# BenChung/SuccessiveConvexification

Measured on AMD Instinct MI355X. Metric: 6-DoF K=50 SCvx iterations/sec (batch), higher is better.
Workload: dtype f64

## Files before the change

successiveconvexification_amd/csrc/scvx_batch.hip:

```cpp
#include <cmath>
#include <cstdlib>
#include <cstring>
#include <limits>
#include <new>
#include <vector>

#include <cstdio>
#include "scvx_socp.hpp"

using scvx::fail;

namespace scvx {

__global__ __launch_bounds__(64, SCVX_K4_OCC) void socp_kernel(ipm::Consts C, int B, size_t work_stride,
                                                  const double* __restrict__ x, const double* __restrict__ u,
                                                  const double* __restrict__ endpoint, const double* __restrict__ deriv,
                                                  const double* __restrict__ rk, const double* __restrict__ ic,
                                                  const int* __restrict__ active, double* __restrict__ work,
                                                  double* __restrict__ sol, double* __restrict__ nu,
                                                  double* __restrict__ info, const int* __restrict__ step_status,
                                                  double* __restrict__ ttr, double* __restrict__ acc,
                                                  const double* __restrict__ marg) {
    socp_body<WaveEx>(C, B, work_stride, x, u, endpoint, deriv, rk, ic, active, work, sol, nu, info, step_status, ttr, acc, marg);
}
__global__ __launch_bounds__(64, SCVX_K4_OCC) void socp_lin32_kernel(ipm::Consts C, int B, size_t work_stride,
                                                  const double* __restrict__ x, const double* __restrict__ u,
                                                  const double* __restrict__ endpoint, const float* __restrict__ deriv,
                                                  const double* __restrict__ rk, const double* __restrict__ ic,
                                                  const int* __restrict__ active, double* __restrict__ work,
                                                  double* __restrict__ sol, double* __restrict__ nu,
                                                  double* __restrict__ info, const int* __restrict__ step_status,
                                                  double* __restrict__ ttr, double* __restrict__ acc,
                                                  const double* __restrict__ marg) {
    socp_body<WaveEx, float>(C, B, work_stride, x, u, endpoint, deriv, rk, ic, active, work, sol, nu, info, step_status, ttr, acc, marg);
}


__global__ void candidate_kernel(int B, int nrec, const double* __restrict__ traj, const double* __restrict__ sol,
                                 double* __restrict__ cand) {
    const size_t i = (size_t)blockIdx.x * blockDim.x + threadIdx.x;
    if (i < (size_t)B * nrec) cand[i] = traj[i] + sol[i];
}

__global__ void unpack_kernel(int B, int K, int NU, const double* __restrict__ rec, double* __restrict__ x,
                              double* __restrict__ u, double* __restrict__ sigma) {
    const int nrec = (K + 1) * (14 + NU) + 1, nx = (K + 1) * 14, nu = (K + 1) * NU;
    const size_t i = (size_t)blockIdx.x * blockDim.x + threadIdx.x;
    if (i >= (size_t)B * nrec) return;
    const size_t b = i / nrec;
    const int r = (int)(i - b * nrec);
    const double v = rec[i];
    if (r < nx) x[b * nx + r] = v;
    else if (r < nx + nu) u[b * nu + (r - nx)] = v;
    else sigma[b] = v;
}

struct TrParams {
    double wNu, rh0, rh1, rh2, alph, bet, ri, nuTol, delTol;
    int K, imax, NU, pad;
};

__global__ __launch_bounds__(64) void tr_update_kernel(TrParams P, int B, const double* __restrict__ cand,
                                                       const double* __restrict__ xprop, const double* __restrict__ nu,
                                                       const double* __restrict__ info, double* __restrict__ traj,
                                                       double* __restrict__ rk, double* __restrict__ cost,
                                                       int* __restrict__ iter, int* __restrict__ status,
                                                       const int* mask , int* active,
                                                       int* live, double* __restrict__ out, double* __restrict__ acc,
                                                       int* __restrict__ nlive, int* __restrict__ k1skip) {
    const int b = blockIdx.x;
    if (b >= B) return;
    if (!mask[b]) {
        if (threadIdx.x == 0) k1skip[b] = SCVX_ST_REJECTED;
        return;
    }
    const int K = P.K, nrec = (K + 1) * (14 + P.NU) + 1;
    const double* c = cand + (size_t)b * nrec;
    const double* xp = xprop + (size_t)b * K * 14;
    const double* nv = nu + (size_t)b * K * 14;
    double d2 = 0, n2 = 0;
    for (int i = threadIdx.x; i < K * 14; i += 64) {
        const double d = c[14 + i] - xp[i];
        d2 += d * d;
        n2 += nv[i] * nv[i];
    }
#pragma unroll
    for (int o = 32; o > 0; o >>= 1) { d2 += __shfl_xor(d2, o, 64); n2 += __shfl_xor(n2, o, 64); }
    const double mf = c[14 * K];
    const double jK = -mf + P.wNu * sqrt(d2);
    const double nun = sqrt(n2);
    const double lK = -mf + P.wNu * nun;
    const int sstat = (int)info[4 * b];
    int st;
    bool accept = false;
    double next_rk = rk[b], dJ = INFINITY;
    if (sstat != 0 && sstat != 4) {
        st = sstat == 3 ? SCVX_ST_NONFINITE : (sstat == 5 ? SCVX_ST_INFEASIBLE : SCVX_ST_SOLVER);
    } else if (!(jK == jK) || !(lK == lK)) {
        st = SCVX_ST_NONFINITE;
    } else {
        const double jKm = cost[b];
        const double djk = jKm - jK, dlk = jKm - lK;
        const double rhk = djk / dlk;
        if (rk[b] == INFINITY) { next_rk = P.ri; accept = true; dJ = NAN; }
        else if (rhk < P.rh0) { next_rk = rk[b] / P.alph; accept = false; dJ = INFINITY; }
        else {
            accept = true;
            dJ = djk;
            if (rhk < P.rh1) next_rk = rk[b] / P.alph;
            else if (P.rh1 <= rhk && rhk < P.rh2) next_rk = rk[b];
            else next_rk = P.bet * rk[b];
        }
        st = accept ? SCVX_ST_RUNNING : SCVX_ST_REJECTED;
    }
    if (accept) {
        double* t = traj + (size_t)b * nrec;
        for (int i = threadIdx.x; i < nrec; i += 64) t[i] = c[i];
    }
    if (threadIdx.x == 0) {
        const int it = iter[b] + 1;
        iter[b] = it;
        const int was_live = live[b];
        if (st == SCVX_ST_SOLVER || st == SCVX_ST_NONFINITE || st == SCVX_ST_INFEASIBLE) {
            active[b] = 0;
            live[b] = 0;
        } else {
            rk[b] = next_rk;
            if (accept) cost[b] = jK;
            if (accept && nun <= P.nuTol && dJ <= P.delTol) { st = SCVX_ST_CONVERGED; live[b] = 0; }
        }
        if (was_live && !live[b]) atomicSub(nlive, 1);
        status[b] = st;
        k1skip[b] = accept && st != SCVX_ST_SOLVER && st != SCVX_ST_NONFINITE && st != SCVX_ST_INFEASIBLE ? SCVX_ST_RUNNING : SCVX_ST_REJECTED;
        out[2 * b] = nun;
        out[2 * b + 1] = dJ;
        atomicAdd(acc + ACC_TRAJ_STEPS, 1.0);
        if (st == SCVX_ST_REJECTED) atomicAdd(acc + ACC_REJECTED, 1.0);
        else if (st == SCVX_ST_CONVERGED) atomicAdd(acc + ACC_CONVERGED, 1.0);
        else if (st != SCVX_ST_RUNNING) atomicAdd(acc + ACC_FAILED, 1.0);
    }
}

__global__ void reset_scalars_kernel(int B, double* __restrict__ rk, double* __restrict__ cost, int* __restrict__ iter,
                                     int* __restrict__ status, int* __restrict__ active, int* __restrict__ live,
                                     double* __restrict__ out, double* __restrict__ info) {
    const int i = blockIdx.x * blockDim.x + threadIdx.x;
    if (i >= B) return;
    rk[i] = 100.0; cost[i] = INFINITY; iter[i] = 0; status[i] = SCVX_ST_RUNNING; active[i] = 1; live[i] = 1;
    out[2 * i] = 0.0; out[2 * i + 1] = 0.0;
    for (int q = 0; q < 4; q++) info[4 * i + q] = 0.0;
}

__global__ void replan_scalars_kernel(int B, double* __restrict__ rk, double* __restrict__ cost, int* __restrict__ iter,
                                      int* __restrict__ status, const int* __restrict__ active, int* __restrict__ live,
                                      double* __restrict__ ttr) {
    const int i = blockIdx.x * blockDim.x + threadIdx.x;
    if (i >= B || !active[i]) return;
    rk[i] = 100.0; cost[i] = INFINITY; iter[i] = 0; status[i] = SCVX_ST_RUNNING; live[i] = 1;
    ttr[i] = 1.7976931348623157e308;
}

__global__ __launch_bounds__(64) void margins_from_psig_kernel(int B, int K, const double* __restrict__ psig, double nsigma, double cap,
                                                               double* __restrict__ marg) {
    const int b = blockIdx.x;
    if (b >= B) return;
    const double* p = psig + (size_t)b * (K + 1) * SCVX_PSIG_N;
    int bad = 0;
    for (int k = threadIdx.x; k <= K; k += 64) {
        const double s = p[(size_t)k * SCVX_PSIG_N + SCVX_PSIG_THRUST];
        bad |= !(s == s);
    }
    bad = __syncthreads_or(bad);
    double* m = marg + (size_t)b * (K + 1) * 2;
    for (int k = threadIdx.x; k <= K; k += 64) {
        const double v = bad ? 0.0 : fmin(nsigma * p[(size_t)k * SCVX_PSIG_N + SCVX_PSIG_THRUST], cap);
        m[2 * k] = v;
        m[2 * k + 1] = v;
    }
}

__global__ void copy_flags_kernel(int B, const int* __restrict__ src, int* __restrict__ dst, int* __restrict__ nlive) {
    const int i = blockIdx.x * blockDim.x + threadIdx.x;
    const int v = i < B ? src[i] : 0;
    if (i < B) dst[i] = v;
    const unsigned long long m = __ballot(v != 0);
    if ((threadIdx.x & 63) == 0 && m) atomicAdd(nlive, (int)__popcll(m));
}

}

struct scvx_batch {
    scvx_ctx* ctx = nullptr;
    int B = 0, K = 0, nrec = 0;
    int NU = 3, dsz = 294;
    scvx_solver_opts opts{};
    scvx::ipm::Consts C{};
    scvx::TrParams tr{};
    size_t work_stride = 0;
    double *traj = nullptr, *cand = nullptr, *sol = nullptr;
    double *traj0 = nullptr;
    double *x = nullptr, *u = nullptr, *sigma = nullptr;
    double *cx = nullptr, *cu = nullptr, *csigma = nullptr;
    double *endpoint = nullptr, *deriv = nullptr, *xprop = nullptr, *nu = nullptr;
    float* deriv_f = nullptr;
    double *rk = nullptr, *cost = nullptr, *ic = nullptr, *info = nullptr, *out = nullptr, *work = nullptr;
    double *ttr = nullptr;
    double *acc = nullptr;
    double *marg = nullptr;
    bool marg_on = false;
    double *cov_s0 = nullptr, *cov_rep = nullptr, *cov_psig = nullptr;
    double *track_gain = nullptr, *track_p0 = nullptr;
    int *k1skip = nullptr;
    int *d_nlive = nullptr;
    int *h_nlive = nullptr;
    hipEvent_t ev_nlive[2] = {nullptr, nullptr};
    int *iter = nullptr, *status = nullptr;
    int *active = nullptr;
    int *live = nullptr;
    int device = 0;
    int nactive_host = -1;
    int nlive_hint = -1;
    bool initialised = false;
    bool profiling = false;
    std::vector<hipEvent_t> events;
    size_t nmarks = 0;
};

namespace {


void rotation_between_e1(const double* b, double* q) {
    const double nb = std::sqrt(b[0] * b[0] + b[1] * b[1] + b[2] * b[2]);
    double w = nb + b[0];
    double v[3];
    if (std::fabs(w) < 100 * std::numeric_limits<double>::epsilon()) {
        v[0] = 0; v[1] = 0; v[2] = 1;
        w = 0;
    } else {
        v[0] = 0; v[1] = -b[2]; v[2] = b[1];
    }
    const double n = std::sqrt(w * w + v[0] * v[0] + v[1] * v[1] + v[2] * v[2]);
    q[0] = w / n; q[1] = v[0] / n; q[2] = v[1] / n; q[3] = v[2] / n;
}

template <class T>
int dmalloc(scvx_ctx* ctx, T** p, size_t n) {
    SCVX_HIP(ctx, hipMalloc((void**)p, n * sizeof(T)));
    return SCVX_OK;
}

int split_views(scvx_batch* b, const double* rec, double* x, double* u, double* sigma) {
    const size_t n = (size_t)b->B * b->nrec;
    hipLaunchKernelGGL(scvx::unpack_kernel, dim3((unsigned)((n + 255) / 256)), dim3(256), 0, b->ctx->stream, b->B, b->K, b->NU,
                       rec, x, u, sigma);
    SCVX_HIP(b->ctx, hipGetLastError());
    return SCVX_OK;
}

int socp_waves(int B, int num_cus) {
    if (const char* v = std::getenv("SCVX_K4_WAVES"); v && *v) {
        const int w = std::atoi(v);
        return w >= 4 ? 4 : (w >= 2 ? 2 : 1);
    }
    const int cus = num_cus > 0 ? num_cus : 256;
    return B <= 2 * cus ? 4 : (B <= 4 * cus ? 2 : 1);
}

template <int NW>
void launch_socp_block(scvx_batch* b, const int* mask) {
    constexpr int NU = 3;
    if (b->deriv_f)
        hipLaunchKernelGGL((scvx::socp_block_kernel<NW, float, NU>), dim3(b->B), dim3(64 * NW), 0, b->ctx->stream, b->C, b->B, b->work_stride,
                           b->x, b->u, b->endpoint, b->deriv_f, b->rk, b->ic, mask, b->work, b->sol, b->nu, b->info, b->status, b->ttr, b->acc, b->marg_on ? b->marg : nullptr);
    else
        hipLaunchKernelGGL((scvx::socp_block_kernel<NW, double, NU>), dim3(b->B), dim3(64 * NW), 0, b->ctx->stream, b->C, b->B, b->work_stride,
                           b->x, b->u, b->endpoint, b->deriv, b->rk, b->ic, mask, b->work, b->sol, b->nu, b->info, b->status, b->ttr, b->acc, b->marg_on ? b->marg : nullptr);
}

hipError_t relinearize(scvx_batch* b, const int* skip) {
    const double dt = 1.0 / (b->K + 1);
    if (b->deriv_f)
        return scvx::launch_linearize_store_f32(b->ctx, b->B, b->K, b->x, b->u, b->sigma, dt, b->endpoint, b->deriv_f, b->ctx->stream, skip);
    return scvx::launch_linearize(b->ctx, b->B, b->K, b->x, b->u, b->sigma, dt, b->endpoint, b->deriv, b->ctx->stream, skip);
}

int enqueue_socp(scvx_batch* b, const int* mask) {
    const int w = socp_waves(b->nlive_hint >= 0 && b->nlive_hint < b->B ? (b->nlive_hint > 0 ? b->nlive_hint : 1) : b->B, b->ctx->num_cus);
    if (b->NU == 5) {
        scvx::SocpLaunch a{b->C, b->B, b->work_stride, b->x, b->u, b->endpoint, b->deriv, b->deriv_f, b->rk, b->ic, mask,
                           b->work, b->sol, b->nu, b->info, b->status, b->ttr, b->acc, b->marg_on ? b->marg : nullptr, b->ctx->stream};
        scvx::launch_socp_fin(a, w);
    } else if (w == 4) launch_socp_block<4>(b, mask);
    else if (w == 2) launch_socp_block<2>(b, mask);
    else if (b->deriv_f)
        hipLaunchKernelGGL(scvx::socp_lin32_kernel, dim3(b->B), dim3(64), 0, b->ctx->stream, b->C, b->B, b->work_stride, b->x, b->u,
                           b->endpoint, b->deriv_f, b->rk, b->ic, mask, b->work, b->sol, b->nu, b->info, b->status, b->ttr, b->acc, b->marg_on ? b->marg : nullptr);
    else
        hipLaunchKernelGGL(scvx::socp_kernel, dim3(b->B), dim3(64), 0, b->ctx->stream, b->C, b->B, b->work_stride, b->x, b->u,
                           b->endpoint, b->deriv, b->rk, b->ic, mask, b->work, b->sol, b->nu, b->info, b->status, b->ttr, b->acc, b->marg_on ? b->marg : nullptr);
    SCVX_HIP(b->ctx, hipGetLastError());
    return SCVX_OK;
}

constexpr size_t PROF_MAX_STEPS = 4096;

int mark(scvx_batch* b) {
    if (!b->profiling || b->nmarks >= 7 * PROF_MAX_STEPS) return SCVX_OK;
    if (b->nmarks == b->events.size()) {
        hipEvent_t e;
        SCVX_HIP(b->ctx, hipEventCreate(&e));
        b->events.push_back(e);
    }
    SCVX_HIP(b->ctx, hipEventRecord(b->events[b->nmarks], b->ctx->stream));
    b->nmarks++;
    return SCVX_OK;
}

int enqueue_step(scvx_batch* b, const int* mask) {
    scvx_ctx* ctx = b->ctx;
    hipStream_t st = ctx->stream;
    const double dt = 1.0 / (b->K + 1);
    int rc = mark(b);
    if (rc) return rc;
    rc = enqueue_socp(b, mask);
    if (rc) return rc;
    if ((rc = mark(b))) return rc;
    const size_t n = (size_t)b->B * b->nrec;
    hipLaunchKernelGGL(scvx::candidate_kernel, dim3((unsigned)((n + 255) / 256)), dim3(256), 0, st, b->B, b->nrec, b->traj,
                       b->sol, b->cand);
    SCVX_HIP(ctx, hipGetLastError());
    rc = split_views(b, b->cand, b->cx, b->cu, b->csigma);
    if (rc) return rc;
    if ((rc = mark(b))) return rc;
    SCVX_HIP(ctx, scvx::launch_propagate(ctx, b->B, b->K, b->cx, b->cu, b->csigma, dt, b->xprop, st));
    if ((rc = mark(b))) return rc;
    hipLaunchKernelGGL(scvx::tr_update_kernel, dim3(b->B), dim3(64), 0, st, b->tr, b->B, b->cand, b->xprop, b->nu, b->info,
                       b->traj, b->rk, b->cost, b->iter, b->status, mask, b->active, b->live, b->out, b->acc, b->d_nlive, b->k1skip);
    SCVX_HIP(ctx, hipGetLastError());
    if ((rc = mark(b))) return rc;
    rc = split_views(b, b->traj, b->x, b->u, b->sigma);
    if (rc) return rc;
    if ((rc = mark(b))) return rc;
    SCVX_HIP(ctx, relinearize(b, b->k1skip));
    if ((rc = mark(b))) return rc;
    return SCVX_OK;
}

int check_batch(scvx_batch* b, bool need_init) {
    if (!b || !b->ctx) return SCVX_ERR_ARG;
    if (need_init && !b->initialised) return fail(b->ctx, SCVX_ERR_STATE, "call scvx_batch_init first");
    if (b->ctx->prob.aero_kind == 1 && !b->ctx->dyn.aero)
        return fail(b->ctx, SCVX_ERR_STATE, "AtmosphericData problem: call scvx_set_aero_table first");
    hipError_t e = hipSetDevice(b->ctx->device);
    if (e != hipSuccess) return fail(b->ctx, SCVX_ERR_HIP, "hipSetDevice failed");
    return SCVX_OK;
}

}

extern "C" {

int scvx_solver_default_opts(scvx_solver_opts* o) {
    if (!o) return SCVX_ERR_ARG;
    o->max_iter = 60;
    o->refine = 6;
    o->tol = 1e-8;
    o->accept_tol = 1e-8;
    o->reuse_inactive_tr = 0;
    o->warm_start = 1;
    o->retries = 5;
    o->reserved0 = 0;
    return SCVX_OK;
}

int scvx_batch_create(scvx_ctx* ctx, int B, scvx_batch** out) {
    if (!ctx || !out) return SCVX_ERR_ARG;
    *out = nullptr;
    if (B < 1) return fail(ctx, SCVX_ERR_ARG, "B >= 1 required");
    SCVX_HIP(ctx, hipSetDevice(ctx->device));
    scvx_batch* b = new (std::nothrow) scvx_batch();
    if (!b) return SCVX_ERR_NOMEM;
    b->ctx = ctx;
    b->device = ctx->device;
    b->B = B;
    const scvx_problem& p = ctx->prob;
    const int K = p.K;
    b->K = K;
    b->NU = scvx_control_dim(ctx);
    b->dsz = 14 * (14 + 2 * b->NU + 1);
    b->nrec = (K + 1) * (14 + b->NU) + 1;
    scvx_solver_default_opts(&b->opts);
    scvx::ipm::Consts& C = b->C;
    const double d2r = M_PI / 180.0;
    C.K = K; C.max_iter = b->opts.max_iter; C.refine = b->opts.refine; C.pad = 0; C.tol = b->opts.tol;
    C.accept = b->opts.accept_tol;
    C.pad = b->opts.reuse_inactive_tr;
    C.warm = b->opts.warm_start;
    C.retries = b->opts.retries;
    C.itan = 1.0 / std::tan(p.gammaGs * d2r);
    C.sqcm = std::sqrt((1.0 - std::cos(p.thetaMax * d2r)) / 2.0);
    C.icos = 1.0 / std::cos(p.deltaMax * d2r);
    C.Tmax = p.Tmax; C.Tmin = p.Tmin; C.omMax = p.omMax; C.mdry = p.mdry; C.wNu = p.wNu; C.mwet = p.mwet;
    C.vmax = (p.model_flags & SCVX_MODEL_DPMAX) ? std::sqrt(2.0 * p.dpMax / p.rho) : 0.0;
    C.finmxf = p.finmxf;
    for (int i = 0; i < 3; i++) { C.rIf[i] = p.rIf[i]; C.vIf[i] = p.vIf[i]; C.wBi[i] = p.wBi[i]; C.wBf[i] = p.wBf[i]; }
    for (int i = 0; i < 4; i++) C.qBIf[i] = p.qBIf[i];
    scvx::TrParams& T = b->tr;
    T.wNu = p.wNu; T.rh0 = p.rh0; T.rh1 = p.rh1; T.rh2 = p.rh2; T.alph = p.alph; T.bet = p.bet; T.ri = p.ri;
    T.nuTol = p.nuTol; T.delTol = p.delTol; T.K = K; T.imax = p.imax; T.NU = b->NU; T.pad = 0;
    scvx::ipm::Layout L;
    L.init(K, C.vmax > 0.0, b->NU);
    b->work_stride = (L.work_doubles() + 7) & ~(size_t)7;
    if (const char* v = std::getenv("SCVX_WORK_PAD"); v && *v) b->work_stride += (size_t)std::atoi(v) & ~(size_t)7;
    const size_t nB = (size_t)B;
    int rc = 0;
    rc |= dmalloc(ctx, &b->traj, nB * b->nrec);
    rc |= dmalloc(ctx, &b->cand, nB * b->nrec);
    rc |= dmalloc(ctx, &b->traj0, nB * b->nrec);
    rc |= dmalloc(ctx, &b->sol, nB * b->nrec);
    rc |= dmalloc(ctx, &b->x, nB * (K + 1) * 14);
    rc |= dmalloc(ctx, &b->u, nB * (K + 1) * b->NU);
    rc |= dmalloc(ctx, &b->sigma, nB);
    rc |= dmalloc(ctx, &b->cx, nB * (K + 1) * 14);
    rc |= dmalloc(ctx, &b->cu, nB * (K + 1) * b->NU);
    rc |= dmalloc(ctx, &b->csigma, nB);
    rc |= dmalloc(ctx, &b->endpoint, nB * K * 14);
    rc |= dmalloc(ctx, &b->deriv, nB * K * b->dsz);
    rc |= dmalloc(ctx, &b->xprop, nB * K * 14);
    rc |= dmalloc(ctx, &b->nu, nB * K * 14);
    rc |= dmalloc(ctx, &b->rk, nB);
    rc |= dmalloc(ctx, &b->cost, nB);
    rc |= dmalloc(ctx, &b->ic, nB * 6);
    rc |= dmalloc(ctx, &b->info, nB * 4);
    rc |= dmalloc(ctx, &b->out, nB * 2);
    rc |= dmalloc(ctx, &b->ttr, nB);
    rc |= dmalloc(ctx, &b->acc, (size_t)scvx::ACC_N);
    rc |= dmalloc(ctx, &b->d_nlive, (size_t)1);
    rc |= dmalloc(ctx, &b->k1skip, nB);
    rc |= dmalloc(ctx, &b->marg, nB * (K + 1) * 2);
    if (!rc && (hipHostMalloc((void**)&b->h_nlive, 2 * sizeof(int), hipHostMallocDefault) != hipSuccess ||
                hipEventCreateWithFlags(&b->ev_nlive[0], hipEventDisableTiming) != hipSuccess ||
                hipEventCreateWithFlags(&b->ev_nlive[1], hipEventDisableTiming) != hipSuccess)) rc = SCVX_ERR_HIP;
    if (!rc && hipMemset(b->acc, 0, sizeof(double) * scvx::ACC_N) != hipSuccess) rc = SCVX_ERR_HIP;
    rc |= dmalloc(ctx, &b->work, nB * b->work_stride);
    rc |= dmalloc(ctx, &b->iter, nB);
    rc |= dmalloc(ctx, &b->status, nB);
    rc |= dmalloc(ctx, &b->active, nB);
    rc |= dmalloc(ctx, &b->live, nB);
    if (rc) {
        scvx_batch_destroy(b);
        return fail(ctx, SCVX_ERR_NOMEM, "device allocation failed for the batch (" + std::to_string(nB * b->work_stride * 8 >> 20) + " MiB of solver workspace)");
    }
    *out = b;
    return SCVX_OK;
}

void scvx_batch_destroy(scvx_batch* b) {
    if (!b) return;
    (void)hipSetDevice(b->device);
    for (hipEvent_t e : b->events) (void)hipEventDestroy(e);
    for (hipEvent_t e : b->ev_nlive) if (e) (void)hipEventDestroy(e);
    if (b->h_nlive) (void)hipHostFree(b->h_nlive);
    void* ptrs[] = {b->traj0, b->traj, b->cand, b->sol, b->x, b->u, b->sigma, b->cx, b->cu, b->csigma, b->endpoint, b->deriv, b->xprop,
                    b->nu, b->rk, b->cost, b->ic, b->info, b->out, b->work, b->iter, b->status, b->active, b->live, b->ttr, b->deriv_f, b->acc, b->d_nlive, b->k1skip,
                    b->track_gain, b->track_p0, b->marg, b->cov_s0, b->cov_rep, b->cov_psig};
    for (void* p : ptrs)
        if (p) (void)hipFree(p);
    delete b;
}

int scvx_batch_set_solver(scvx_batch* b, const scvx_solver_opts* o) {
    if (!b || !o) return SCVX_ERR_ARG;
    if (o->max_iter < 1 || o->refine < 0 || !(o->tol > 0) || !(o->accept_tol >= o->tol) || o->retries < 0 || o->retries > 7)
        return fail(b->ctx, SCVX_ERR_ARG, "bad solver options (max_iter >= 1, refine >= 0, 0 < tol <= accept_tol, 0 <= retries <= 7)");
    if (o->reserved0 != 0)
        return fail(b->ctx, SCVX_ERR_ARG, "scvx_solver_opts.reserved0 must be 0 (start from scvx_solver_opts_default; an older struct layout is not accepted)");
    b->opts = *o;
    b->C.max_iter = o->max_iter;
    b->C.refine = o->refine;
    b->C.tol = o->tol;
    b->C.accept = o->accept_tol;
    b->C.pad = o->reuse_inactive_tr ? 1 : 0;
    b->C.warm = o->warm_start ? 1 : 0;
    b->C.retries = o->retries;
    return SCVX_OK;
}

int scvx_batch_init(scvx_batch* b, const double* ic) {
    int rc = check_batch(b, false);
    if (rc) return rc;
    scvx_ctx* ctx = b->ctx;
    const scvx_problem& p = ctx->prob;
    const int K = b->K, B = b->B, nrec = b->nrec;
    std::vector<double> rec((size_t)B * nrec), hic((size_t)B * 6), hrk(B, 100.0), hcost(B, INFINITY);
    std::vector<int> hiter(B, 0), hstat(B, SCVX_ST_RUNNING), hact(B, 1);
    for (int t = 0; t < B; t++) {
        double* c = &hic[(size_t)t * 6];
        for (int i = 0; i < 3; i++) { c[i] = ic ? ic[(size_t)t * 6 + i] : p.rIi[i]; c[3 + i] = ic ? ic[(size_t)t * 6 + 3 + i] : p.vIi[i]; }
        double* r = &rec[(size_t)t * nrec];
        double* X = r;
        double* U = r + (size_t)(K + 1) * 14;
        for (int k = 0; k <= K; k++) {
            const double a = (double)(K - k) / K, bb = (double)k / K;
            double* xk = X + 14 * k;
            const double mk = a * p.mwet + bb * p.mdry;
            xk[0] = mk;
            double nv[3];
            for (int i = 0; i < 3; i++) {
                xk[1 + i] = a * c[i] + bb * p.rIf[i];
                xk[4 + i] = a * c[3 + i] + bb * p.vIf[i];
                nv[i] = -xk[4 + i];
                xk[11 + i] = 0.0;
            }
            rotation_between_e1(nv, xk + 7);
            for (int c = 0; c < b->NU; c++) U[b->NU * k + c] = 0.0;
            U[b->NU * k] = mk * p.g;
        }
        r[nrec - 1] = p.tf_guess;
    }
    hipStream_t st = ctx->stream;
    SCVX_HIP(ctx, hipMemcpyAsync(b->traj, rec.data(), rec.size() * 8, hipMemcpyHostToDevice, st));
    SCVX_HIP(ctx, hipMemcpyAsync(b->traj0, b->traj, rec.size() * 8, hipMemcpyDeviceToDevice, st));
    SCVX_HIP(ctx, hipMemcpyAsync(b->ic, hic.data(), hic.size() * 8, hipMemcpyHostToDevice, st));
    SCVX_HIP(ctx, hipMemcpyAsync(b->rk, hrk.data(), (size_t)B * 8, hipMemcpyHostToDevice, st));
    SCVX_HIP(ctx, hipMemcpyAsync(b->cost, hcost.data(), (size_t)B * 8, hipMemcpyHostToDevice, st));
    SCVX_HIP(ctx, hipMemcpyAsync(b->iter, hiter.data(), (size_t)B * 4, hipMemcpyHostToDevice, st));
    SCVX_HIP(ctx, hipMemcpyAsync(b->status, hstat.data(), (size_t)B * 4, hipMemcpyHostToDevice, st));
    SCVX_HIP(ctx, hipMemcpyAsync(b->active, hact.data(), (size_t)B * 4, hipMemcpyHostToDevice, st));
    SCVX_HIP(ctx, hipMemcpyAsync(b->live, hact.data(), (size_t)B * 4, hipMemcpyHostToDevice, st));
    SCVX_HIP(ctx, hipMemsetAsync(b->out, 0, (size_t)B * 16, st));
    SCVX_HIP(ctx, hipMemsetAsync(b->info, 0, (size_t)B * 32, st));
    SCVX_HIP(ctx, hipMemsetAsync(b->ttr, 0x7f, (size_t)B * 8, st));
    rc = split_views(b, b->traj, b->x, b->u, b->sigma);
    if (rc) return rc;
    SCVX_HIP(ctx, relinearize(b, nullptr));
    SCVX_HIP(ctx, hipStreamSynchronize(st));
    b->initialised = true;
    b->nactive_host = -1;
    b->marg_on = false;
    return SCVX_OK;
}

int scvx_batch_init_threedof(scvx_batch* b, const double* ic, const scvx_threedof_opts* opts, int32_t* status3) {
    int rc = scvx_batch_init(b, ic);
    if (rc) return rc;
    scvx_ctx* ctx = b->ctx;
    const int B = b->B, K = b->K;
    hipStream_t st = ctx->stream;
    const size_t no = (size_t)scvx_threedof_record_doubles(K);
    double *d_sol = nullptr, *d_info = nullptr;
    hipError_t e = hipMalloc((void**)&d_sol, (size_t)B * no * 8);
    if (e == hipSuccess) e = hipMalloc((void**)&d_info, (size_t)B * 6 * 8);
    std::vector<double> hinfo((size_t)B * 6);
    if (e == hipSuccess) {
        rc = scvx::threedof_solve_dev(ctx, B, b->ic, opts, d_sol, d_info);
        if (rc == SCVX_OK) rc = scvx::threedof_to_record(ctx, B, K, d_sol, d_info, b->traj, opts ? opts->attitude : 0);
        if (rc == SCVX_OK) {
            e = hipMemcpyAsync(b->traj0, b->traj, (size_t)B * b->nrec * 8, hipMemcpyDeviceToDevice, st);
            if (e == hipSuccess) e = hipMemcpyAsync(hinfo.data(), d_info, hinfo.size() * 8, hipMemcpyDeviceToHost, st);
        }
        if (rc == SCVX_OK && e == hipSuccess) rc = split_views(b, b->traj, b->x, b->u, b->sigma);
        if (rc == SCVX_OK && e == hipSuccess)
            e = relinearize(b, nullptr);
    }
    const hipError_t es = hipStreamSynchronize(st);
    if (d_sol) (void)hipFree(d_sol);
    if (d_info) (void)hipFree(d_info);
    if (rc) return rc;
    if (e != hipSuccess || es != hipSuccess)
        return fail(ctx, SCVX_ERR_HIP, std::string("scvx_batch_init_threedof: ") + hipGetErrorString(e != hipSuccess ? e : es));
    if (status3) for (int t = 0; t < B; t++) status3[t] = (int32_t)hinfo[(size_t)t * 6];
    return SCVX_OK;
}

int scvx_batch_reset(scvx_batch* b) {
    int rc = check_batch(b, true);
    if (rc) return rc;
    scvx_ctx* ctx = b->ctx;
    hipStream_t st = ctx->stream;
    SCVX_HIP(ctx, hipMemcpyAsync(b->traj, b->traj0, (size_t)b->B * b->nrec * 8, hipMemcpyDeviceToDevice, st));
    hipLaunchKernelGGL(scvx::reset_scalars_kernel, dim3((unsigned)((b->B + 255) / 256)), dim3(256), 0, st, b->B, b->rk, b->cost,
                       b->iter, b->status, b->active, b->live, b->out, b->info);
    SCVX_HIP(ctx, hipGetLastError());
    rc = split_views(b, b->traj, b->x, b->u, b->sigma);
    if (rc) return rc;
    SCVX_HIP(ctx, relinearize(b, nullptr));
    b->nactive_host = -1;
    return SCVX_OK;
}

int scvx_solve_step_async(scvx_batch* b) {
    int rc = check_batch(b, true);
    if (rc) return rc;
    b->nlive_hint = b->nactive_host >= 0 && b->nactive_host < b->B ? b->nactive_host : -1;
    rc = enqueue_step(b, b->active);
    b->nlive_hint = -1;
    return rc;
}

static int read_step_outputs(scvx_batch* b, int32_t* status, double* nu_norm, double* dJ) {
    scvx_ctx* ctx = b->ctx;
    const int B = b->B;
    std::vector<double> out((size_t)B * 2);
    SCVX_HIP(ctx, hipMemcpyAsync(out.data(), b->out, out.size() * 8, hipMemcpyDeviceToHost, ctx->stream));
    if (status) SCVX_HIP(ctx, hipMemcpyAsync(status, b->status, (size_t)B * 4, hipMemcpyDeviceToHost, ctx->stream));
    SCVX_HIP(ctx, hipStreamSynchronize(ctx->stream));
    for (int t = 0; t < B; t++) {
        if (nu_norm) nu_norm[t] = out[2 * t];
        if (dJ) dJ[t] = out[2 * t + 1];
    }
    return SCVX_OK;
}

int scvx_solve_step(scvx_batch* b, int32_t* status, double* nu_norm, double* dJ) {
    int rc = scvx_solve_step_async(b);
    if (rc) return rc;
    return read_step_outputs(b, status, nu_norm, dJ);
// ... 372 lines not shown
        SCVX_HIP(ctx, relinearize(b, nullptr));
        SCVX_HIP(ctx, hipMemsetAsync(b->ttr, 0x7f, (size_t)b->B * 8, ctx->stream));
        SCVX_HIP(ctx, hipStreamSynchronize(ctx->stream));
    }
    return SCVX_OK;
}

int scvx_batch_get_scalars(scvx_batch* b, double* rk, double* cost, int32_t* iter) {
    int rc = check_batch(b, true);
    if (rc) return rc;
    scvx_ctx* ctx = b->ctx;
    if (rk) SCVX_HIP(ctx, hipMemcpyAsync(rk, b->rk, (size_t)b->B * 8, hipMemcpyDeviceToHost, ctx->stream));
    if (cost) SCVX_HIP(ctx, hipMemcpyAsync(cost, b->cost, (size_t)b->B * 8, hipMemcpyDeviceToHost, ctx->stream));
    if (iter) SCVX_HIP(ctx, hipMemcpyAsync(iter, b->iter, (size_t)b->B * 4, hipMemcpyDeviceToHost, ctx->stream));
    SCVX_HIP(ctx, hipStreamSynchronize(ctx->stream));
    return SCVX_OK;
}

int scvx_batch_set_scalars(scvx_batch* b, const double* rk, const double* cost, const int32_t* iter) {
    int rc = check_batch(b, true);
    if (rc) return rc;
    scvx_ctx* ctx = b->ctx;
    if (rk) SCVX_HIP(ctx, hipMemcpyAsync(b->rk, rk, (size_t)b->B * 8, hipMemcpyHostToDevice, ctx->stream));
    if (cost) SCVX_HIP(ctx, hipMemcpyAsync(b->cost, cost, (size_t)b->B * 8, hipMemcpyHostToDevice, ctx->stream));
    if (iter) SCVX_HIP(ctx, hipMemcpyAsync(b->iter, iter, (size_t)b->B * 4, hipMemcpyHostToDevice, ctx->stream));
    SCVX_HIP(ctx, hipMemsetAsync(b->ttr, 0x7f, (size_t)b->B * 8, ctx->stream));
    SCVX_HIP(ctx, hipStreamSynchronize(ctx->stream));
    return SCVX_OK;
}

int scvx_batch_get_solver_stats(scvx_batch* b, int32_t* status, int32_t* iters, double* merit, double* pobj) {
    int rc = check_batch(b, true);
    if (rc) return rc;
    scvx_ctx* ctx = b->ctx;
    std::vector<double> info((size_t)b->B * 4);
    SCVX_HIP(ctx, hipMemcpyAsync(info.data(), b->info, info.size() * 8, hipMemcpyDeviceToHost, ctx->stream));
    SCVX_HIP(ctx, hipStreamSynchronize(ctx->stream));
    for (int t = 0; t < b->B; t++) {
        if (status) status[t] = (int32_t)info[4 * t];
        if (iters) iters[t] = (int32_t)info[4 * t + 1];
        if (merit) merit[t] = info[4 * t + 2];
        if (pobj) pobj[t] = info[4 * t + 3];
    }
    return SCVX_OK;
}

int scvx_debug_build_switches(char* out, int n) {
    return std::snprintf(out, (size_t)(n > 0 ? n : 0),
                         "CHOL_DPP=%d CHOL_ORDER=%d RESID_UPDATE=%d RESID_FRESH_FROM=%g TWISTED_TSPACE=%d FUSED_RES=%d CARRY_BIGSUMS=%d REFINE_FUSED=%d "
                         "K4_OCC=%d K4_BLOCK_OCC=%d K4_PIPELINE=%d K4_TWISTED=%d STREAM_U=%d CHAIN_R=%d FACTOR_T=%d PROF=%d",
                         SCVX_CHOL_DPP, SCVX_CHOL_ORDER, SCVX_RESID_UPDATE, (double)SCVX_RESID_FRESH_FROM, SCVX_TWISTED_TSPACE, SCVX_FUSED_RES,
                         SCVX_CARRY_BIGSUMS, SCVX_REFINE_FUSED, SCVX_K4_OCC, SCVX_K4_BLOCK_OCC, SCVX_K4_PIPELINE, SCVX_K4_TWISTED, SCVX_STREAM_U,
                         SCVX_CHAIN_R, (int)sizeof(SCVX_FACTOR_T),
#if defined(SCVX_IPM_PROF)
                         1
#else
                         0
#endif
                         );
}

#if defined(SCVX_IPM_PROF)
int scvx_debug_ipm_prof(scvx_batch* b, double* out32) {
    (void)hipStreamSynchronize(b->ctx->stream);
    return hipMemcpy(out32, b->work, 128 * 8, hipMemcpyDeviceToHost) == hipSuccess ? 0 : -2;
}
#endif

int scvx_batch_get_step_stats(scvx_batch* b, double* out8, int reset) {
    int rc = check_batch(b, false);
    if (rc) return rc;
    if (!out8) return fail(b->ctx, SCVX_ERR_ARG, "null buffer");
    scvx_ctx* ctx = b->ctx;
    static_assert(scvx::ACC_N == 8, "scvx_batch_get_step_stats documents eight totals");
    SCVX_HIP(ctx, hipMemcpyAsync(out8, b->acc, sizeof(double) * scvx::ACC_N, hipMemcpyDeviceToHost, ctx->stream));
    if (reset) SCVX_HIP(ctx, hipMemsetAsync(b->acc, 0, sizeof(double) * scvx::ACC_N, ctx->stream));
    SCVX_HIP(ctx, hipStreamSynchronize(ctx->stream));
    return SCVX_OK;
}

int scvx_batch_set_profiling(scvx_batch* b, int enable) {
    if (!b) return SCVX_ERR_ARG;
    b->nmarks = 0;
    b->profiling = enable != 0;
    return SCVX_OK;
}

int scvx_batch_get_profile(scvx_batch* b, double* ms, int64_t* steps) {
    int rc = check_batch(b, true);
    if (rc) return rc;
    if (!ms || !steps) return fail(b->ctx, SCVX_ERR_ARG, "null buffer");
    scvx_ctx* ctx = b->ctx;
    SCVX_HIP(ctx, hipStreamSynchronize(ctx->stream));
    for (int i = 0; i < 5; i++) ms[i] = 0.0;
    const size_t n = b->nmarks / 7;
    static const int slot[6] = {0, 4, 1, 2, 4, 3};
    for (size_t s = 0; s < n; s++)
        for (int i = 0; i < 6; i++) {
            float t = 0.f;
            SCVX_HIP(ctx, hipEventElapsedTime(&t, b->events[7 * s + i], b->events[7 * s + i + 1]));
            ms[slot[i]] += (double)t;
        }
    *steps = (int64_t)n;
    b->nmarks = 0;
    return SCVX_OK;
}

int scvx_batch_get_flags(scvx_batch* b, int32_t* status, int32_t* active, int32_t* live) {
    int rc = check_batch(b, true);
    if (rc) return rc;
    scvx_ctx* ctx = b->ctx;
    if (status) SCVX_HIP(ctx, hipMemcpyAsync(status, b->status, (size_t)b->B * 4, hipMemcpyDeviceToHost, ctx->stream));
    if (active) SCVX_HIP(ctx, hipMemcpyAsync(active, b->active, (size_t)b->B * 4, hipMemcpyDeviceToHost, ctx->stream));
    if (live) SCVX_HIP(ctx, hipMemcpyAsync(live, b->live, (size_t)b->B * 4, hipMemcpyDeviceToHost, ctx->stream));
    SCVX_HIP(ctx, hipStreamSynchronize(ctx->stream));
    return SCVX_OK;
}

int scvx_batch_set_flags(scvx_batch* b, const int32_t* status, const int32_t* active, const int32_t* live) {
    int rc = check_batch(b, true);
    if (rc) return rc;
    scvx_ctx* ctx = b->ctx;
    if (status) SCVX_HIP(ctx, hipMemcpyAsync(b->status, status, (size_t)b->B * 4, hipMemcpyHostToDevice, ctx->stream));
    if (active) {
        SCVX_HIP(ctx, hipMemcpyAsync(b->active, active, (size_t)b->B * 4, hipMemcpyHostToDevice, ctx->stream));
        int n = 0;
        for (int t = 0; t < b->B; t++) n += active[t] != 0;
        b->nactive_host = n;
    }
    if (live) SCVX_HIP(ctx, hipMemcpyAsync(b->live, live, (size_t)b->B * 4, hipMemcpyHostToDevice, ctx->stream));
    SCVX_HIP(ctx, hipMemsetAsync(b->ttr, 0x7f, (size_t)b->B * 8, ctx->stream));
    SCVX_HIP(ctx, hipStreamSynchronize(ctx->stream));
    return SCVX_OK;
}

int scvx_allgather_trajectories(scvx_batch* b, double* out_dev) {
    int rc = check_batch(b, true);
    if (rc) return rc;
    return scvx_allgather_f64(b->ctx, b->traj, out_dev, (int64_t)b->B * b->nrec);
}

int scvx_allgather_status(scvx_batch* b, int32_t* status_out_dev, int32_t* iters_out_dev) {
    int rc = check_batch(b, true);
    if (rc) return rc;
    if (status_out_dev && (rc = scvx_allgather_i32(b->ctx, b->status, status_out_dev, b->B))) return rc;
    if (iters_out_dev && (rc = scvx_allgather_i32(b->ctx, b->iter, iters_out_dev, b->B))) return rc;
    return SCVX_OK;
}

int scvx_socp_solve(scvx_batch* b, double* sol, double* nu) {
    int rc = check_batch(b, true);
    if (rc) return rc;
    scvx_ctx* ctx = b->ctx;
    rc = enqueue_socp(b, b->active);
    if (rc) return rc;
    const size_t n = (size_t)b->B * b->nrec;
    hipLaunchKernelGGL(scvx::candidate_kernel, dim3((unsigned)((n + 255) / 256)), dim3(256), 0, ctx->stream, b->B, b->nrec,
                       b->traj, b->sol, b->cand);
    SCVX_HIP(ctx, hipGetLastError());
    if (sol) SCVX_HIP(ctx, hipMemcpyAsync(sol, b->cand, n * 8, hipMemcpyDeviceToHost, ctx->stream));
    if (nu) SCVX_HIP(ctx, hipMemcpyAsync(nu, b->nu, (size_t)b->B * b->K * 14 * 8, hipMemcpyDeviceToHost, ctx->stream));
    SCVX_HIP(ctx, hipStreamSynchronize(ctx->stream));
    return SCVX_OK;
}

}
```

successiveconvexification_amd/csrc/scvx_discretize.hip:

```cpp
#include <type_traits>
#include "scvx_internal.hpp"

namespace scvx {

constexpr int WAVES_PER_BLOCK = 4;

template <bool AERO, bool FIN = false> struct K1Map {
    static constexpr int LPS = FIN ? 25 : (AERO ? 21 : 15), SPW = FIN ? 2 : (AERO ? 3 : 4);
    static constexpr int NU = FIN ? 5 : 3, NP = 14 + 2 * NU + 1, DSZ = 14 * NP, HV = DSZ / 2;
};
__device__ __forceinline__ int exo_slot_to_col(int slot) {
    return slot == 0 ? 0 : slot + 6;
}

__device__ __forceinline__ bool block_unchanged(const int* skip, long seg0, int nseg_block, long nseg, int K) {
    if (!skip || seg0 >= nseg) return false;
    long seg1 = seg0 + nseg_block - 1;
    if (seg1 >= nseg) seg1 = nseg - 1;
    const long b0 = seg0 / K, b1 = seg1 / K;
    for (long b = b0; b <= b1; b++)
        if (skip[b] < SCVX_ST_REJECTED) return false;
    return true;
}

template <typename R> struct Vec2;
template <> struct Vec2<double> { typedef double2 type; };
template <> struct Vec2<float> { typedef float2 type; };

template <bool AERO, typename R>
__global__ __launch_bounds__(64 * WAVES_PER_BLOCK, sizeof(R) == 4 ? 2 : 1) void linearize_kernel(
    DynP<R> p, long nseg, int K, const R* __restrict__ x, const R* __restrict__ u,
    const R* __restrict__ sigma, R dt, int nsub, R* __restrict__ endpoint,
    R* __restrict__ deriv, const int* __restrict__ skip) {
    constexpr int LPS = K1Map<AERO>::LPS, SPW = K1Map<AERO>::SPW;
    typedef typename Vec2<R>::type VEC2;
    if (block_unchanged(skip, (long)blockIdx.x * WAVES_PER_BLOCK * SPW, WAVES_PER_BLOCK * SPW, nseg, K)) return;
    __shared__ __attribute__((aligned(16))) R tile[WAVES_PER_BLOCK][SPW * 294];
    const int lane = threadIdx.x & 63;
    const int wave = threadIdx.x >> 6;
    const long gwave = (long)blockIdx.x * WAVES_PER_BLOCK + wave;
    const int sl = lane / LPS;
    const int slot = lane - sl * LPS;
    const int col = AERO ? slot : exo_slot_to_col(slot);
    const long seg0 = gwave * SPW;
    long seg = seg0 + sl;
    const bool active = (sl < SPW) && (seg < nseg);
    if (!active) seg = (seg0 < nseg) ? seg0 : nseg - 1;
    const long b = seg / K;
    const int k = (int)(seg - b * K);
    const R* xk = x + ((size_t)b * (K + 1) + k) * 14;
    const R* uk = u + ((size_t)b * (K + 1) + k) * 3;
    const R sig = sigma[b];

    R xs[14], c[14];
#pragma unroll
    for (int i = 0; i < 14; i++) {
        xs[i] = xk[i];
        c[i] = (col == i) ? R(1.0) : R(0.0);
    }
    const R uk0 = uk[0], uk1 = uk[1], uk2 = uk[2];
    const R up0 = uk[3], up1 = uk[4], up2 = uk[5];
    const bool is_uk = (col >= 14) && (col < 17);
    const bool is_up = (col >= 17) && (col < 20);
    const int comp = is_uk ? col - 14 : (is_up ? col - 17 : -1);
    const R gsel = (col == 20) ? R(1.0) : R(0.0);
    const R e0 = (comp == 0) ? R(1.0) : R(0.0), e1 = (comp == 1) ? R(1.0) : R(0.0), e2 = (comp == 2) ? R(1.0) : R(0.0);

    const R h = dt / R(nsub);
    const R inv_n = R(1.0) / R(nsub);
    for (int s = 0; s < nsub; s++) {
        R xa[14], ca[14], xt[14], ct[14];
#pragma unroll
        for (int i = 0; i < 14; i++) {
            xa[i] = xs[i];
            ca[i] = c[i];
            xt[i] = xs[i];
            ct[i] = c[i];
        }
#pragma unroll
        for (int stg = 0; stg < 4; stg++) {
            const R lkp = (R(s) + (stg == 0 ? R(0.0) : (stg == 3 ? R(1.0) : R(0.5)))) * inv_n;
            const R lkm = R(1.0) - lkp;
            R uu[3] = {fma(uk0, lkm, up0 * lkp), fma(uk1, lkm, up1 * lkp), fma(uk2, lkm, up2 * lkp)};
            const R wk = is_uk ? lkm : (is_up ? lkp : R(0.0));
            const R wc[3] = {e0 * wk, e1 * wk, e2 * wk};
            Stage<AERO, R> st;
            stage_eval<AERO>(p, xt, uu, st);
            R dc[14];
            column_deriv<AERO>(p, st, xt, uu, ct, wc, gsel, sig, dc);
            const R wacc = h * ((stg == 0 || stg == 3) ? (R(1.0) / R(6.0)) : (R(1.0) / R(3.0)));
            const R wnext = h * (stg == 2 ? R(1.0) : R(0.5));
#pragma unroll
            for (int i = 0; i < 14; i++) {
                const R dx = sig * st.g[i];
                xa[i] = fma(wacc, dx, xa[i]);
                ca[i] = fma(wacc, dc[i], ca[i]);
                if (stg < 3) {
                    xt[i] = fma(wnext, dx, xs[i]);
                    ct[i] = fma(wnext, dc[i], c[i]);
                }
            }
        }
#pragma unroll
        for (int i = 0; i < 14; i++) {
            xs[i] = xa[i];
            c[i] = ca[i];
        }
    }

    R* t = tile[wave];
    if (sl < SPW) {
#pragma unroll
        for (int i = 0; i < 14; i++) t[sl * 294 + col * 14 + i] = c[i];
        if (!AERO && slot < 6) {
            const int j = slot < 3 ? slot : slot - 3;
            R* cc = t + sl * 294 + (slot < 3 ? 1 + j : 4 + j) * 14;
#pragma unroll
            for (int i = 0; i < 14; i++) cc[i] = R(0.0);
            if (slot < 3) cc[1 + j] = R(1.0);
            else { cc[1 + j] = sig * dt; cc[4 + j] = R(1.0); }
        }
    }
    __syncthreads();
    if (seg0 < nseg) {
        const long rem = nseg - seg0;
        const int nvalid = rem < SPW ? (int)rem : SPW;
        const int n2 = nvalid * 147;
        VEC2* out = reinterpret_cast<VEC2*>(deriv + (size_t)seg0 * 294);
        const VEC2* src = reinterpret_cast<const VEC2*>(t);
#pragma unroll
        for (int r = 0; r < (SPW * 147 + 63) / 64; r++) {
            const int e = lane + 64 * r;
            if (e < n2) out[e] = src[e];
        }
        if (active && slot == 0) {
            R* ep = endpoint + (size_t)seg * 14;
#pragma unroll
            for (int i = 0; i < 14; i++) ep[i] = xs[i];
        }
    }
}

#ifndef SCVX_PC_WAVES
#define SCVX_PC_WAVES 8
#endif
#ifndef SCVX_PC_PROD
#define SCVX_PC_PROD 0
#endif
#ifndef SCVX_PC_BLOCKS_PER_CU
#define SCVX_PC_BLOCKS_PER_CU 1
#endif
constexpr int PC_BLOCKS_PER_CU = SCVX_PC_BLOCKS_PER_CU;
constexpr int PC_WAVES = SCVX_PC_WAVES;
constexpr int PC_PROD = SCVX_PC_PROD;
__device__ __forceinline__ void lds_barrier() {
    __builtin_amdgcn_fence(__ATOMIC_RELEASE, "workgroup", "local");
    __builtin_amdgcn_s_barrier();
    __builtin_amdgcn_fence(__ATOMIC_ACQUIRE, "workgroup", "local");
}
#if defined(SCVX_K1_PROF)
__device__ double g_k1prof[2 * 16];
#define K1_BAR() do { const unsigned long long tb_ = __builtin_amdgcn_s_memtime(); lds_barrier(); k1wait_ += (double)(__builtin_amdgcn_s_memtime() - tb_); } while (0)
#else
#define K1_BAR() lds_barrier()
#endif
template <bool AERO, bool FIN, bool TRQ, typename R>
__device__ __forceinline__ void column_deriv_rec_any(const DynP<R>& p, const R* rec, int stride, const R* c, const R* wc, R gsel,
                                                     R sigma, R* dc) {
    column_deriv_rec_pieces<AERO, FIN, TRQ, R>(p, rec, stride, c, wc, gsel, sigma, dc);
}
constexpr int PC_GROUP = 4;
template <bool AERO, bool SG, typename R, typename O = R, bool FIN = false, bool TRQ = false>
__global__ __launch_bounds__(64 * PC_WAVES) void linearize_pc_kernel(
    DynPK<R, TRQ> p, long nseg, int K, const R* __restrict__ x, const R* __restrict__ u,
    const R* __restrict__ sigma, R dt, int nsub, R* __restrict__ endpoint,
    O* __restrict__ deriv, const int* __restrict__ skip) {
    constexpr int LPS = K1Map<AERO, FIN>::LPS, SPW = K1Map<AERO, FIN>::SPW;
    constexpr int NU = K1Map<AERO, FIN>::NU, NP = K1Map<AERO, FIN>::NP, DSZ = K1Map<AERO, FIN>::DSZ, HV = K1Map<AERO, FIN>::HV;
    typedef typename Vec2<R>::type VEC2;
    typedef typename Vec2<O>::type OVEC2;
    constexpr int NC = PC_WAVES - 1;
    if (block_unchanged(skip, (long)blockIdx.x * (NC * SPW), NC * SPW, nseg, K)) return;
    constexpr int NS = NC * SPW;
    constexpr int NR = StageRec<AERO, FIN, TRQ>::N;
    constexpr int RING = SG ? 2 : 2 * PC_GROUP;
    constexpr int RING_D = RING * NR * NS, TILE_D = NC * SPW * DSZ;
    __shared__ __attribute__((aligned(16))) R lds[RING_D > TILE_D ? RING_D : TILE_D];
    const int lane = threadIdx.x & 63;
    const int wave = threadIdx.x >> 6;
    const long seg_base = (long)blockIdx.x * NS;
    const R h = dt / R(nsub);
    const R inv_n = R(1.0) / R(nsub);

    if (wave == PC_PROD) {
        const bool live = lane < NS;
        long seg = seg_base + (live ? lane : 0);
        const bool valid = live && seg < nseg;
        if (seg >= nseg) seg = nseg - 1;
        const long b = seg / K;
        const int k = (int)(seg - b * K);
        const R* xk = x + ((size_t)b * (K + 1) + k) * 14;
        const R* uk = u + ((size_t)b * (K + 1) + k) * NU;
        const R sig = sigma[b];
        R xs[14], xa[14], xt[14];
#pragma unroll
        for (int i = 0; i < 14; i++) { xs[i] = xk[i]; xa[i] = xs[i]; xt[i] = xs[i]; }
        R ukv[NU], upv[NU];
#pragma unroll
        for (int j = 0; j < NU; j++) { ukv[j] = uk[j]; upv[j] = uk[NU + j]; }
        const int l = live ? lane : 0;
        for (int s = 0; s <= nsub; s++) {
            if (s < nsub) {
#pragma unroll
                for (int stg = 0; stg < 4; stg++) {
                    const R lkp = (R(s) + (stg == 0 ? R(0.0) : (stg == 3 ? R(1.0) : R(0.5)))) * inv_n;
                    const R lkm = R(1.0) - lkp;
                    R uu[NU];
#pragma unroll
                    for (int j = 0; j < NU; j++) uu[j] = fma(ukv[j], lkm, upv[j] * lkp);
                    struct { R g[14]; } st;
                    stage_eval_publish<AERO, FIN, TRQ>(p, xt, uu, st.g, lds + (SG ? (stg & 1) : (s & 1) * PC_GROUP + stg) * NR * NS + l, NS, live);
                    const R wacc = h * ((stg == 0 || stg == 3) ? (R(1.0) / R(6.0)) : (R(1.0) / R(3.0)));
                    const R wnext = h * (stg == 2 ? R(1.0) : R(0.5));
#pragma unroll
                    for (int i = 0; i < 14; i++) {
                        const R dx = sig * st.g[i];
                        xa[i] = fma(wacc, dx, xa[i]);
                        xt[i] = (stg < 3) ? fma(wnext, dx, xs[i]) : xa[i];
                    }
                    if (SG) __syncthreads();
                }
#pragma unroll
                for (int i = 0; i < 14; i++) xs[i] = xa[i];
            }
            if (!SG || s == nsub) __syncthreads();
        }
        if (valid) {
            R* ep = endpoint + (size_t)seg * 14;
#pragma unroll
            for (int i = 0; i < 14; i++) ep[i] = xs[i];
        }
        __syncthreads();
        return;
    }

    const int cw = wave < PC_PROD ? wave : wave - 1;
    const int sl = lane / LPS;
    const int slot = lane - sl * LPS;
    const int col = (AERO || FIN) ? slot : exo_slot_to_col(slot);
    const bool lane_live = sl < SPW;
    const int ls = cw * SPW + (lane_live ? sl : 0);
    long seg = seg_base + ls;
    if (seg >= nseg) seg = nseg - 1;
    const R sig = sigma[seg / K];
    R c[14], ca[14], ct[14];
#pragma unroll
    for (int i = 0; i < 14; i++) { c[i] = (col == i) ? R(1.0) : R(0.0); ca[i] = c[i]; ct[i] = c[i]; }
    const bool is_uk = (col >= 14) && (col < 14 + NU);
    const bool is_up = (col >= 14 + NU) && (col < 14 + 2 * NU);
    const int comp = is_uk ? col - 14 : (is_up ? col - 14 - NU : -1);
    const R gsel = (col == NP - 1) ? R(1.0) : R(0.0);
    R ec[NU];
#pragma unroll
    for (int j = 0; j < NU; j++) ec[j] = (comp == j) ? R(1.0) : R(0.0);
    __syncthreads();
    for (int s = 0; s < nsub; s++) {
#pragma unroll
        for (int stg = 0; stg < 4; stg++) {
            const R lkp = (R(s) + (stg == 0 ? R(0.0) : (stg == 3 ? R(1.0) : R(0.5)))) * inv_n;
            const R lkm = R(1.0) - lkp;
            const R wk = is_uk ? lkm : (is_up ? lkp : R(0.0));
            R wc[NU];
#pragma unroll
            for (int j = 0; j < NU; j++) wc[j] = ec[j] * wk;
            R dc[14];
            column_deriv_rec_any<AERO, FIN, TRQ>(p, lds + (SG ? (stg & 1) : (s & 1) * PC_GROUP + stg) * NR * NS + ls, NS, ct, wc, gsel, sig, dc);
            const R wacc = h * ((stg == 0 || stg == 3) ? (R(1.0) / R(6.0)) : (R(1.0) / R(3.0)));
            const R wnext = h * (stg == 2 ? R(1.0) : R(0.5));
#pragma unroll
            for (int i = 0; i < 14; i++) {
                ca[i] = fma(wacc, dc[i], ca[i]);
                ct[i] = (stg < 3) ? fma(wnext, dc[i], c[i]) : ca[i];
            }
            if (SG) __syncthreads();
        }
#pragma unroll
        for (int i = 0; i < 14; i++) c[i] = ca[i];
        if (!SG) __syncthreads();
    }
    R* t = lds + cw * SPW * DSZ;
    if (lane_live) {
#pragma unroll
        for (int i = 0; i < 14; i++) t[sl * DSZ + col * 14 + i] = c[i];
        if (!AERO && !FIN && slot < 6) {
            const int j = slot < 3 ? slot : slot - 3;
            R* cc = t + sl * DSZ + (slot < 3 ? 1 + j : 4 + j) * 14;
#pragma unroll
            for (int i = 0; i < 14; i++) cc[i] = R(0.0);
            if (slot < 3) cc[1 + j] = R(1.0);
            else { cc[1 + j] = sig * dt; cc[4 + j] = R(1.0); }
        }
    }
    __syncthreads();
    const long seg0 = seg_base + (long)cw * SPW;
    if (seg0 < nseg) {
        const long rem = nseg - seg0;
        const int nvalid = rem < SPW ? (int)rem : SPW;
        const int n2 = nvalid * HV;
        OVEC2* out = reinterpret_cast<OVEC2*>(deriv + (size_t)seg0 * DSZ);
        const VEC2* src = reinterpret_cast<const VEC2*>(t);
#pragma unroll
        for (int r = 0; r < (SPW * HV + 63) / 64; r++) {
            const int e = lane + 64 * r;
            if (e < n2) { const VEC2 v = src[e]; OVEC2 o; o.x = O(v.x); o.y = O(v.y); out[e] = o; }
        }
    }
}

#ifndef SCVX_K1_NB_EXO
#define SCVX_K1_NB_EXO 1
#endif
template <bool AERO, typename R, typename O = R, bool FIN = false, int NB = 1, bool TRQ = false>
__global__ __launch_bounds__(64 * PC_WAVES) void linearize_pcp_kernel(
    DynPK<R, TRQ> p, long nseg, int K, const R* __restrict__ x, const R* __restrict__ u,
    const R* __restrict__ sigma, R dt, int nsub, R* __restrict__ endpoint,
    O* __restrict__ deriv, const int* __restrict__ skip) {
    constexpr int LPS = K1Map<AERO, FIN>::LPS, SPW = K1Map<AERO, FIN>::SPW;
    constexpr int NU = K1Map<AERO, FIN>::NU, NP = K1Map<AERO, FIN>::NP, DSZ = K1Map<AERO, FIN>::DSZ, HV = K1Map<AERO, FIN>::HV;
    typedef typename Vec2<R>::type VEC2;
    typedef typename Vec2<O>::type OVEC2;
    constexpr bool SG = true;
    constexpr int NC = PC_WAVES - 1;
    constexpr int NS = NC * SPW * NB;
    static_assert(NS <= 64, "one producer lane per segment");
    constexpr int NR = StageRec<AERO, FIN, TRQ>::N;
    constexpr int RING = SG ? 2 : 2 * PC_GROUP;
    constexpr int RING_D = RING * NR * NS, TILE_D = NC * SPW * DSZ;
    constexpr bool SHARE = false;
    __shared__ __attribute__((aligned(16))) R lds[SHARE ? (RING_D > TILE_D ? RING_D : TILE_D) : RING_D + TILE_D];
    R* const tiles = SHARE ? lds : lds + RING_D;
    const int lane = threadIdx.x & 63;
    const int wave = threadIdx.x >> 6;
#if defined(SCVX_K1_PROF)
    double k1wait_ = 0.0;
    const unsigned long long k1t0_ = __builtin_amdgcn_s_memtime();
#endif
    const R h = dt / R(nsub);
    const R inv_n = R(1.0) / R(nsub);
    const long ngrp = (nseg + NS - 1) / NS;
    auto advance = [&](long g) {
        while (g < ngrp && block_unchanged(skip, g * NS, NS, nseg, K)) g += gridDim.x;
        return g;
    };
    long grp = advance(blockIdx.x);

    if (wave == PC_PROD) {
        const bool live = lane < NS;
        const int l = live ? lane : 0;
        R nx[14], nu6[2 * NU], nsig = R(0.0);
        auto fetch = [&](long g) {
            long seg = g * NS + l;
            if (seg >= nseg) seg = nseg - 1;
            const long b = seg / K;
            const int k = (int)(seg - b * K);
            const R* xk = x + ((size_t)b * (K + 1) + k) * 14;
            const R* uk = u + ((size_t)b * (K + 1) + k) * NU;
#pragma unroll
            for (int i = 0; i < 14; i++) nx[i] = xk[i];
#pragma unroll
            for (int i = 0; i < 2 * NU; i++) nu6[i] = uk[i];
            nsig = sigma[b];
        };
        if (grp < ngrp) fetch(grp);
        while (grp < ngrp) {
            const long nxt = advance(grp + gridDim.x);
            const long seg = grp * NS + l;
            const bool valid = live && seg < nseg;
            const R sig = nsig;
            R xs[14], xa[14], xt[14];
#pragma unroll
            for (int i = 0; i < 14; i++) { xs[i] = nx[i]; xa[i] = xs[i]; xt[i] = xs[i]; }
            R ukv[NU], upv[NU];
#pragma unroll
            for (int j = 0; j < NU; j++) { ukv[j] = nu6[j]; upv[j] = nu6[NU + j]; }
            for (int s = 0; s <= nsub; s++) {
                if (s < nsub) {
#pragma unroll
                    for (int stg = 0; stg < 4; stg++) {
                        const R lkp = (R(s) + (stg == 0 ? R(0.0) : (stg == 3 ? R(1.0) : R(0.5)))) * inv_n;
                        const R lkm = R(1.0) - lkp;
                        R uu[NU];
#pragma unroll
                        for (int j = 0; j < NU; j++) uu[j] = fma(ukv[j], lkm, upv[j] * lkp);
                        struct { R g[14]; } st;
                        stage_eval_publish<AERO, FIN, TRQ>(p, xt, uu, st.g, lds + (SG ? (stg & 1) : (s & 1) * PC_GROUP + stg) * NR * NS + l, NS, live);
                        const R wacc = h * ((stg == 0 || stg == 3) ? (R(1.0) / R(6.0)) : (R(1.0) / R(3.0)));
                        const R wnext = h * (stg == 2 ? R(1.0) : R(0.5));
#pragma unroll
                        for (int i = 0; i < 14; i++) {
                            const R dx = sig * st.g[i];
                            xa[i] = fma(wacc, dx, xa[i]);
                            xt[i] = (stg < 3) ? fma(wnext, dx, xs[i]) : xa[i];
                        }
                        if (SG) K1_BAR();
                    }
#pragma unroll
                    for (int i = 0; i < 14; i++) xs[i] = xa[i];
                }
                if (!SG || s == nsub) K1_BAR();
            }
            if (nxt < ngrp) fetch(nxt);
            if (valid) {
                R* ep = endpoint + (size_t)seg * 14;
#pragma unroll
                for (int i = 0; i < 14; i++) ep[i] = xs[i];
            }
#pragma unroll
            for (int bb = 0; bb < NB; bb++) K1_BAR();
            if (SHARE) K1_BAR();
            grp = nxt;
        }
#if defined(SCVX_K1_PROF)
        if (blockIdx.x == 0 && lane == 0) { g_k1prof[2 * wave] = k1wait_; g_k1prof[2 * wave + 1] = (double)(__builtin_amdgcn_s_memtime() - k1t0_); }
#endif
        return;
    }

    const int cw = wave < PC_PROD ? wave : wave - 1;
    const int sl = lane / LPS;
    const int slot = lane - sl * LPS;
    const int col = (AERO || FIN) ? slot : exo_slot_to_col(slot);
    const bool lane_live = sl < SPW;
    int ls[NB];
#pragma unroll
    for (int bb = 0; bb < NB; bb++) ls[bb] = (bb * NC + cw) * SPW + (lane_live ? sl : 0);
    const bool is_uk = (col >= 14) && (col < 14 + NU);
    const bool is_up = (col >= 14 + NU) && (col < 14 + 2 * NU);
    const int comp = is_uk ? col - 14 : (is_up ? col - 14 - NU : -1);
    const R gsel = (col == NP - 1) ? R(1.0) : R(0.0);
    R ec[NU];
#pragma unroll
    for (int j = 0; j < NU; j++) ec[j] = (comp == j) ? R(1.0) : R(0.0);
    auto sigma_of = [&](long g, int bb) {
        long seg = g * NS + ls[bb];
        if (seg >= nseg) seg = nseg - 1;
        return sigma[seg / K];
    };
    R nsig[NB];
#pragma unroll
    for (int bb = 0; bb < NB; bb++) nsig[bb] = grp < ngrp ? sigma_of(grp, bb) : R(0.0);
    while (grp < ngrp) {
        const long nxt = advance(grp + gridDim.x);
        const long seg_base = grp * NS;
        R sig[NB];
        R c[NB][14], ca[NB][14], ct[NB][14];
#pragma unroll
        for (int bb = 0; bb < NB; bb++) {
            sig[bb] = nsig[bb];
#pragma unroll
            for (int i = 0; i < 14; i++) { c[bb][i] = (col == i) ? R(1.0) : R(0.0); ca[bb][i] = c[bb][i]; ct[bb][i] = c[bb][i]; }
        }
        K1_BAR();
        for (int s = 0; s < nsub; s++) {
#pragma unroll
            for (int stg = 0; stg < 4; stg++) {
                const R lkp = (R(s) + (stg == 0 ? R(0.0) : (stg == 3 ? R(1.0) : R(0.5)))) * inv_n;
                const R lkm = R(1.0) - lkp;
                const R wk = is_uk ? lkm : (is_up ? lkp : R(0.0));
                R wc[NU];
#pragma unroll
                for (int j = 0; j < NU; j++) wc[j] = ec[j] * wk;
                const R wacc = h * ((stg == 0 || stg == 3) ? (R(1.0) / R(6.0)) : (R(1.0) / R(3.0)));
                const R wnext = h * (stg == 2 ? R(1.0) : R(0.5));
#pragma unroll
                for (int bb = 0; bb < NB; bb++) {
                    R dc[14];
                    column_deriv_rec_any<AERO, FIN, TRQ>(p, lds + (SG ? (stg & 1) : (s & 1) * PC_GROUP + stg) * NR * NS + ls[bb], NS, ct[bb], wc, gsel, sig[bb], dc);
#pragma unroll
                    for (int i = 0; i < 14; i++) {
                        ca[bb][i] = fma(wacc, dc[i], ca[bb][i]);
                        ct[bb][i] = (stg < 3) ? fma(wnext, dc[i], c[bb][i]) : ca[bb][i];
                    }
                }
                if (SG) K1_BAR();
            }
#pragma unroll
            for (int bb = 0; bb < NB; bb++)
#pragma unroll
                for (int i = 0; i < 14; i++) c[bb][i] = ca[bb][i];
            if (!SG) K1_BAR();
        }
#pragma unroll
        for (int bb = 0; bb < NB; bb++) if (nxt < ngrp) nsig[bb] = sigma_of(nxt, bb);
        R* t = tiles + cw * SPW * DSZ;
#pragma unroll
        for (int bb = 0; bb < NB; bb++) {
            if (lane_live) {
#pragma unroll
                for (int i = 0; i < 14; i++) t[sl * DSZ + col * 14 + i] = c[bb][i];
                if (!AERO && !FIN && slot < 6) {
                    const int j = slot < 3 ? slot : slot - 3;
                    R* cc = t + sl * DSZ + (slot < 3 ? 1 + j : 4 + j) * 14;
#pragma unroll
                    for (int i = 0; i < 14; i++) cc[i] = R(0.0);
                    if (slot < 3) cc[1 + j] = R(1.0);
                    else { cc[1 + j] = sig[bb] * dt; cc[4 + j] = R(1.0); }
                }
            }
            K1_BAR();
            const long seg0 = seg_base + (long)(bb * NC + cw) * SPW;
            if (seg0 < nseg) {
                const long rem = nseg - seg0;
                const int nvalid = rem < SPW ? (int)rem : SPW;
                const int n2 = nvalid * HV;
                OVEC2* out = reinterpret_cast<OVEC2*>(deriv + (size_t)seg0 * DSZ);
                const VEC2* src = reinterpret_cast<const VEC2*>(t);
#pragma unroll
                for (int r = 0; r < (SPW * HV + 63) / 64; r++) {
                    const int e = lane + 64 * r;
                    if (e < n2) { const VEC2 v = src[e]; OVEC2 o; o.x = O(v.x); o.y = O(v.y); out[e] = o; }
                }
            }
        }
        if (SHARE) K1_BAR();
        grp = nxt;
    }
#if defined(SCVX_K1_PROF)
    if (blockIdx.x == 0 && lane == 0) { g_k1prof[2 * wave] = k1wait_; g_k1prof[2 * wave + 1] = (double)(__builtin_amdgcn_s_memtime() - k1t0_); }
#endif
}

#ifndef SCVX_K1_SPLIT
#define SCVX_K1_SPLIT 1
#endif
#ifndef SCVX_K1_NB
#define SCVX_K1_NB 2
#endif
template <bool AERO> struct K1Split { static constexpr int NB = AERO ? SCVX_K1_NB : 1; };
template <bool AERO, typename R, typename O = R, bool FIN = false, bool TRQ = false>
__global__ __launch_bounds__(64 * PC_WAVES) void linearize_pcp2_kernel(
    DynPK<R, TRQ> p, long nseg, int K, const R* __restrict__ x, const R* __restrict__ u,
    const R* __restrict__ sigma, R dt, int nsub, R* __restrict__ endpoint,
    O* __restrict__ deriv, const int* __restrict__ skip) {
    static_assert(AERO || FIN, "the exo producer is not the bottleneck");
    constexpr int LPS = K1Map<AERO, FIN>::LPS, SPW = K1Map<AERO, FIN>::SPW;
    constexpr int NU = K1Map<AERO, FIN>::NU, NP = K1Map<AERO, FIN>::NP, DSZ = K1Map<AERO, FIN>::DSZ, HV = K1Map<AERO, FIN>::HV;
    typedef typename Vec2<R>::type VEC2;
    typedef typename Vec2<O>::type OVEC2;
    constexpr int NC = PC_WAVES - 2;
    constexpr int NB = K1Split<AERO>::NB;
    constexpr int NS = NC * SPW * NB;
    constexpr int NR = StageRec<AERO, FIN, TRQ>::N, NH = HandRec<FIN, TRQ>::N;
    constexpr int RING_D = 3 * NR * NS, HAND_D = 2 * NH * NS, TILE_D = NC * SPW * DSZ;
    __shared__ __attribute__((aligned(16))) R lds[RING_D + HAND_D + TILE_D];
    R* const hand = lds + RING_D;
    R* const tiles = hand + HAND_D;
    const int lane = threadIdx.x & 63;
    const int wave = threadIdx.x >> 6;
#if defined(SCVX_K1_PROF)
    double k1wait_ = 0.0;
    const unsigned long long k1t0_ = __builtin_amdgcn_s_memtime();
#endif
    const R h = dt / R(nsub);
    const R inv_n = R(1.0) / R(nsub);
    const int T = 4 * nsub;
    const long ngrp = (nseg + NS - 1) / NS;
    auto advance = [&](long g) {
        while (g < ngrp && block_unchanged(skip, g * NS, NS, nseg, K)) g += gridDim.x;
        return g;
    };
    long grp = advance(blockIdx.x);

    if (wave == 0) {
        const bool live = lane < NS;
        const int l = live ? lane : 0;
        R nx[14], nu6[2 * NU], nsig = R(0.0);
        auto fetch = [&](long g) {
            long seg = g * NS + l;
            if (seg >= nseg) seg = nseg - 1;
            const long b = seg / K;
            const int k = (int)(seg - b * K);
            const R* xk = x + ((size_t)b * (K + 1) + k) * 14;
            const R* uk = u + ((size_t)b * (K + 1) + k) * NU;
#pragma unroll
            for (int i = 0; i < 14; i++) nx[i] = xk[i];
#pragma unroll
            for (int i = 0; i < 2 * NU; i++) nu6[i] = uk[i];
            nsig = sigma[b];
        };
        if (grp < ngrp) fetch(grp);
        while (grp < ngrp) {
            const long nxt = advance(grp + gridDim.x);
            const long seg = grp * NS + l;
            const bool valid = live && seg < nseg;
            const R sig = nsig;
            R xs[14], xa[14], xt[14];
#pragma unroll
            for (int i = 0; i < 14; i++) { xs[i] = nx[i]; xa[i] = xs[i]; xt[i] = xs[i]; }
            R ukv[NU], upv[NU];
#pragma unroll
            for (int j = 0; j < NU; j++) { ukv[j] = nu6[j]; upv[j] = nu6[NU + j]; }
            int slot = 0, hs = 0;
            for (int s = 0; s < nsub; s++) {
#pragma unroll
                for (int stg = 0; stg < 4; stg++) {
                    const R lkp = (R(s) + (stg == 0 ? R(0.0) : (stg == 3 ? R(1.0) : R(0.5)))) * inv_n;
                    const R lkm = R(1.0) - lkp;
                    R uu[NU];
#pragma unroll
                    for (int j = 0; j < NU; j++) uu[j] = fma(ukv[j], lkm, upv[j] * lkp);
                    struct { R g[14]; } st;
                    stage_state_publish<AERO, FIN, TRQ>(p, xt, uu, st.g, lds + slot * NR * NS + l, NS, live, hand + hs * NH * NS + l, NS);
                    const R wacc = h * ((stg == 0 || stg == 3) ? (R(1.0) / R(6.0)) : (R(1.0) / R(3.0)));
                    const R wnext = h * (stg == 2 ? R(1.0) : R(0.5));
#pragma unroll
                    for (int i = 0; i < 14; i++) {
                        const R dx = sig * st.g[i];
                        xa[i] = fma(wacc, dx, xa[i]);
                        xt[i] = (stg < 3) ? fma(wnext, dx, xs[i]) : xa[i];
                    }
                    slot = slot == 2 ? 0 : slot + 1;
                    hs ^= 1;
                    K1_BAR();
                }
#pragma unroll
                for (int i = 0; i < 14; i++) xs[i] = xa[i];
            }
            K1_BAR();
            K1_BAR();
            if (nxt < ngrp) fetch(nxt);
            if (valid) {
                R* ep = endpoint + (size_t)seg * 14;
#pragma unroll
                for (int i = 0; i < 14; i++) ep[i] = xs[i];
            }
#pragma unroll
            for (int bb = 0; bb < NB; bb++) K1_BAR();
            grp = nxt;
        }
#if defined(SCVX_K1_PROF)
        if (blockIdx.x == 0 && lane == 0) { g_k1prof[2 * wave] = k1wait_; g_k1prof[2 * wave + 1] = (double)(__builtin_amdgcn_s_memtime() - k1t0_); }
#endif
        return;
    }
    if (wave == 1) {
        const bool live = lane < NS;
        const int l = live ? lane : 0;
        while (grp < ngrp) {
            const long nxt = advance(grp + gridDim.x);
            int slot = 0, hs = 0;
            K1_BAR();
            for (int n = 0; n < T; n++) {
                stage_cols_publish<AERO, FIN, TRQ>(p, hand + hs * NH * NS + l, NS, lds + slot * NR * NS + l, NS, live);
                slot = slot == 2 ? 0 : slot + 1;
                hs ^= 1;
                K1_BAR();
            }
            K1_BAR();
#pragma unroll
            for (int bb = 0; bb < NB; bb++) K1_BAR();
            grp = nxt;
        }
#if defined(SCVX_K1_PROF)
        if (blockIdx.x == 0 && lane == 0) { g_k1prof[2 * wave] = k1wait_; g_k1prof[2 * wave + 1] = (double)(__builtin_amdgcn_s_memtime() - k1t0_); }
#endif
        return;
    }

    const int cw = wave - 2;
    const int sl = lane / LPS;
    const int slot_c = lane - sl * LPS;
    const int col = slot_c;
    const bool lane_live = sl < SPW;
    int ls[NB];
#pragma unroll
    for (int bb = 0; bb < NB; bb++) ls[bb] = (bb * NC + cw) * SPW + (lane_live ? sl : 0);
    const bool is_uk = (col >= 14) && (col < 14 + NU);
    const bool is_up = (col >= 14 + NU) && (col < 14 + 2 * NU);
    const int comp = is_uk ? col - 14 : (is_up ? col - 14 - NU : -1);
    const R gsel = (col == NP - 1) ? R(1.0) : R(0.0);
    R ec[NU];
#pragma unroll
    for (int j = 0; j < NU; j++) ec[j] = (comp == j) ? R(1.0) : R(0.0);
    auto sigma_of = [&](long g, int bb) {
        long seg = g * NS + ls[bb];
        if (seg >= nseg) seg = nseg - 1;
        return sigma[seg / K];
    };
    R nsig[NB];
#pragma unroll
    for (int bb = 0; bb < NB; bb++) nsig[bb] = grp < ngrp ? sigma_of(grp, bb) : R(0.0);
    while (grp < ngrp) {
        const long nxt = advance(grp + gridDim.x);
        const long seg_base = grp * NS;
        R sig[NB];
        R c[NB][14], ca[NB][14], ct[NB][14];
#pragma unroll
        for (int bb = 0; bb < NB; bb++) {
            sig[bb] = nsig[bb];
#pragma unroll
            for (int i = 0; i < 14; i++) { c[bb][i] = (col == i) ? R(1.0) : R(0.0); ca[bb][i] = c[bb][i]; ct[bb][i] = c[bb][i]; }
        }
        K1_BAR();
        K1_BAR();
        int slot = 0;
        for (int s = 0; s < nsub; s++) {
#pragma unroll
            for (int stg = 0; stg < 4; stg++) {
                const R lkp = (R(s) + (stg == 0 ? R(0.0) : (stg == 3 ? R(1.0) : R(0.5)))) * inv_n;
                const R lkm = R(1.0) - lkp;
                const R wk = is_uk ? lkm : (is_up ? lkp : R(0.0));
                R wc[NU];
#pragma unroll
                for (int j = 0; j < NU; j++) wc[j] = ec[j] * wk;
                const R wacc = h * ((stg == 0 || stg == 3) ? (R(1.0) / R(6.0)) : (R(1.0) / R(3.0)));
                const R wnext = h * (stg == 2 ? R(1.0) : R(0.5));
#pragma unroll
                for (int bb = 0; bb < NB; bb++) {
                    R dc[14];
                    column_deriv_rec_any<AERO, FIN, TRQ>(p, lds + slot * NR * NS + ls[bb], NS, ct[bb], wc, gsel, sig[bb], dc);
#pragma unroll
                    for (int i = 0; i < 14; i++) {
                        ca[bb][i] = fma(wacc, dc[i], ca[bb][i]);
                        ct[bb][i] = (stg < 3) ? fma(wnext, dc[i], c[bb][i]) : ca[bb][i];
                    }
                }
                slot = slot == 2 ? 0 : slot + 1;
                K1_BAR();
            }
#pragma unroll
            for (int bb = 0; bb < NB; bb++)
#pragma unroll
                for (int i = 0; i < 14; i++) c[bb][i] = ca[bb][i];
        }
#pragma unroll
        for (int bb = 0; bb < NB; bb++) if (nxt < ngrp) nsig[bb] = sigma_of(nxt, bb);
        R* t = tiles + cw * SPW * DSZ;
#pragma unroll
        for (int bb = 0; bb < NB; bb++) {
            if (lane_live) {
#pragma unroll
                for (int i = 0; i < 14; i++) t[sl * DSZ + col * 14 + i] = c[bb][i];
            }
            K1_BAR();
            const long seg0 = seg_base + (long)(bb * NC + cw) * SPW;
            if (seg0 < nseg) {
                const long rem = nseg - seg0;
                const int nvalid = rem < SPW ? (int)rem : SPW;
                const int n2 = nvalid * HV;
                OVEC2* out = reinterpret_cast<OVEC2*>(deriv + (size_t)seg0 * DSZ);
                const VEC2* src = reinterpret_cast<const VEC2*>(t);
#pragma unroll
                for (int r = 0; r < (SPW * HV + 63) / 64; r++) {
                    const int e = lane + 64 * r;
                    if (e < n2) { const VEC2 v = src[e]; OVEC2 o; o.x = O(v.x); o.y = O(v.y); out[e] = o; }
                }
            }
        }
        grp = nxt;
    }
#if defined(SCVX_K1_PROF)
    if (blockIdx.x == 0 && lane == 0) { g_k1prof[2 * wave] = k1wait_; g_k1prof[2 * wave + 1] = (double)(__builtin_amdgcn_s_memtime() - k1t0_); }
#endif
}

template <bool AERO, typename R, bool FIN = false, bool TRQ = false>
__global__ __launch_bounds__(256) void propagate_kernel(DynPK<R, TRQ> p, long nseg, int K, const R* __restrict__ x,
                                                        const R* __restrict__ u,
                                                        const R* __restrict__ sigma, R dt, int nsub,
                                                        R* __restrict__ xnext) {
    const long seg = (long)blockIdx.x * blockDim.x + threadIdx.x;
    if (seg >= nseg) return;
    const long b = seg / K;
    const int k = (int)(seg - b * K);
    const R* xk = x + ((size_t)b * (K + 1) + k) * 14;
    constexpr int NU = FIN ? 5 : 3;
    const R* uk = u + ((size_t)b * (K + 1) + k) * NU;
    const R sig = sigma[b];
    R xs[14];
#pragma unroll
    for (int i = 0; i < 14; i++) xs[i] = xk[i];
    R ukv[NU], upv[NU];
#pragma unroll
    for (int j = 0; j < NU; j++) { ukv[j] = uk[j]; upv[j] = uk[NU + j]; }
    const R h = dt / R(nsub);
    const R inv_n = R(1.0) / R(nsub);
    for (int s = 0; s < nsub; s++) {
        R xa[14], xt[14];
#pragma unroll
        for (int i = 0; i < 14; i++) {
            xa[i] = xs[i];
            xt[i] = xs[i];
        }
#pragma unroll
        for (int stg = 0; stg < 4; stg++) {
            const R lkp = (R(s) + (stg == 0 ? R(0.0) : (stg == 3 ? R(1.0) : R(0.5)))) * inv_n;
            const R lkm = R(1.0) - lkp;
            R uu[NU];
#pragma unroll
            for (int j = 0; j < NU; j++) uu[j] = fma(ukv[j], lkm, upv[j] * lkp);
            R g[14];
            rhs_only<AERO, FIN, TRQ>(p, xt, uu, g);
            const R wacc = h * ((stg == 0 || stg == 3) ? (R(1.0) / R(6.0)) : (R(1.0) / R(3.0)));
            const R wnext = h * (stg == 2 ? R(1.0) : R(0.5));
#pragma unroll
            for (int i = 0; i < 14; i++) {
                const R dx = sig * g[i];
                xa[i] = fma(wacc, dx, xa[i]);
                if (stg < 3) xt[i] = fma(wnext, dx, xs[i]);
            }
        }
#pragma unroll
        for (int i = 0; i < 14; i++) xs[i] = xa[i];
    }
    R* o = xnext + (size_t)seg * 14;
#pragma unroll
    for (int i = 0; i < 14; i++) o[i] = xs[i];
}

template <typename R>
hipError_t launch_linearize_simple(const scvx_ctx* ctx, int B, int K, const R* x, const R* u, const R* sigma, R dt,
                                   R* endpoint, R* deriv, hipStream_t st, const int* skip = nullptr) {
    const long nseg = (long)B * K;
    if (nseg == 0) return hipSuccess;
    const int spw = ctx->dyn.aero ? K1Map<true>::SPW : K1Map<false>::SPW;
    const long nwave = (nseg + spw - 1) / spw;
    const unsigned grid = (unsigned)((nwave + WAVES_PER_BLOCK - 1) / WAVES_PER_BLOCK);
    const DynP<R> dp(ctx->dyn);
    if (ctx->dyn.aero)
        hipLaunchKernelGGL((linearize_kernel<true, R>), dim3(grid), dim3(64 * WAVES_PER_BLOCK), 0, st, dp, nseg, K, x, u,
                           sigma, dt, ctx->nsub, endpoint, deriv, skip);
    else
        hipLaunchKernelGGL((linearize_kernel<false, R>), dim3(grid), dim3(64 * WAVES_PER_BLOCK), 0, st, dp, nseg, K, x, u,
                           sigma, dt, ctx->nsub, endpoint, deriv, skip);
    return hipGetLastError();
}

template <typename R, typename O = R>
hipError_t launch_linearize_t(const scvx_ctx* ctx, int B, int K, const R* x, const R* u, const R* sigma, R dt, R* endpoint,
                              O* deriv, hipStream_t st, const int* skip = nullptr) {
    const long nseg = (long)B * K;
    if (nseg == 0) return hipSuccess;
    const bool fin = ctx->dyn.fin != 0;
    const bool trq = ctx->dyn.trq != 0;
    if constexpr (std::is_same<R, O>::value)
        if (ctx->k1_variant == 0 && !fin && !trq) return launch_linearize_simple<R>(ctx, B, K, x, u, sigma, dt, endpoint, deriv, st, skip);
    const bool split = SCVX_K1_SPLIT != 0 && (fin || ctx->dyn.aero) && ctx->k1_sg != 0 && (ctx->k1_persist < 0 ? ctx->nsub >= 3 : ctx->k1_persist != 0);
    const bool exo_nb = !fin && !ctx->dyn.aero && ctx->k1_sg != 0 && (ctx->k1_persist < 0 ? ctx->nsub >= 3 : ctx->k1_persist != 0);
    const int ns = (PC_WAVES - (split ? 2 : 1)) * (split ? (ctx->dyn.aero ? K1Split<true>::NB : K1Split<false>::NB) : (exo_nb ? SCVX_K1_NB_EXO : 1))
                   * (fin ? K1Map<true, true>::SPW : (ctx->dyn.aero ? K1Map<true>::SPW : K1Map<false>::SPW));
    const bool sg = ctx->k1_sg != 0;
    const long ngrp = (nseg + ns - 1) / ns;
    const long cap = (long)(ctx->num_cus > 0 ? ctx->num_cus : 256) * PC_BLOCKS_PER_CU;
    const bool persist = (sg || fin || trq) && (ctx->k1_persist < 0 ? ctx->nsub >= 3 : ctx->k1_persist != 0);
    const unsigned grid = (unsigned)(!persist || ngrp < cap ? ngrp : cap);
    const dim3 g(grid), blk(64 * PC_WAVES);
    const DynP<R> dp(ctx->dyn);
    if (trq) {
        const DynPT<R> dpt(ctx->dyn);
        if (split) {
            if (fin) hipLaunchKernelGGL((linearize_pcp2_kernel<true, R, O, true, true>), g, blk, 0, st, dpt, nseg, K, x, u, sigma, dt, ctx->nsub, endpoint, deriv, skip);
            else hipLaunchKernelGGL((linearize_pcp2_kernel<true, R, O, false, true>), g, blk, 0, st, dpt, nseg, K, x, u, sigma, dt, ctx->nsub, endpoint, deriv, skip);
        } else if (persist) {
            if (fin) hipLaunchKernelGGL((linearize_pcp_kernel<true, R, O, true, 1, true>), g, blk, 0, st, dpt, nseg, K, x, u, sigma, dt, ctx->nsub, endpoint, deriv, skip);
            else hipLaunchKernelGGL((linearize_pcp_kernel<true, R, O, false, 1, true>), g, blk, 0, st, dpt, nseg, K, x, u, sigma, dt, ctx->nsub, endpoint, deriv, skip);
        } else {
            if (fin) hipLaunchKernelGGL((linearize_pc_kernel<true, true, R, O, true, true>), g, blk, 0, st, dpt, nseg, K, x, u, sigma, dt, ctx->nsub, endpoint, deriv, skip);
            else hipLaunchKernelGGL((linearize_pc_kernel<true, true, R, O, false, true>), g, blk, 0, st, dpt, nseg, K, x, u, sigma, dt, ctx->nsub, endpoint, deriv, skip);
        }
    } else if (split) {
        if (fin) {
            if (ctx->dyn.aero) hipLaunchKernelGGL((linearize_pcp2_kernel<true, R, O, true>), g, blk, 0, st, dp, nseg, K, x, u, sigma, dt, ctx->nsub, endpoint, deriv, skip);
            else hipLaunchKernelGGL((linearize_pcp2_kernel<false, R, O, true>), g, blk, 0, st, dp, nseg, K, x, u, sigma, dt, ctx->nsub, endpoint, deriv, skip);
        } else hipLaunchKernelGGL((linearize_pcp2_kernel<true, R, O, false>), g, blk, 0, st, dp, nseg, K, x, u, sigma, dt, ctx->nsub, endpoint, deriv, skip);
    } else if (fin) {
        if (persist) {
            if (ctx->dyn.aero) hipLaunchKernelGGL((linearize_pcp_kernel<true, R, O, true>), g, blk, 0, st, dp, nseg, K, x, u, sigma, dt, ctx->nsub, endpoint, deriv, skip);
            else hipLaunchKernelGGL((linearize_pcp_kernel<false, R, O, true>), g, blk, 0, st, dp, nseg, K, x, u, sigma, dt, ctx->nsub, endpoint, deriv, skip);
        } else {
            if (ctx->dyn.aero) hipLaunchKernelGGL((linearize_pc_kernel<true, true, R, O, true>), g, blk, 0, st, dp, nseg, K, x, u, sigma, dt, ctx->nsub, endpoint, deriv, skip);
            else hipLaunchKernelGGL((linearize_pc_kernel<false, true, R, O, true>), g, blk, 0, st, dp, nseg, K, x, u, sigma, dt, ctx->nsub, endpoint, deriv, skip);
        }
    } else if (persist) {
        if (ctx->dyn.aero) hipLaunchKernelGGL((linearize_pcp_kernel<true, R, O>), g, blk, 0, st, dp, nseg, K, x, u, sigma, dt, ctx->nsub, endpoint, deriv, skip);
        else hipLaunchKernelGGL((linearize_pcp_kernel<false, R, O, false, SCVX_K1_NB_EXO>), g, blk, 0, st, dp, nseg, K, x, u, sigma, dt, ctx->nsub, endpoint, deriv, skip);
    } else if (ctx->dyn.aero) {
        if (sg) hipLaunchKernelGGL((linearize_pc_kernel<true, true, R, O>), g, blk, 0, st, dp, nseg, K, x, u, sigma, dt, ctx->nsub, endpoint, deriv, skip);
        else hipLaunchKernelGGL((linearize_pc_kernel<true, false, R, O>), g, blk, 0, st, dp, nseg, K, x, u, sigma, dt, ctx->nsub, endpoint, deriv, skip);
    } else {
        if (sg) hipLaunchKernelGGL((linearize_pc_kernel<false, true, R, O>), g, blk, 0, st, dp, nseg, K, x, u, sigma, dt, ctx->nsub, endpoint, deriv, skip);
        else hipLaunchKernelGGL((linearize_pc_kernel<false, false, R, O>), g, blk, 0, st, dp, nseg, K, x, u, sigma, dt, ctx->nsub, endpoint, deriv, skip);
    }
    return hipGetLastError();
}

hipError_t launch_linearize(const scvx_ctx* ctx, int B, int K, const double* x, const double* u, const double* sigma,
                            double dt, double* endpoint, double* deriv, hipStream_t st, const int* skip) {
    return launch_linearize_t<double>(ctx, B, K, x, u, sigma, dt, endpoint, deriv, st, skip);
}

hipError_t launch_linearize_store_f32(const scvx_ctx* ctx, int B, int K, const double* x, const double* u, const double* sigma,
                                      double dt, double* endpoint, float* deriv, hipStream_t st, const int* skip) {
    return launch_linearize_t<double, float>(ctx, B, K, x, u, sigma, dt, endpoint, deriv, st, skip);
}

hipError_t launch_linearize_f32(const scvx_ctx* ctx, int B, int K, const float* x, const float* u, const float* sigma,
                                float dt, float* endpoint, float* deriv, hipStream_t st) {
    if (ctx->nsub <= 2 && ctx->k1_variant != 0 && !ctx->dyn.fin && !ctx->dyn.trq) return launch_linearize_simple<float>(ctx, B, K, x, u, sigma, dt, endpoint, deriv, st);
    return launch_linearize_t<float>(ctx, B, K, x, u, sigma, dt, endpoint, deriv, st);
}

template <typename R>
hipError_t launch_propagate_t(const scvx_ctx* ctx, int B, int K, const R* x, const R* u, const R* sigma, R dt, R* xnext,
                              hipStream_t st) {
    const long nseg = (long)B * K;
    if (nseg == 0) return hipSuccess;
    const unsigned grid = (unsigned)((nseg + 255) / 256);
    const DynP<R> dp(ctx->dyn);
    if (ctx->dyn.trq) {
        const DynPT<R> dpt(ctx->dyn);
        if (ctx->dyn.fin) hipLaunchKernelGGL((propagate_kernel<true, R, true, true>), dim3(grid), dim3(256), 0, st, dpt, nseg, K, x, u, sigma, dt, ctx->nsub, xnext);
        else hipLaunchKernelGGL((propagate_kernel<true, R, false, true>), dim3(grid), dim3(256), 0, st, dpt, nseg, K, x, u, sigma, dt, ctx->nsub, xnext);
    } else if (ctx->dyn.fin) {
        if (ctx->dyn.aero) hipLaunchKernelGGL((propagate_kernel<true, R, true>), dim3(grid), dim3(256), 0, st, dp, nseg, K, x, u, sigma, dt, ctx->nsub, xnext);
        else hipLaunchKernelGGL((propagate_kernel<false, R, true>), dim3(grid), dim3(256), 0, st, dp, nseg, K, x, u, sigma, dt, ctx->nsub, xnext);
    } else if (ctx->dyn.aero)
        hipLaunchKernelGGL((propagate_kernel<true, R>), dim3(grid), dim3(256), 0, st, dp, nseg, K, x, u, sigma, dt,
                           ctx->nsub, xnext);
    else
        hipLaunchKernelGGL((propagate_kernel<false, R>), dim3(grid), dim3(256), 0, st, dp, nseg, K, x, u, sigma, dt,
                           ctx->nsub, xnext);
    return hipGetLastError();
}

hipError_t launch_propagate(const scvx_ctx* ctx, int B, int K, const double* x, const double* u, const double* sigma,
                            double dt, double* xnext, hipStream_t st) {
    return launch_propagate_t<double>(ctx, B, K, x, u, sigma, dt, xnext, st);
}
hipError_t launch_propagate_f32(const scvx_ctx* ctx, int B, int K, const float* x, const float* u, const float* sigma,
                                float dt, float* xnext, hipStream_t st) {
    return launch_propagate_t<float>(ctx, B, K, x, u, sigma, dt, xnext, st);
}

#if defined(SCVX_K1_PROF)
extern "C" int scvx_debug_k1_prof(double* out32) {
    (void)hipDeviceSynchronize();
    return hipMemcpyFromSymbol(out32, HIP_SYMBOL(g_k1prof), sizeof(double) * 32) == hipSuccess ? 0 : -2;
}
#endif

}
```

successiveconvexification_amd/csrc/scvx_internal.hpp:

```cpp
#pragma once
#include <hip/hip_runtime.h>
#include <string>
#include "scvx.h"
#include "scvx_dyn.hpp"

namespace scvx { struct TdCache; }

struct scvx_ctx {
    int device = 0;
    hipStream_t own_stream = nullptr;
    hipStream_t stream = nullptr;
    scvx_problem prob{};
    scvx::DynParams dyn{};
    int nsub = 10;
    int k1_persist = -1;
    int num_cus = 0;
    int k1_variant = 1;
    int k1_sg = 1;
    double* d_cdrag = nullptr;
    double* d_clift = nullptr;
    double* d_ctrq = nullptr;
    void* comm = nullptr;
    int comm_rank = 0, comm_world = 0;
    scvx::TdCache* td = nullptr;
    std::string err;
};

namespace scvx {

struct NcclId { char internal[SCVX_COMM_ID_BYTES]; };

hipError_t launch_linearize(const scvx_ctx* ctx, int B, int K, const double* x, const double* u, const double* sigma,
                            double dt, double* endpoint, double* deriv, hipStream_t st, const int* skip = nullptr);
hipError_t launch_linearize_store_f32(const scvx_ctx* ctx, int B, int K, const double* x, const double* u, const double* sigma,
                                      double dt, double* endpoint, float* deriv, hipStream_t st, const int* skip = nullptr);
hipError_t launch_propagate(const scvx_ctx* ctx, int B, int K, const double* x, const double* u, const double* sigma,
                            double dt, double* xnext, hipStream_t st);

hipError_t launch_linearize_f32(const scvx_ctx* ctx, int B, int K, const float* x, const float* u, const float* sigma,
                                float dt, float* endpoint, float* deriv, hipStream_t st);
hipError_t launch_propagate_f32(const scvx_ctx* ctx, int B, int K, const float* x, const float* u, const float* sigma,
                                float dt, float* xnext, hipStream_t st);

struct PathK {
    double rIf[3], vIf[3], qBIf[4], wBf[3];
    double mdry, tggs, sqcm, omMax, Tmax, Tmin, inv_cosd, vmax, finmxf;
    int dp;
};
PathK path_constants(const scvx_problem& P);

__device__ __forceinline__ double nan_max(double a, double v) { return (v > a || v != v) ? v : a; }
__device__ __forceinline__ double nan_min(double a, double v) { return (v < a || v != v) ? v : a; }

template <typename T>
struct DevBuf {
    T* p = nullptr;
    ~DevBuf() {
        if (p) (void)hipFree(p);
    }
};

hipError_t launch_flight(const scvx_ctx* ctx, int B, int K, const double* x, const double* u, const double* sigma, int nsub,
                         int mode, double* report, double* xfly, hipStream_t st);
int check_flight(scvx_ctx* ctx, int B, int K, const void* x, const void* u, const void* sigma, int nsub, int mode, const void* report);

hipError_t launch_track_gains(const scvx_ctx* ctx, int B, int K, const double* deriv, const double* q, const double* r, const double* qf,
                              double* gain, double* p0, hipStream_t st);
hipError_t launch_track_gains_f32(const scvx_ctx* ctx, int B, int K, const float* deriv, const double* q, const double* r,
                                  const double* qf, double* gain, double* p0, hipStream_t st);
hipError_t launch_track_fly(const scvx_ctx* ctx, int B, int K, const double* x, const double* u, const double* sigma, const double* gain,
                            const double* dx0, int nsub, int flags, double* report, double* xfly, double* ufly, hipStream_t st);
hipError_t launch_track_fly_nav(const scvx_ctx* ctx, int B, int K, const double* x, const double* u, const double* sigma,
                                const double* gain, const double* dx0, const double* nav, int nsub, int flags, double* report,
                                double* xfly, double* ufly, hipStream_t st);
int check_track_weights(scvx_ctx* ctx, const double* q, const double* r, const double* qf);
int check_track_fly(scvx_ctx* ctx, int B, int K, const void* x, const void* u, const void* sigma, const void* gain, int nsub, int flags,
                    const void* report);

hipError_t launch_cov(const scvx_ctx* ctx, int B, int K, const double* x, const double* u, const double* deriv, const double* gain,
                      const double* S0, const double* w, double* report, double* sig, double* covK, double* cov, hipStream_t st);
hipError_t launch_cov_f32(const scvx_ctx* ctx, int B, int K, const double* x, const double* u, const float* deriv, const double* gain,
                          const double* S0, const double* w, double* report, double* sig, double* covK, double* cov, hipStream_t st);
hipError_t launch_cov_psig(const scvx_ctx* ctx, int B, int K, const double* x, const double* u, const double* deriv, const double* gain,
                           const double* S0, const double* w, double* report, double* psig, hipStream_t st);
hipError_t launch_cov_psig_f32(const scvx_ctx* ctx, int B, int K, const double* x, const double* u, const float* deriv, const double* gain,
                               const double* S0, const double* w, double* report, double* psig, hipStream_t st);
int check_cov_noise(scvx_ctx* ctx, const double* w);
int check_cov(scvx_ctx* ctx, int B, int K, const void* x, const void* u, const void* deriv, const void* gain, const void* S0,
              const double* w, const void* report);

hipError_t launch_nav_cov(const scvx_ctx* ctx, int B, int K, const double* x, const double* u, const double* deriv, const double* gain,
                          const double* S0, const double* N0, int m, const double* H, const double* rm, const double* w, double* report,
                          double* navrep, double* sig, double* navsig, double* kf, double* joint, hipStream_t st);
hipError_t launch_nav_cov_f32(const scvx_ctx* ctx, int B, int K, const double* x, const double* u, const float* deriv, const double* gain,
                              const double* S0, const double* N0, int m, const double* H, const double* rm, const double* w,
                              double* report, double* navrep, double* sig, double* navsig, double* kf, double* joint, hipStream_t st);
int check_nav_model(scvx_ctx* ctx, int m, const double* H, const double* rm);

int threedof_solve_dev(scvx_ctx* ctx, int B, const double* ic_dev, const scvx_threedof_opts* opts, double* sol_dev,
                       double* info_dev);
int threedof_to_record(scvx_ctx* ctx, int B, int K, const double* sol_dev, const double* info_dev, double* rec_dev, int attitude);
void td_cache_free(scvx_ctx* ctx);

inline int fail(scvx_ctx* ctx, int code, const std::string& msg) {
    if (ctx) ctx->err = msg;
    return code;
}

}

#define SCVX_HIP(ctx, call)                                                                        \
    do {                                                                                           \
        hipError_t e_ = (call);                                                                    \
        if (e_ != hipSuccess)                                                                      \
            return scvx::fail((ctx), SCVX_ERR_HIP, std::string(#call) + ": " + hipGetErrorString(e_)); \
    } while (0)
```

successiveconvexification_amd/csrc/scvx_ipm_core.hpp:

```cpp
#pragma once
#include <math.h>
#include <stdint.h>
#include <type_traits>

#if defined(__HIPCC__)
#define SCVX_HD __host__ __device__ __forceinline__
#define SCVX_HD_NI __host__ __device__ __attribute__((noinline))
#else
#define SCVX_HD inline
#define SCVX_HD_NI inline
#endif
#if defined(SCVX_IPM_PROF) && defined(__HIP_DEVICE_COMPILE__)
#define SCVX_TS(v) const unsigned long long v = __builtin_amdgcn_s_memtime()
#define SCVX_TE(v, slot) prof[slot] += (double)(__builtin_amdgcn_s_memtime() - v)
#else
#define SCVX_TS(v)
#define SCVX_TE(v, slot)
#endif
#ifndef SCVX_NODE_QR
#define SCVX_NODE_QR 0
#endif
#ifndef SCVX_STALL_ITERS
#define SCVX_STALL_ITERS 3
#endif
// ... 236 lines not shown
    Mi[0] = i00 * i00 + i10 * i10 + i20 * i20;
    Mi[1] = Mi[3] = i10 * i11 + i20 * i21;
    Mi[2] = Mi[6] = i20 * i22;
    Mi[4] = i11 * i11 + i21 * i21;
    Mi[5] = Mi[7] = i21 * i22;
    Mi[8] = i22 * i22;
}
template <class PO>
SCVX_HD void inv2(double a, double b, double d, PO Mi) {
    const double l00 = sqrt(a), l10 = b / l00, l11 = sqrt(piv_floor(d - l10 * l10, d));
    const double i00 = 1.0 / l00, i11 = 1.0 / l11, i10 = -l10 * i00 * i11;
    Mi[0] = i00 * i00 + i10 * i10; Mi[1] = Mi[2] = i10 * i11; Mi[3] = i11 * i11;
}

template <class PO>
SCVX_HD void inv_iso_rank1_3(double a, double kappa, double v0, double v1, double v2, PO Mi) {
    const double n2 = v0 * v0 + v1 * v1 + v2 * v2;
    const double den = 1.0 / (a + kappa * n2), ia = 1.0 / a;
    const double off = -kappa * ia * den;
    Mi[0] = (a + kappa * (v1 * v1 + v2 * v2)) * ia * den;
    Mi[4] = (a + kappa * (v0 * v0 + v2 * v2)) * ia * den;
    Mi[8] = (a + kappa * (v0 * v0 + v1 * v1)) * ia * den;
    Mi[1] = Mi[3] = off * v0 * v1;
    Mi[2] = Mi[6] = off * v0 * v2;
    Mi[5] = Mi[7] = off * v1 * v2;
}
template <class PO>
SCVX_HD void inv_iso_rank1_2(double a, double kappa, double v0, double v1, PO Mi) {
    const double den = 1.0 / (a + kappa * (v0 * v0 + v1 * v1)), ia = 1.0 / a;
    Mi[0] = (a + kappa * v1 * v1) * ia * den;
    Mi[3] = (a + kappa * v0 * v0) * ia * den;
    Mi[1] = Mi[2] = -kappa * v0 * v1 * ia * den;
}
template <int D>
SCVX_HD void soc_Winv_col(const double* v, double ibeta, const double* x, double* y) {
    double vx = v[0] * x[0];
    for (int i = 1; i < D; i++) vx -= v[i] * x[i];
    y[0] = (2.0 * vx * v[0] - x[0]) * ibeta;
    for (int i = 1; i < D; i++) y[i] = (-2.0 * vx * v[i] + x[i]) * ibeta;
}
template <int NR, class PO>
SCVX_HD void qr_inv3(double (&A)[NR][3], PO Mi) {
    double R[3][3] = {{0, 0, 0}, {0, 0, 0}, {0, 0, 0}};
    for (int j = 0; j < 3; j++) {
        double nrm2 = 0;
        for (int r = j; r < NR; r++) nrm2 += A[r][j] * A[r][j];
        const double nrm = sqrt(nrm2);
        const double x0 = A[j][j];
        const double alpha = x0 > 0.0 ? -nrm : nrm;
        R[j][j] = alpha;
        const double v0 = x0 - alpha;
        const double vtv = nrm2 - x0 * x0 + v0 * v0;
        if (vtv > 0.0) {
            const double tv = 2.0 / vtv;
            for (int c = j + 1; c < 3; c++) {
                double d = v0 * A[j][c];
                for (int r = j + 1; r < NR; r++) d += A[r][j] * A[r][c];
                d *= tv;
                R[j][c] = A[j][c] - d * v0;
                for (int r = j + 1; r < NR; r++) A[r][c] -= d * A[r][j];
            }
        } else {
            for (int c = j + 1; c < 3; c++) R[j][c] = A[j][c];
        }
    }
    for (int j = 0; j < 3; j++) if (!(fabs(R[j][j]) > 1e-300)) R[j][j] = 1e-300;
    const double i00 = 1.0 / R[0][0], i11 = 1.0 / R[1][1], i22 = 1.0 / R[2][2];
    const double i01 = -R[0][1] * i00 * i11;
    const double i12 = -R[1][2] * i11 * i22;
    const double i02 = -(R[0][1] * i12 + R[0][2] * i22) * i00;
    Mi[0] = i00 * i00 + i01 * i01 + i02 * i02;
    Mi[1] = Mi[3] = i01 * i11 + i02 * i12;
    Mi[2] = Mi[6] = i02 * i22;
    Mi[4] = i11 * i11 + i12 * i12;
    Mi[5] = Mi[7] = i12 * i22;
    Mi[8] = i22 * i22;
}

template <class PH>
SCVX_HD double hxi_entry(PH h, int a, int b) {
    if (a == 0) return b == 0 ? h[HX_M] : 0.0;
    if (a < 4) return (b >= 1 && b < 4) ? h[HX_R + 3 * (a - 1) + (b - 1)] : 0.0;
    if (a < 7) return (b >= 4 && b < 7) ? h[HX_V + 3 * (a - 4) + (b - 4)] : 0.0;
    if (a < 9) return a == b ? h[HX_Q] : 0.0;
    if (a < 11) return (b >= 9 && b < 11) ? h[HX_Q34 + 2 * (a - 9) + (b - 9)] : 0.0;
    return (b >= 11) ? h[HX_W + 3 * (a - 11) + (b - 11)] : 0.0;
}
template <class PH>
SCVX_HD void hxi_apply(PH h, const double* x, double* y) {
    y[0] = h[HX_M] * x[0];
    for (int i = 0; i < 3; i++) y[1 + i] = h[HX_R + 3 * i] * x[1] + h[HX_R + 3 * i + 1] * x[2] + h[HX_R + 3 * i + 2] * x[3];
    for (int i = 0; i < 3; i++) y[4 + i] = h[HX_V + 3 * i] * x[4] + h[HX_V + 3 * i + 1] * x[5] + h[HX_V + 3 * i + 2] * x[6];
    y[7] = h[HX_Q] * x[7]; y[8] = h[HX_Q] * x[8];
    y[9] = h[HX_Q34] * x[9] + h[HX_Q34 + 1] * x[10];
    y[10] = h[HX_Q34 + 2] * x[9] + h[HX_Q34 + 3] * x[10];
    for (int i = 0; i < 3; i++) y[11 + i] = h[HX_W + 3 * i] * x[11] + h[HX_W + 3 * i + 1] * x[12] + h[HX_W + 3 * i + 2] * x[13];
}
SCVX_HD int hx_dense_pos(int l) {
    if (l >= HX_SZ) return 8 * 15;
    if (l >= HX_W) { const int q = l - HX_W; return 14 * (11 + q / 3) + 11 + q % 3; }
    if (l >= HX_Q34) { const int q = l - HX_Q34; return 14 * (9 + q / 2) + 9 + q % 2; }
    if (l == HX_Q) return 7 * 15;
    if (l >= HX_V) { const int q = l - HX_V; return 14 * (4 + q / 3) + 4 + q % 3; }
    if (l >= HX_R) { const int q = l - HX_R; return 14 * (1 + q / 3) + 1 + q % 3; }
    return 0;
}
struct Result {
    int status;
    int iters;
    double merit, pobj;
    int warmed;
    int attempts;
};

template <class Ex, class Stor = double, class DStor = Stor, int NU = 3, class FStor = SCVX_FACTOR_T>
struct Solver {
    static_assert(NU == 3 || NU == 5, "control_dim 3 (the reference's live model) or 5 (fin extension)");
    static constexpr int NP = 14 + 2 * NU + 1;
    static constexpr int DSZ = 14 * NP;
    static constexpr int CS = 14 + 2 * NU;
    static constexpr int NXU = 14 + NU;
    static constexpr int HU_SZ = hu_size(NU);
    static constexpr int NODE_SZ = HX_SZ + HU_SZ;
    static constexpr int TW = 14 + 2 * NU;
    static constexpr int TS = NU == 5 ? 26 : 22;
    static constexpr int BPN = 14 * NU;
    static constexpr int NPW = (DSZ + 63) / 64;
    typedef typename gp<Stor>::ptr gptr;
    typedef typename gp<Stor>::cptr cgptr;
    typedef typename gp<DStor>::ptr dptr;
    typedef typename gp<DStor>::cptr dcptr;
    typedef typename gp<double>::cptr cdptr;
    typedef typename gp<FStor>::ptr fptr;
    typedef typename gp<FStor>::cptr cfptr;
    Ex& ex;
    const Consts& C;
    Layout L;
    cdptr xbar, ubar, endpoint;
    dcptr D;
    double rk;
    gptr dk, V, rx, gx, dw, r1, cw, Vbest, tmpv;
    gptr y, ry, dy, r2, cy, tmpy, tmpy2, rp, tq0, tq1;
    gptr S, Z, lam, Wv, Wibz, tmpc, Wirz, sd;
    gptr Wbeta;
    gptr hx, hu;
    fptr Linv, Nf;
    gptr tchain;
    dptr At;
    gptr ys, ytr, ynu;
    gptr ptl, rtr;
    gptr tmpl, tmpl2;
    gptr uhat, lb0, tmx;
    cgptr marg = nullptr;
    gptr wh, Vw, yw, Sw, Zw;
    double h_tr[4], h_nu[4], hrk, hnui;
    double q_tr[2], q_nu[2], q_sg[4], h00s;
    double css, cst, csn, cts, ctt, ctn, cns, cnt_, pny;
    double p_step_frac = SCVX_STEP_FRAC, p_init_shift = SCVX_INIT_SHIFT, p_init_balance = SCVX_INIT_BALANCE;
    bool p_sigma_cube = false;
    double p_mu_floor = 0.25;
    double bigvz[2];
    double bigs[2][6];
    bool bigs_ok;
    double bigvv[2];
    double bigq[2][6];
    double res_nrx2, res_nry2, res_sgy;
    bool tsp;
    double gram[16];
    double gn_pred;
    double bigvx2[2];
#if defined(SCVX_IPM_PROF)
    double prof[32];
#endif
    double cur_gate;

    SCVX_HD Solver(Ex& e, const Consts& c) : ex(e), C(c) {
        L.init(c.K, c.vmax > 0.0, NU);
#if defined(SCVX_IPM_PROF)
        for (int i = 0; i < 32; i++) prof[i] = 0.0;
#endif
    }

    SCVX_HD void carve(gptr w) {
        const int nv = L.nv, ny = L.ny, nc = L.nc, nloc = L.nloc, K = L.K;
        dk = w; w += ny;
        V = w; w += nv; rx = w; w += nv; gx = w; w += nv; dw = w; w += nv; r1 = w; w += nv; cw = w; w += nv;
        Vbest = w; w += nv; tmpv = w; w += nv;
        y = w; w += ny; ry = w; w += ny; dy = w; w += ny; r2 = w; w += ny; cy = w; w += ny; tmpy = w; w += ny; tmpy2 = w; w += ny; rp = w; w += ny; tq0 = w; w += ny; tq1 = w; w += ny;
        S = w; w += nc; Z = w; w += nc; lam = w; w += nc; Wv = w; w += nc;
        Wibz = w; w += nc; tmpc = w; w += nc; Wirz = w; w += nc; sd = w; w += nc;
        Wbeta = w; w += L.ncones;
        hx = w; w += (size_t)(K + 1) * HX_SZ; hu = w; w += (size_t)(K + 1) * HU_SZ;
        Linv = (fptr)w; w += (size_t)K * LINV_SZ; Nf = (fptr)w; w += (size_t)K * 196; At = (dptr)w; w += (size_t)K * 196;
        tchain = w; w += ny;
        ys = w; w += ny; ytr = w; w += ny; ynu = w; w += ny; rtr = w; w += ny; ptl = w; w += nloc;
        tmpl = w; w += nloc; tmpl2 = w; w += nloc;
        uhat = w; w += 3 * (K + 1); lb0 = w; w += (K + 1); tmx = w; w += (K + 1);
        w += 64;
        wh = w; w += 8; Vw = w; w += nv; yw = w; w += ny; Sw = w; w += nc; Zw = w; w += nc;
    }

    SCVX_HD bool fixed_x(int k, int j) const {
        if (k == 0) return !(j >= 7 && j < 11);
        if (k == L.K) return j != 0;
        return false;
    }
    SCVX_HD bool fixed_u(int k, int c) const { return k == L.K && (c == 1 || c == 2); }

    template <class PH>
    static SCVX_HD double bhu(const double* Dt, int c0, int i, int c, PH h) {
        if (NU == 3 || c < 3) return Dt[14 * c0 + i] * h[c] + Dt[14 * (c0 + 1) + i] * h[3 + c] + Dt[14 * (c0 + 2) + i] * h[6 + c];
        return Dt[14 * (c0 + 3) + i] * h[9 + (c - 3)] + Dt[14 * (c0 + 4) + i] * h[11 + (c - 3)];
    }
    static SCVX_HD double so_elem(const double* T, const double* Bp, int i, int j) {
        double a = -T[TS * i + j];
        SCVX_UNROLL
        for (int c = 0; c < NU; c++) a += T[TS * i + 14 + c] * Bp[14 * c + j];
        return a;
    }

    template <int U = SCVX_STREAM_U, class LD, class ST>
    SCVX_HD void stream(int i0, int n, LD&& ld, ST&& st) {
        const int nl = ex.nlanes();
        int i = i0 + ex.lane();
        for (; i + (U - 1) * nl < n; i += U * nl) {
            decltype(ld(0)) v[U];
            SCVX_UNROLL
            for (int q = 0; q < U; q++) v[q] = ld(i + q * nl);
            SCVX_UNROLL
            for (int q = 0; q < U; q++) st(i + q * nl, v[q]);
        }
        for (; i < n; i += nl) st(i, ld(i));
    }
    struct D2 { double a, b; };
    struct D3 { double a, b, c; };
    struct D4 { double a, b, c, d; };
    struct D5 { double a, b, c, d, e; };

    SCVX_HD double dot(cgptr a, cgptr b, int n) {
        double s = 0;
        stream(0, n, [&](int i) { return D2{a[i], b[i]}; }, [&](int, const D2& v) { s += v.a * v.b; });
        return ex.sum(s);
    }
    SCVX_HD double sumsq(cgptr a, int n) {
        double s = 0;
        stream<8>(0, n, [&](int i) { return a[i]; }, [&](int, double v) { s += v * v; });
        return ex.sum(s);
    }
    SCVX_HD void zero(gptr o, int n) {
        for (int i = ex.lane(); i < n; i += ex.nlanes()) o[i] = 0.0;
        ex.sync();
    }
    SCVX_HD void copy(gptr o, cgptr a, int n) {
        stream<8>(0, n, [&](int i) { return a[i]; }, [&](int i, double v) { o[i] = v; });
        ex.sync();
    }

    SCVX_HD_NI double E_apply(cgptr v, gptr out, bool with_s, cgptr add = nullptr, double sa = 1.0) {
        SCVX_THIS_LDS();
        SCVX_T0();
        const int K = L.K;
        const double s = with_s ? v[L.iS] : 0.0;
        double n2 = 0;
        for (int r = ex.lane(); r < 14 * K; r += ex.nlanes()) {
            const int k = r / 14, i = r - 14 * k;
            dcptr Dk = D + (size_t)k * DSZ + i;
            cgptr dx = v + 14 * k;
            cgptr du = v + L.nx + NU * k;
            const double ad = add ? add[r] : 0.0;
            double a = 0;
            for (int j = 0; j < 14; j++) a += Dk[14 * j] * dx[j];
            for (int j = 0; j < 2 * NU; j++) a += Dk[14 * (14 + j)] * du[j];
            a += Dk[14 * CS] * s;
            a += v[L.nx + L.nu_ + r] - v[14 * (k + 1) + i];
            a += sa * ad;
            out[r] = a;
            n2 += a * a;
        }
        ex.sync();
        SCVX_T1(1);
        return ex.sum(n2);
    }
    SCVX_HD_NI double Et_apply(cgptr yy, gptr g, cgptr base = nullptr, int mode = 0, double pc = 0.0, double pn = 0.0, gptr eout = nullptr,
                               double* n2out = nullptr) {
        SCVX_THIS_LDS();
        SCVX_T0();
        const int K = L.K;
        const bool corr = pc != 0.0 || pn != 0.0;
        const bool resn = n2out != nullptr;
        double n2 = 0.0;
        cgptr Pt = Wv + L.o_tr + 1; cgptr Pn = Wv + L.o_nu + 1;
        for (int t = ex.lane(); t < L.nx; t += ex.nlanes()) {
            const int k = t / 14, j = t - 14 * k;
            const double b0 = mode ? base[t] - (corr ? pc * Pt[t] : 0.0) : 0.0;
            double a = 0;
            if (k < K) {
                dcptr col = At + (size_t)k * 196 + j;
                cgptr yk = yy + 14 * k;
                for (int i = 0; i < 14; i++) a += col[14 * i] * yk[i];
            }
            if (k > 0) a -= yy[14 * (k - 1) + j];
            if (eout) eout[t] = a;
            if (mode) a = mode == 1 ? b0 - a : a - b0;
            if (resn) {
                if (t == 14 * K) a += -1.0;
                if ((k == 0 && fixed_x(0, j)) || (k == K && fixed_x(K, j))) a = 0.0;
// ... 2469 lines not shown
            mask_fixed(gx);
        }
        SCVX_COUNT(0);
        kkt_solve(gx, ry, dw, dy, -1.0, pred);
#if defined(SCVX_IPM_DEBUG) && !defined(__HIPCC__)
        {
            H_apply(dw, r1);
            const double sgy = Et_apply(dy, tmpl);
            double e1 = 0, e2 = 0, e3 = 0;
            for (int i = 0; i < L.nloc; i++) { double r = gx[i] - r1[i] - tmpl[i]; bool fx = false;
                if (i < 14) fx = fixed_x(0, i); else if (i >= 14 * L.K && i < L.nx) fx = fixed_x(L.K, i - 14 * L.K); else if (i == L.nx + NU * L.K + 1 || i == L.nx + NU * L.K + 2) fx = true;
                if (!fx) { if (i < L.nx + L.nu_) e1 += r * r; else e2 += r * r; } }
            E_apply(dw, tmpy2, true);
            for (int i = 0; i < L.ny; i++) { double r = -ry[i] - tmpy2[i]; e3 += r * r; }
            SCVX_DBG("      kkt res: xu %.2e nu %.2e s %.2e tnu %.2e ttr %.2e ts %.2e | E %.2e\n", sqrt(e1), sqrt(e2), gx[L.iS] - r1[L.iS] - sgy,
                     gx[L.iTNU] - r1[L.iTNU], gx[L.iTTR] - r1[L.iTTR], gx[L.iTS] - r1[L.iTS], sqrt(e3));
        }
#endif
        const int nref = (cur_gate < SCVX_REFINE_FROM && !(pred && !SCVX_REFINE_PRED)) ? C.refine : 0;
        double nr_prev = INFINITY;
        for (int it = 0; it < nref; it++) {
            SCVX_COUNT(1);
            H_apply(dw, r1);
            const double sgy = Et_apply(dy, tmpl);
            ex.sync();
            {
                gptr r1_ = r1; cgptr g_ = gx; cgptr tl = tmpl;
                stream(0, L.nloc, [&](int i) { return D3{g_[i], r1_[i], tl[i]}; }, [&](int i, const D3& v) { r1_[i] = v.a - v.b - v.c; });
            }
            ex.sync();
            if (ex.lane() == 0) {
                r1[L.iS] = gx[L.iS] - r1[L.iS] - sgy;
                r1[L.iTNU] = gx[L.iTNU] - r1[L.iTNU];
                r1[L.iTTR] = gx[L.iTTR] - r1[L.iTTR];
                r1[L.iTS] = gx[L.iTS] - r1[L.iTS];
            }
            ex.sync();
            mask_fixed(r1);
            const double nr1 = sqrt(sumsq(r1, L.nv));
            SCVX_DBG("      refine %d: |r1| %.3e\n", it, nr1);
#if defined(SCVX_IPM_DEBUG) && !defined(__HIPCC__)
            if (it == 0) {
                int am = 0; double mx = 0;
                for (int i = 0; i < L.nv; i++) if (fabs((double)r1[i]) > mx) { mx = fabs((double)r1[i]); am = i; }
                if (am < L.nx) SCVX_DBG("        max at x node %d comp %d (%.3e)\n", am / 14, am % 14, mx);
                else if (am < L.nx + L.nu_) SCVX_DBG("        max at u node %d comp %d (%.3e)\n", (am - L.nx) / NU, (am - L.nx) % NU, mx);
                else SCVX_DBG("        max at index %d of nv %d (%.3e)\n", am, L.nv, mx);
            }
#endif
            if (nr1 <= SCVX_REFINE_STOP * C.tol * (C.wNu > 1.0 ? C.wNu : 1.0)) break;
            if (it > 0 && !(nr1 < 0.5 * nr_prev)) break;
            nr_prev = nr1;
            E_apply(dw, tmpy2, true);
            ex.sync();
            {
                gptr t2 = tmpy2; cgptr ry_ = ry;
                stream(0, L.ny, [&](int i) { return D2{ry_[i], t2[i]}; }, [&](int i, const D2& v) { t2[i] = -v.a - v.b; });
            }
            ex.sync();
            SCVX_COUNT(2);
            kkt_solve(r1, tmpy2, cw, cy);
            {
                gptr dw_ = dw; cgptr cw_ = cw; gptr dy_ = dy; cgptr cy_ = cy;
                stream(0, L.nv, [&](int i) { return D2{dw_[i], cw_[i]}; }, [&](int i, const D2& v) { dw_[i] = v.a + v.b; });
                stream(0, L.ny, [&](int i) { return D2{dy_[i], cy_[i]}; }, [&](int i, const D2& v) { dy_[i] = v.a + v.b; });
            }
            ex.sync();
        }
    }

    SCVX_NEWTON_CORR_ATTR double newton_corr() {
        SCVX_THIS_LDS();
        cone_map_t(tmpc, gx, rx, false, false, true);
        SCVX_COUNT(0);
        const int nref = cur_gate < SCVX_REFINE_FROM ? C.refine : 0;
        if (nref == 0) {
            kkt_solve(gx, ry, dw, dy, -1.0, false);
            return dir_pass<false>();
        }
        const gptr et = tmpv;
        double sgy = 0.0;
        kkt_solve(gx, ry, dw, dy, -1.0, false, et, &sgy);
        const int nxu = L.nx + L.nu_;
        double nr_prev = INFINITY, amax = INFINITY;
        for (int it = 0;; it++) {
            if (it >= nref) { amax = dir_pass<false>(); break; }
            amax = dir_pass<false, true>();
            SCVX_COUNT(1);
            cone_map_t(tmpc, r1, nullptr, true);
            {
                gptr r1_ = r1; cgptr g_ = gx; cgptr et_ = et; cgptr dy_ = dy;
                stream(0, nxu, [&](int i) { return D3{g_[i], r1_[i], et_[i]}; }, [&](int i, const D3& v) { r1_[i] = v.a - v.b - v.c; });
                stream(nxu, L.nloc, [&](int i) { return D3{g_[i], r1_[i], dy_[i - nxu]}; }, [&](int i, const D3& v) { r1_[i] = v.a - v.b - v.c; });
            }
            ex.sync();
            if (ex.lane() == 0) {
                r1[L.iS] = gx[L.iS] - r1[L.iS] - sgy;
                r1[L.iTNU] = gx[L.iTNU] - r1[L.iTNU];
                r1[L.iTTR] = gx[L.iTTR] - r1[L.iTTR];
                r1[L.iTS] = gx[L.iTS] - r1[L.iTS];
            }
            ex.sync();
            mask_fixed(r1);
            const double nr1 = sqrt(sumsq(r1, L.nv));
            SCVX_DBG("      refine %d: |r1| %.3e\n", it, nr1);
            if (nr1 <= SCVX_REFINE_STOP * C.tol * (C.wNu > 1.0 ? C.wNu : 1.0)) break;
            if (it > 0 && !(nr1 < 0.5 * nr_prev)) break;
            nr_prev = nr1;
            E_apply(dw, tmpy2, true);
            ex.sync();
            {
                gptr t2 = tmpy2; cgptr ry_ = ry;
                stream(0, L.ny, [&](int i) { return D2{ry_[i], t2[i]}; }, [&](int i, const D2& v) { t2[i] = -v.a - v.b; });
            }
            ex.sync();
            SCVX_COUNT(2);
            double sgc = 0.0;
            kkt_solve(r1, tmpy2, cw, cy, 1.0, false, tmpl, &sgc);
            sgy += sgc;
            {
                gptr dw_ = dw; cgptr cw_ = cw; gptr dy_ = dy; cgptr cy_ = cy; gptr et_ = et; cgptr ec = tmpl;
                stream(0, L.nv, [&](int i) { return D2{dw_[i], cw_[i]}; }, [&](int i, const D2& v) { dw_[i] = v.a + v.b; });
                stream(0, L.ny, [&](int i) { return D2{dy_[i], cy_[i]}; }, [&](int i, const D2& v) { dy_[i] = v.a + v.b; });
                stream(0, nxu, [&](int i) { return D2{et_[i], ec[i]}; }, [&](int i, const D2& v) { et_[i] = v.a + v.b; });
            }
            ex.sync();
        }
        return amax;
    }

    SCVX_HD_NI void shift_into_cone(gptr X) {
        SCVX_THIS_LDS();
        all_small([&](auto Dt_, int off, int) {
            constexpr int dm = decltype(Dt_)::value;
            double n = 0;
            for (int i = 1; i < dm; i++) n += X[off + i] * X[off + i];
            const double m = sqrt(n) - X[off];
            if (m >= -p_init_shift) X[off] += p_init_shift + m;
        }, true);
        const int offs[2] = {L.o_nu, L.o_tr};
        const int dims[2] = {14 * L.K + 1, NXU * (L.K + 1) + 1};
        for (int q = 0; q < 2; q++) {
            double n = 0;
            for (int i = 1 + ex.lane(); i < dims[q]; i += ex.nlanes()) n += X[offs[q] + i] * X[offs[q] + i];
            n = ex.sum(n);
            const double m = sqrt(n) - X[offs[q]];
            ex.sync();
            if (ex.lane() == 0 && m >= -p_init_shift) X[offs[q]] += p_init_shift + m;
        }
        ex.sync();
    }

    SCVX_HD void set_margins(cgptr m) { marg = m; }

    SCVX_HD Result solve(cdptr xbar_, cdptr ubar_, cdptr endpoint_, dcptr D_,
                         double rk_, cdptr ic, gptr work, bool warm = false) {
        xbar = xbar_; ubar = ubar_; endpoint = endpoint_; D = D_; rk = rk_;
        SCVX_TS(tTot_);
        carve(work);
        const int K = L.K;
        for (int r = ex.lane(); r < L.ny; r += ex.nlanes()) dk[r] = endpoint[r] - xbar[14 + r];
        {
            const dcptr D_ = D; const dptr At_ = At;
            stream(0, 196 * K, [&](int e) { const int k = e / 196, r = e - 196 * k, i = r / 14, j = r - 14 * i; return D_[(size_t)k * DSZ + 14 * j + i]; },
                   [&](int e, double v) { At_[e] = v; });
        }
        for (int k = ex.lane(); k <= K; k += ex.nlanes()) {
            cdptr u = ubar + NU * k;
            const double un = sqrt(u[0] * u[0] + u[1] * u[1] + u[2] * u[2]);
            for (int c = 0; c < 3; c++) uhat[3 * k + c] = u[c] / un;
            lb0[k] = (marg ? C.Tmin + marg[2 * k] : C.Tmin) - un;
            tmx[k] = marg ? C.Tmax - marg[2 * k + 1] : C.Tmax;
        }
        ex.sync();
        Result res;
        int iters_all = 0, first_warmed = 0;
        const gptr V_first = V, Vbest_first = Vbest;
        for (int attempt = 0;; attempt++) {
            V = V_first; Vbest = Vbest_first;
            const double r_step[8] = {SCVX_STEP_FRAC,   0.9,  0.95, SCVX_STEP_FRAC, 0.8, 0.9, 0.85, 0.7};
            const double r_shift[8] = {SCVX_INIT_SHIFT, SCVX_INIT_SHIFT, SCVX_INIT_SHIFT, 1.0, SCVX_INIT_SHIFT, 5.0, 2.0, 0.5};
            const double r_bal[8] = {SCVX_INIT_BALANCE, SCVX_INIT_BALANCE, SCVX_INIT_BALANCE, 0.5, SCVX_INIT_BALANCE, SCVX_INIT_BALANCE, 0.5, 2.0};
            const double r_floor[8] = {0.25, 0.25, 0.25, 0.25, 0.5, 0.25, 0.25, 0.5};
            const int a = attempt < 8 ? attempt : 7;
            p_step_frac = r_step[a]; p_init_shift = r_shift[a]; p_init_balance = r_bal[a]; p_mu_floor = r_floor[a];
            p_sigma_cube = a == 2 || a == 6;
            res = attempt_solve(ic, warm && attempt == 0);
            iters_all += res.iters;
            if (attempt == 0) first_warmed = res.warmed;
            if (!(res.status >= 1 && res.status <= 3) || attempt >= C.retries) { res.attempts = attempt + 1; break; }
            SCVX_DBG("attempt %d ended with status %d at merit %.3e: next rule\n", attempt, res.status, res.merit);
        }
        res.iters = iters_all; res.warmed = first_warmed;
        SCVX_TE(tTot_, 15);
        return res;
    }

    SCVX_HD_NI Result attempt_solve(cdptr ic, bool warm) {
        SCVX_THIS_LDS();
        const int K = L.K;
        zero(V, L.nv); zero(y, L.ny);
        if (ex.lane() == 0) {
            V[0] = C.mwet - xbar[0];
            for (int i = 0; i < 3; i++) { V[1 + i] = ic[i] - xbar[1 + i]; V[4 + i] = ic[3 + i] - xbar[4 + i]; V[11 + i] = C.wBi[i] - xbar[11 + i]; }
            cdptr xK = xbar + 14 * K;
            gptr vK = V + 14 * K;
            for (int i = 0; i < 3; i++) { vK[1 + i] = C.rIf[i] - xK[1 + i]; vK[4 + i] = C.vIf[i] - xK[4 + i]; vK[11 + i] = C.wBf[i] - xK[11 + i]; }
            for (int i = 0; i < 4; i++) vK[7 + i] = C.qBIf[i] - xK[7 + i];
            V[L.nx + NU * K + 1] = 0.0 - ubar[NU * K + 1];
            V[L.nx + NU * K + 2] = 0.0 - ubar[NU * K + 2];
        }
        ex.sync();
        Result res; res.status = 1; res.iters = 0; res.merit = INFINITY; res.pobj = 0; res.warmed = 0; res.attempts = 1;
        {
            const double r1 = ic[0], r2 = ic[1], r3 = ic[2];
            bool bad = sqrt(r2 * r2 + r3 * r3) > r1 * C.itan * (1.0 + 1e-12) + 1e-14;
            bad = bad || sqrt(C.wBi[0] * C.wBi[0] + C.wBi[1] * C.wBi[1] + C.wBi[2] * C.wBi[2]) > C.omMax * (1.0 + 1e-12);
            if (C.vmax > 0.0) bad = bad || sqrt(ic[3] * ic[3] + ic[4] * ic[4] + ic[5] * ic[5]) > C.vmax * (1.0 + 1e-12);
            if (bad) { res.status = 5; return res; }
        }
        cur_gate = INFINITY;
        bigs_ok = false;
        const bool warmed = warm && wh[0] == 1.0 && Vw[L.iTTR] < SCVX_WARM_RADIUS * rk;
        const bool blend = warm && wh[0] == 1.0 && !warmed;
        res.warmed = warmed ? 1 : 0;
        if (warmed) {
            copy(V, Vw, L.nv); copy(y, yw, L.ny); copy(S, Sw, L.nc); copy(Z, Zw, L.nc);
            if (ex.lane() == 0) {
                const double srk = rk - V[L.iTTR], flo = 1e-3 * rk;
                S[L.o_rk] = srk > flo ? srk : flo;
            }
            ex.sync();
        } else {
        ex.sync();
        if (ex.lane() == 0) wh[0] = 0.0;
        identity_scaling();
        if (!build_kkt()) { res.status = 2; return res; }
        cone_map(V, S, true);
        cone_map_t(S, gx);
        for (int i = ex.lane(); i < L.nv; i += ex.nlanes()) gx[i] = -gx[i];
        ex.sync();
        mask_fixed(gx);
        E_apply(V, ry, true);
        for (int i = ex.lane(); i < L.ny; i += ex.nlanes()) r2[i] = -(ry[i] + dk[i]);
        ex.sync();
        kkt_solve(gx, r2, dw, dy);
        for (int i = ex.lane(); i < L.nv; i += ex.nlanes()) V[i] += dw[i];
        ex.sync();
        cone_map(V, S, true);
        zero(gx, L.nv);
        if (ex.lane() == 0) { gx[14 * K] = 1.0; gx[L.iTNU] = -C.wNu; gx[L.iTTR] = -0.5; gx[L.iTS] = -1.0; }
        ex.sync();
        mask_fixed(gx);
        zero(r2, L.ny);
        kkt_solve(gx, r2, dw, y);
        cone_map(dw, Z, false);
        for (int i = ex.lane(); i < L.nc; i += ex.nlanes()) Z[i] = -Z[i];
        ex.sync();
        SCVX_DBG("init: |V|^2 %.12e s %.6e tnu %.6e ttr %.6e ts %.6e |y|^2 %.6e |S|^2 %.12e |Z|^2 %.6e\n", dot(V, V, L.nv), V[L.iS], V[L.iTNU], V[L.iTTR], V[L.iTS], dot(y, y, L.ny), dot(S, S, L.nc), dot(Z, Z, L.nc));
        shift_into_cone(S);
        shift_into_cone(Z);
        if (p_init_balance > 0.0) {
            const double sz = dot(S, Z, L.nc);
            double es = 0, ez = 0;
            all_small([&](auto, int off, int) { es += S[off]; ez += Z[off]; }, true);
            if (ex.lane() == 0) { es += S[L.o_nu] + S[L.o_tr]; ez += Z[L.o_nu] + Z[L.o_tr]; }
            es = ex.sum(es); ez = ex.sum(ez);
            const double dsh = p_init_balance * sz / ez, dzh = p_init_balance * sz / es;
            ex.sync();
            all_small([&](auto, int off, int) { S[off] += dsh; Z[off] += dzh; }, true);
            if (ex.lane() == 0) { S[L.o_nu] += dsh; S[L.o_tr] += dsh; Z[L.o_nu] += dzh; Z[L.o_tr] += dzh; }
            ex.sync();
        }
        SCVX_DBG("shifted: |S|^2 %.12e |Z|^2 %.12e\n", dot(S, S, L.nc), dot(Z, Z, L.nc));
        if (blend && SCVX_BLEND_WARM > 0.0) {
            const double lm = SCVX_BLEND_WARM, th = SCVX_BLEND_RADIUS * rk / Vw[L.iTTR];
            cone_map(V, tmpc, true);
            for (int i = ex.lane(); i < L.nc; i += ex.nlanes()) tmpc[i] = S[i] - tmpc[i];
            ex.sync();
            for (int i = ex.lane(); i < L.nv; i += ex.nlanes()) {
                bool fx = false;
                if (i < 14) fx = fixed_x(0, i); else if (i >= 14 * K && i < L.nx) fx = fixed_x(K, i - 14 * K);
                else if (i == L.nx + NU * K + 1 || i == L.nx + NU * K + 2) fx = true;
                if (!fx) V[i] = lm * th * Vw[i] + (1.0 - lm) * V[i];
            }
            for (int i = ex.lane(); i < L.ny; i += ex.nlanes()) y[i] = lm * yw[i] + (1.0 - lm) * y[i];
            ex.sync();
            cone_map(V, S, true);
            for (int i = ex.lane(); i < L.nc; i += ex.nlanes()) { S[i] += (1.0 - lm) * tmpc[i]; Z[i] = lm * Zw[i] + (1.0 - lm) * Z[i]; }
            ex.sync();
        }
        }

        double best_merit = INFINITY; int best_it = 0;
        bool best_in_V = false;
        bool kept = false;
        const int degree = L.ncones;
        bool res_carried = false;
        double nrx_c = 0.0, nry_c = 0.0;
        for (int it = 1; it <= C.max_iter; it++) {
            res.iters = it;
            double gap, nrz2;
            scale_pass(gap, nrz2);
            SCVX_TS(tR_);
            const bool fused = SCVX_FUSED_RES != 0 && Ex::kFusedResidual && !(warmed && it == 1);
            double nrx, nry;
            bool kkt_ok = true;
            auto eval_residuals = [&]() {
                cone_map_t(Z, rx);
                double nrx2 = 0.0;
                const double sgy = Et_apply(y, rx, rx, 2, 0.0, 0.0, nullptr, &nrx2);
                const double g0 = -rx[L.iS] + sgy, g1 = C.wNu - rx[L.iTNU], g2 = 0.5 - rx[L.iTTR], g3 = 1.0 - rx[L.iTS];
                ex.sync();
                if (ex.lane() == 0) { rx[L.iS] = g0; rx[L.iTNU] = g1; rx[L.iTTR] = g2; rx[L.iTS] = g3; }
                ex.sync();
// ... 119 lines not shown
```

successiveconvexification_amd/csrc/scvx_socp.hpp:

```cpp
#pragma once
#include <new>
#include "scvx_internal.hpp"
#include "scvx_ipm_core.hpp"

#ifndef SCVX_LDS_FENCE_SCOPE
#define SCVX_LDS_FENCE_SCOPE "wavefront"
#endif
#ifndef SCVX_CHOL_FUSED_INV
#define SCVX_CHOL_FUSED_INV 0
#endif
#ifndef SCVX_CHOL_DPP
#define SCVX_CHOL_DPP 2
#endif
#ifndef SCVX_CHOL_ORDER
#define SCVX_CHOL_ORDER 1
#endif
#ifndef SCVX_CHAIN_R
#define SCVX_CHAIN_R 8
#endif

namespace scvx {

__shared__ __attribute__((aligned(16))) double g_socp_lds[SCVX_FUSED_RES ? 2112 : 1904];
__shared__ __attribute__((aligned(16))) double g_socp_lds5[SCVX_FUSED_RES ? 2272 : 2072];
// ... 370 lines not shown
        const bool zin = rin && g < NR;
        const int offZ = zin ? n : 0;
        ipm::cgptr zp = z[0];
        ipm::gptr op = o[0];
#pragma unroll
        for (int q = 1; q < NR; q++) {
            if (g == q) zp = z[q];
            if (n == q) op = o[q];
        }
        const double bsel = (g == n) ? 1.0 : 0.0;
        const bool oin = n < NR;
        const bool oin3 = oin && g < 2;
        const int dk = reverse ? -1 : 1;
        typedef decltype(+(*N)) NT;
        NT st[R][4];
        double sz[R];
        auto issue = [&](int s, NT (&f)[4], double& fz) {
            const int k = k0 + dk * s;
            const NP base = N + (size_t)(reverse ? (k + 1 < K ? k + 1 : k) : k) * 196;
#pragma unroll
            for (int c = 0; c < 4; c++) f[c] = base[offA[c]];
            fz = zp[14 * k + offZ];
        };
#pragma unroll
        for (int q = 0; q < R; q++)
            if (q < ns) issue(q, st[q], sz[q]);
        v4f64 d = {0.0, 0.0, 0.0, 0.0};
        for (int s0 = 0; s0 < ns; s0 += R) {
#pragma unroll
            for (int q = 0; q < R; q++) {
                const int s = s0 + q;
                if (s < ns) {
                    const double m0 = s > 0 ? 1.0 : 0.0;
                    v4f64 acc = {0.0, 0.0, 0.0, 0.0};
                    acc = __builtin_amdgcn_mfma_f64_16x16x4f64(zin ? sz[q] : 0.0, bsel, acc, 0, 0, 0);
#pragma unroll
                    for (int c = 0; c < 4; c++) {
                        const double a = (mA[c] * m0 != 0.0) ? (double)st[q][c] : 0.0;
                        acc = __builtin_amdgcn_mfma_f64_16x16x4f64(a, d[c], acc, 0, 0, 0);
                    }
                    d = acc;
                    if (s + R < ns) issue(s + R, st[q], sz[q]);
                    const int k = k0 + dk * s;
                    const bool st_ = store_first || s > 0;
                    if (oin && st_) {
                        op[14 * k + g] = d[0];
                        op[14 * k + g + 4] = d[1];
                        op[14 * k + g + 8] = d[2];
                    }
                    if (oin3 && st_) op[14 * k + g + 12] = d[3];
                }
            }
        }
    }
    template <class NP>
    __device__ __forceinline__ void chain(int K, ipm::cgptr z, NP N, ipm::gptr out, bool reverse) {
        const ipm::cgptr zs[1] = {z};
        const ipm::gptr os[1] = {out};
        chain_n<1>(K, zs, N, os, reverse);
    }
};

typedef WaveExT<3> WaveEx;

template <int NW, int NU_ = 3>
struct BlockEx {
    WaveExT<NU_> w0;
    static constexpr int kLanes = 64 * NW;
    static constexpr int kPrefetchRegs = 1;
    static constexpr bool kFusedResidual = false;
    static constexpr bool kPipelineFactor = SCVX_K4_PIPELINE != 0;
    static constexpr bool kTwisted = SCVX_K4_PIPELINE != 0 && ((NW == 4 && SCVX_K4_TWISTED != 0) || (NW == 2 && SCVX_K4_TWISTED2 != 0));
    static constexpr int kPipeDoubles = NU_ == 5 ? SCVX_PIPE_LDS5 : SCVX_PIPE_LDS3;
    static constexpr int kPipe1Doubles = NU_ == 5 ? SCVX_PIPE1_LDS5 : SCVX_PIPE1_LDS3;
    __device__ __forceinline__ double* pipe_scratch2() { return socp_pipe_lds2<NU_>(); }
    template <int NR, class NP>
    __device__ __forceinline__ void chain_range_n(int wv, int K, const ipm::cgptr (&z)[NR], NP N, const ipm::gptr (&o)[NR],
                                                     bool reverse, int k0, int ns, bool store_first) {
        if (wave() == (NW == 2 ? wv >> 1 : wv)) w0.template chain_range_n<NR>(K, z, N, o, reverse, k0, ns, store_first);
    }
    __device__ __forceinline__ int wave() const { return (int)(threadIdx.x >> 6); }
    __device__ __forceinline__ int wlane() const { return (int)(threadIdx.x & 63); }
    __device__ __forceinline__ double* pipe_scratch() { return socp_pipe_lds<NU_>(); }
    __device__ __forceinline__ void w_sync_lds() { w0.sync_lds(); }
    __device__ __forceinline__ void w_tile_gemm(double* Cm, int sci, int scj, const double* A, int sai, int sak, const double* B,
                                                int sbk, int sbj, int Kd, double alpha, bool acc) {
        w0.tile_gemm(Cm, sci, scj, A, sai, sak, B, sbk, sbj, Kd, alpha, acc);
    }
    __device__ __forceinline__ bool w_chol_inv14(const double* M, double* Li) { return w0.chol_inv14(M, Li); }
    typedef typename WaveExT<NU_>::Acc WAcc;
    __device__ __forceinline__ void w_acc_zero(WAcc& c) { w0.acc_zero(c); }
    __device__ __forceinline__ void w_acc_mac(WAcc& c, const double* A, int sai, int sak, const double* B, int sbk, int sbj, int Kd,
                                              double alpha, int nb = 14) { w0.acc_mac(c, A, sai, sak, B, sbk, sbj, Kd, alpha, nb); }
    __device__ __forceinline__ void w_acc_store(const WAcc& c, double* Cm, int sci, int scj, bool add, int nb = 14) { w0.acc_store(c, Cm, sci, scj, add, nb); }
    __device__ __forceinline__ void w_acc_store_init(const WAcc& c, double* Cm, const double* H, double diag) { w0.acc_store_init(c, Cm, H, diag); }
    __device__ __forceinline__ void acc_store_init(const WAcc& c, double* Cm, const double* H, double diag) { if (first()) w0.acc_store_init(c, Cm, H, diag); }
    __device__ __forceinline__ int lane() const { return (int)threadIdx.x; }
    __device__ __forceinline__ int nlanes() const { return 64 * NW; }
    __device__ __forceinline__ void sync() { __syncthreads(); }
    __device__ __forceinline__ void sync_lds() { __syncthreads(); }
    __device__ __forceinline__ double* hdr() { if constexpr (kPipelineFactor) return g_socp_blk_hdr; else return socp_lds<NU_>(); }
    __device__ __forceinline__ double* scratch() { return hdr(); }
    __device__ __forceinline__ bool first() const { return threadIdx.x < 64; }
    template <class OP>
    __device__ __forceinline__ double reduce(double x, OP op) {
#pragma unroll
        for (int o = 32; o > 0; o >>= 1) x = op(x, __shfl_xor(x, o, 64));
        double* red = hdr();
        if ((threadIdx.x & 63) == 0) red[threadIdx.x >> 6] = x;
        __syncthreads();
        double r = red[0];
#pragma unroll
        for (int q = 1; q < NW; q++) r = op(r, red[q]);
        __syncthreads();
        return r;
    }
    __device__ __forceinline__ double sum(double x) { return reduce(x, [](double a, double b) { return a + b; }); }
    __device__ __forceinline__ double min(double x) { return reduce(x, [](double a, double b) { return fmin(a, b); }); }
    __device__ __forceinline__ bool all(bool b) { return __syncthreads_and(b ? 1 : 0) != 0; }
    __device__ __forceinline__ void tile_gemm(double* Cm, int sci, int scj, const double* A, int sai, int sak, const double* B,
                                              int sbk, int sbj, int Kd, double alpha, bool acc, int nb = 14) {
        if (first()) w0.tile_gemm(Cm, sci, scj, A, sai, sak, B, sbk, sbj, Kd, alpha, acc, nb);
    }
    typedef typename WaveExT<NU_>::Acc Acc;
    __device__ __forceinline__ void acc_zero(Acc& c) { w0.acc_zero(c); }
    __device__ __forceinline__ void acc_mac(Acc& c, const double* A, int sai, int sak, const double* B, int sbk, int sbj, int Kd,
                                            double alpha, int nb = 14) {
        if (first()) w0.acc_mac(c, A, sai, sak, B, sbk, sbj, Kd, alpha, nb);
    }
    __device__ __forceinline__ void acc_store(const Acc& c, double* Cm, int sci, int scj, bool add, int nb = 14) {
        if (first()) w0.acc_store(c, Cm, sci, scj, add, nb);
    }
    __device__ __forceinline__ bool chol_inv14(const double* M, double* Li) {
        double* flag = hdr() + 16;
        if (first()) {
            const bool ok = w0.chol_inv14(M, Li);
            if (threadIdx.x == 0) *flag = ok ? 1.0 : 0.0;
        }
        __syncthreads();
        const bool ok = *flag != 0.0;
        __syncthreads();
        return ok;
    }
    template <class NP>
    __device__ __forceinline__ void chain(int K, ipm::cgptr z, NP N, ipm::gptr out, bool reverse) {
        if (first()) w0.chain(K, z, N, out, reverse);
    }
    template <int NR, class NP>
    __device__ __forceinline__ void chain_n(int K, const ipm::cgptr (&z)[NR], NP N, const ipm::gptr (&o)[NR], bool reverse) {
        if (first()) w0.template chain_n<NR>(K, z, N, o, reverse);
    }
};

enum { ACC_TRAJ_STEPS = 0, ACC_SOLVES, ACC_IPM_ITERS, ACC_WARM, ACC_SKIPPED, ACC_REJECTED, ACC_FAILED, ACC_CONVERGED, ACC_N };

template <class Ex, class DS = double, int NU = 3>
__device__ __forceinline__ void socp_body(const ipm::Consts& Cin, int B, size_t work_stride, const double* x, const double* u,
                                          const double* endpoint, const DS* deriv, const double* rk, const double* ic,
                                          const int* active, double* work, double* sol, double* nu, double* info,
                                          const int* step_status, double* ttr, double* acc, const double* marg) {
    const int b = blockIdx.x;
    if (b >= B) return;
    if (active && !active[b]) return;
    if (Cin.pad && step_status[b] == SCVX_ST_REJECTED && ttr[b] <= (1.0 - 1e-6) * rk[b]) {
        if (threadIdx.x == 0) { info[4 * b + 1] = 0.0; atomicAdd(acc + ACC_SKIPPED, 1.0); }
        return;
    }
#if defined(SCVX_K4_STAGGER_US)
    if (blockIdx.x < 2048) {
        const unsigned long long t0 = __builtin_amdgcn_s_memrealtime();
        const unsigned long long wait = (unsigned long long)(((blockIdx.x * 2654435761u) >> 16) % 16u) * (unsigned long long)(SCVX_K4_STAGGER_US * 100 / 16);
        while (__builtin_amdgcn_s_memrealtime() - t0 < wait) __builtin_amdgcn_s_sleep(64);
    }
#endif
    const int K = Cin.K;
    typedef ipm::Solver<Ex, double, DS, NU, SCVX_FACTOR_T> SolverT;
    struct Frame {
        ipm::Consts C; Ex ex; SolverT S;
        __device__ Frame(const ipm::Consts& c) : C(c), ex(), S(ex, C) {}
    };
    constexpr int NWV = Ex::kLanes / 64;
    constexpr int FSZ = (int)((sizeof(Frame) + 15) & ~(size_t)15);
    __shared__ __attribute__((aligned(16))) unsigned char frame_mem[NWV * FSZ];
    Frame* const F = new (frame_mem + (threadIdx.x >> 6) * FSZ) Frame(Cin);
    const ipm::Consts& C = F->C;
    Ex& ex = F->ex;
    SolverT& S = F->S;
    const bool warm = C.warm && step_status[b] == SCVX_ST_REJECTED && ttr[b] < 1e300;
    S.set_margins(marg ? (ipm::cgptr)(marg + (size_t)b * (K + 1) * 2) : (ipm::cgptr) nullptr);
    const ipm::Result r = S.solve((ipm::cgptr)(x + (size_t)b * (K + 1) * 14), (ipm::cgptr)(u + (size_t)b * (K + 1) * NU),
                                  (ipm::cgptr)(endpoint + (size_t)b * K * 14), (typename ipm::gp<DS>::cptr)(deriv + (size_t)b * K * (14 * (14 + 2 * NU + 1))), rk[b],
                                  (ipm::cgptr)(ic + (size_t)b * 6), (ipm::gptr)(work + (size_t)b * work_stride), warm);
    const int nxu = S.L.nx + S.L.nu_;
    const int nl = ex.nlanes();
    double* so = sol + (size_t)b * (nxu + 1);
    for (int i = threadIdx.x; i < nxu; i += nl) so[i] = S.V[i];
    double* no = nu + (size_t)b * S.L.ny;
    for (int i = threadIdx.x; i < S.L.ny; i += nl) no[i] = S.V[nxu + i];
    if (threadIdx.x == 0) {
        so[nxu] = S.V[S.L.iS];
        info[4 * b + 0] = (double)r.status;
        info[4 * b + 1] = (double)r.iters;
        info[4 * b + 2] = r.merit;
        info[4 * b + 3] = r.pobj;
        ttr[b] = S.V[S.L.iTTR];
        atomicAdd(acc + ACC_SOLVES, 1.0);
        atomicAdd(acc + ACC_IPM_ITERS, (double)r.iters);
        if (r.warmed) atomicAdd(acc + ACC_WARM, 1.0);
#if defined(SCVX_IPM_PROF)
        if (b == 0) for (int i = 0; i < 32; i++) work[i] = S.prof[i];
#endif
    }
#if defined(SCVX_IPM_PROF)
    if (b == 0 && threadIdx.x > 0 && (threadIdx.x & 63) == 0 && threadIdx.x < 256)
        for (int i = 0; i < 32; i++) work[32 * (threadIdx.x >> 6) + i] = S.prof[i];
#endif
}

#ifndef SCVX_K4_OCC
#define SCVX_K4_OCC 2
#endif
template <class DS, int NU>
__global__ __launch_bounds__(64, SCVX_K4_OCC) void socp_kernel_t(ipm::Consts C, int B, size_t work_stride,
                                                  const double* __restrict__ x, const double* __restrict__ u,
                                                  const double* __restrict__ endpoint, const DS* __restrict__ deriv,
                                                  const double* __restrict__ rk, const double* __restrict__ ic,
                                                  const int* __restrict__ active, double* __restrict__ work,
                                                  double* __restrict__ sol, double* __restrict__ nu,
                                                  double* __restrict__ info, const int* __restrict__ step_status,
                                                  double* __restrict__ ttr, double* __restrict__ acc,
                                                  const double* __restrict__ marg) {
    socp_body<WaveExT<NU>, DS, NU>(C, B, work_stride, x, u, endpoint, deriv, rk, ic, active, work, sol, nu, info, step_status, ttr, acc, marg);
}
#ifndef SCVX_K4_BLOCK_OCC
#define SCVX_K4_BLOCK_OCC 2
#endif
template <int NW, class DS = double, int NU = 3>
__global__ __launch_bounds__(64 * NW, SCVX_K4_BLOCK_OCC) void socp_block_kernel(ipm::Consts C, int B, size_t work_stride,
                                                  const double* __restrict__ x, const double* __restrict__ u,
                                                  const double* __restrict__ endpoint, const DS* __restrict__ deriv,
                                                  const double* __restrict__ rk, const double* __restrict__ ic,
                                                  const int* __restrict__ active, double* __restrict__ work,
                                                  double* __restrict__ sol, double* __restrict__ nu,
                                                  double* __restrict__ info, const int* __restrict__ step_status,
                                                  double* __restrict__ ttr, double* __restrict__ acc,
                                                  const double* __restrict__ marg) {
    socp_body<BlockEx<NW, NU>, DS, NU>(C, B, work_stride, x, u, endpoint, deriv, rk, ic, active, work, sol, nu, info, step_status, ttr, acc, marg);
}

struct SocpLaunch {
    ipm::Consts C;
    int B;
    size_t work_stride;
    const double *x, *u, *endpoint, *deriv;
    const float* deriv_f;
    const double *rk, *ic;
    const int* mask;
    double *work, *sol, *nu, *info;
    const int* status;
    double *ttr, *acc;
    const double* marg;
    hipStream_t stream;
};
void launch_socp_fin(const SocpLaunch& a, int waves);

}
```

Before: 147,900.

## Fuse step tail into one kernel and relinearize only accepted trajectories via compacted list

Replaces the separate candidate/unpack/propagate/trust-region update kernels with a single fused step_tail kernel per trajectory. That kernel also builds a compacted list of trajectories that need relinearization, and the linearize kernels launch over that list so rejected trajectories cost no work. The SOCP solver also skips rebuilding the A-transposes when the data is unchanged after a rejected step. This reduces launches, intermediate buffer traffic and redundant linearization, at the cost of indirect scatter writes and more complex indexing.

```diff
diff --git a/successiveconvexification_amd/csrc/scvx_batch.hip b/successiveconvexification_amd/csrc/scvx_batch.hip
--- a/successiveconvexification_amd/csrc/scvx_batch.hip
+++ b/successiveconvexification_amd/csrc/scvx_batch.hip
@@ -54,11 +54,6 @@
     else if (r < nx + nu) u[b * nu + (r - nx)] = v;
     else sigma[b] = v;
 }
-
-struct TrParams {
-    double wNu, rh0, rh1, rh2, alph, bet, ri, nuTol, delTol;
-    int K, imax, NU, pad;
-};
 
 __global__ __launch_bounds__(64) void tr_update_kernel(TrParams P, int B, const double* __restrict__ cand,
                                                        const double* __restrict__ xprop, const double* __restrict__ nu,
@@ -211,6 +206,9 @@
     double *cov_s0 = nullptr, *cov_rep = nullptr, *cov_psig = nullptr;
     double *track_gain = nullptr, *track_p0 = nullptr;
     int *k1skip = nullptr;
+    int *k1list = nullptr;
+    int k1par = 0;
+    bool fused_tail = true;
     int *d_nlive = nullptr;
     int *h_nlive = nullptr;
     hipEvent_t ev_nlive[2] = {nullptr, nullptr};
@@ -277,11 +275,11 @@
                            b->x, b->u, b->endpoint, b->deriv, b->rk, b->ic, mask, b->work, b->sol, b->nu, b->info, b->status, b->ttr, b->acc, b->marg_on ? b->marg : nullptr);
 }
 
-hipError_t relinearize(scvx_batch* b, const int* skip) {
+hipError_t relinearize(scvx_batch* b, const int* skip, const int* list = nullptr, const int* count = nullptr) {
     const double dt = 1.0 / (b->K + 1);
     if (b->deriv_f)
-        return scvx::launch_linearize_store_f32(b->ctx, b->B, b->K, b->x, b->u, b->sigma, dt, b->endpoint, b->deriv_f, b->ctx->stream, skip);
-    return scvx::launch_linearize(b->ctx, b->B, b->K, b->x, b->u, b->sigma, dt, b->endpoint, b->deriv, b->ctx->stream, skip);
+        return scvx::launch_linearize_store_f32(b->ctx, b->B, b->K, b->x, b->u, b->sigma, dt, b->endpoint, b->deriv_f, b->ctx->stream, skip, list, count);
+    return scvx::launch_linearize(b->ctx, b->B, b->K, b->x, b->u, b->sigma, dt, b->endpoint, b->deriv, b->ctx->stream, skip, list, count);
 }
 
 int enqueue_socp(scvx_batch* b, const int* mask) {
@@ -325,6 +323,17 @@
     rc = enqueue_socp(b, mask);
     if (rc) return rc;
     if ((rc = mark(b))) return rc;
+    if (b->fused_tail) {
+        if ((rc = mark(b)) || (rc = mark(b))) return rc;
+        int* const count = b->k1list + b->B + b->k1par;
+        const scvx::StepTail a{b->tr, b->B, b->sol, b->nu, b->info, b->traj, b->x, b->u, b->sigma, b->rk, b->cost, b->iter, b->status, mask,
+                               b->active, b->live, b->out, b->acc, b->d_nlive, b->k1skip, b->k1list, count, b->k1list + b->B + (b->k1par ^ 1)};
+        SCVX_HIP(ctx, scvx::launch_step_tail(ctx, a, dt, st));
+        b->k1par ^= 1;
+        if ((rc = mark(b)) || (rc = mark(b))) return rc;
+        SCVX_HIP(ctx, relinearize(b, nullptr, b->k1list, count));
+        return mark(b);
+    }
     const size_t n = (size_t)b->B * b->nrec;
     hipLaunchKernelGGL(scvx::candidate_kernel, dim3((unsigned)((n + 255) / 256)), dim3(256), 0, st, b->B, b->nrec, b->traj,
                        b->sol, b->cand);
@@ -413,20 +422,23 @@
     b->work_stride = (L.work_doubles() + 7) & ~(size_t)7;
     if (const char* v = std::getenv("SCVX_WORK_PAD"); v && *v) b->work_stride += (size_t)std::atoi(v) & ~(size_t)7;
     const size_t nB = (size_t)B;
+    if (const char* v = std::getenv("SCVX_STEP_TAIL"); v && *v) b->fused_tail = std::atoi(v) != 0;
     int rc = 0;
     rc |= dmalloc(ctx, &b->traj, nB * b->nrec);
-    rc |= dmalloc(ctx, &b->cand, nB * b->nrec);
     rc |= dmalloc(ctx, &b->traj0, nB * b->nrec);
     rc |= dmalloc(ctx, &b->sol, nB * b->nrec);
     rc |= dmalloc(ctx, &b->x, nB * (K + 1) * 14);
     rc |= dmalloc(ctx, &b->u, nB * (K + 1) * b->NU);
     rc |= dmalloc(ctx, &b->sigma, nB);
-    rc |= dmalloc(ctx, &b->cx, nB * (K + 1) * 14);
-    rc |= dmalloc(ctx, &b->cu, nB * (K + 1) * b->NU);
-    rc |= dmalloc(ctx, &b->csigma, nB);
+    if (!b->fused_tail) {
+        rc |= dmalloc(ctx, &b->cand, nB * b->nrec);
+        rc |= dmalloc(ctx, &b->cx, nB * (K + 1) * 14);
+        rc |= dmalloc(ctx, &b->cu, nB * (K + 1) * b->NU);
+        rc |= dmalloc(ctx, &b->csigma, nB);
+        rc |= dmalloc(ctx, &b->xprop, nB * K * 14);
+    }
     rc |= dmalloc(ctx, &b->endpoint, nB * K * 14);
     rc |= dmalloc(ctx, &b->deriv, nB * K * b->dsz);
-    rc |= dmalloc(ctx, &b->xprop, nB * K * 14);
     rc |= dmalloc(ctx, &b->nu, nB * K * 14);
     rc |= dmalloc(ctx, &b->rk, nB);
     rc |= dmalloc(ctx, &b->cost, nB);
@@ -437,6 +449,8 @@
     rc |= dmalloc(ctx, &b->acc, (size_t)scvx::ACC_N);
     rc |= dmalloc(ctx, &b->d_nlive, (size_t)1);
     rc |= dmalloc(ctx, &b->k1skip, nB);
+    rc |= dmalloc(ctx, &b->k1list, nB + 2);
+    if (!rc && hipMemset(b->k1list + nB, 0, 2 * sizeof(int)) != hipSuccess) rc = SCVX_ERR_HIP;
     rc |= dmalloc(ctx, &b->marg, nB * (K + 1) * 2);
     if (!rc && (hipHostMalloc((void**)&b->h_nlive, 2 * sizeof(int), hipHostMallocDefault) != hipSuccess ||
                 hipEventCreateWithFlags(&b->ev_nlive[0], hipEventDisableTiming) != hipSuccess ||
@@ -462,7 +476,7 @@
     for (hipEvent_t e : b->ev_nlive) if (e) (void)hipEventDestroy(e);
     if (b->h_nlive) (void)hipHostFree(b->h_nlive);
     void* ptrs[] = {b->traj0, b->traj, b->cand, b->sol, b->x, b->u, b->sigma, b->cx, b->cu, b->csigma, b->endpoint, b->deriv, b->xprop,
-                    b->nu, b->rk, b->cost, b->ic, b->info, b->out, b->work, b->iter, b->status, b->active, b->live, b->ttr, b->deriv_f, b->acc, b->d_nlive, b->k1skip,
+                    b->nu, b->rk, b->cost, b->ic, b->info, b->out, b->work, b->iter, b->status, b->active, b->live, b->ttr, b->deriv_f, b->acc, b->d_nlive, b->k1skip, b->k1list,
                     b->track_gain, b->track_p0, b->marg, b->cov_s0, b->cov_rep, b->cov_psig};
     for (void* p : ptrs)
         if (p) (void)hipFree(p);
@@ -1141,9 +1155,10 @@
     int rc = check_batch(b, true);
     if (rc) return rc;
     scvx_ctx* ctx = b->ctx;
+    const size_t n = (size_t)b->B * b->nrec;
+    if (!b->cand) SCVX_HIP(ctx, hipMalloc((void**)&b->cand, n * 8));
     rc = enqueue_socp(b, b->active);
     if (rc) return rc;
-    const size_t n = (size_t)b->B * b->nrec;
     hipLaunchKernelGGL(scvx::candidate_kernel, dim3((unsigned)((n + 255) / 256)), dim3(256), 0, ctx->stream, b->B, b->nrec,
                        b->traj, b->sol, b->cand);
     SCVX_HIP(ctx, hipGetLastError());
diff --git a/successiveconvexification_amd/csrc/scvx_discretize.hip b/successiveconvexification_amd/csrc/scvx_discretize.hip
--- a/successiveconvexification_amd/csrc/scvx_discretize.hip
+++ b/successiveconvexification_amd/csrc/scvx_discretize.hip
@@ -23,6 +23,14 @@
     return true;
 }
 
+__device__ __forceinline__ long k1_nseg(long nseg, const int* list, const int* count, int K) { return list ? (long)*count * K : nseg; }
+__device__ __forceinline__ long k1_traj(const int* list, long c) { return list ? (long)list[c] : c; }
+
+template <bool LIST> __device__ __forceinline__ long k1_traj_t(const int* list, long c) {
+    if constexpr (LIST) return (long)list[c];
+    else return c;
+}
+
 template <typename R> struct Vec2;
 template <> struct Vec2<double> { typedef double2 type; };
 template <> struct Vec2<float> { typedef float2 type; };
@@ -31,9 +39,11 @@
 __global__ __launch_bounds__(64 * WAVES_PER_BLOCK, sizeof(R) == 4 ? 2 : 1) void linearize_kernel(
     DynP<R> p, long nseg, int K, const R* __restrict__ x, const R* __restrict__ u,
     const R* __restrict__ sigma, R dt, int nsub, R* __restrict__ endpoint,
-    R* __restrict__ deriv, const int* __restrict__ skip) {
+    R* __restrict__ deriv, const int* __restrict__ skip, const int* __restrict__ list, const int* __restrict__ count) {
     constexpr int LPS = K1Map<AERO>::LPS, SPW = K1Map<AERO>::SPW;
     typedef typename Vec2<R>::type VEC2;
+    nseg = k1_nseg(nseg, list, count, K);
+    if ((long)blockIdx.x * WAVES_PER_BLOCK * SPW >= nseg) return;
     if (block_unchanged(skip, (long)blockIdx.x * WAVES_PER_BLOCK * SPW, WAVES_PER_BLOCK * SPW, nseg, K)) return;
     __shared__ __attribute__((aligned(16))) R tile[WAVES_PER_BLOCK][SPW * 294];
     const int lane = threadIdx.x & 63;
@@ -46,8 +56,10 @@
     long seg = seg0 + sl;
     const bool active = (sl < SPW) && (seg < nseg);
     if (!active) seg = (seg0 < nseg) ? seg0 : nseg - 1;
-    const long b = seg / K;
-    const int k = (int)(seg - b * K);
+    const long cb = seg / K;
+    const int k = (int)(seg - cb * K);
+    const long b = k1_traj(list, cb);
+    const long pseg = b * K + k;
     const R* xk = x + ((size_t)b * (K + 1) + k) * 14;
     const R* uk = u + ((size_t)b * (K + 1) + k) * 3;
     const R sig = sigma[b];
@@ -126,15 +138,16 @@
         const long rem = nseg - seg0;
         const int nvalid = rem < SPW ? (int)rem : SPW;
         const int n2 = nvalid * 147;
-        VEC2* out = reinterpret_cast<VEC2*>(deriv + (size_t)seg0 * 294);
         const VEC2* src = reinterpret_cast<const VEC2*>(t);
 #pragma unroll
         for (int r = 0; r < (SPW * 147 + 63) / 64; r++) {
             const int e = lane + 64 * r;
-            if (e < n2) out[e] = src[e];
+            const int si = e / 147 < SPW ? e / 147 : SPW - 1;
+            const long ps = __shfl(pseg, si * LPS, 64);
+            if (e < n2) reinterpret_cast<VEC2*>(deriv + (size_t)ps * 294)[e - si * 147] = src[e];
         }
         if (active && slot == 0) {
-            R* ep = endpoint + (size_t)seg * 14;
+            R* ep = endpoint + (size_t)pseg * 14;
 #pragma unroll
             for (int i = 0; i < 14; i++) ep[i] = xs[i];
         }
@@ -174,12 +187,14 @@
 __global__ __launch_bounds__(64 * PC_WAVES) void linearize_pc_kernel(
     DynPK<R, TRQ> p, long nseg, int K, const R* __restrict__ x, const R* __restrict__ u,
     const R* __restrict__ sigma, R dt, int nsub, R* __restrict__ endpoint,
-    O* __restrict__ deriv, const int* __restrict__ skip) {
+    O* __restrict__ deriv, const int* __restrict__ skip, const int* __restrict__ list, const int* __restrict__ count) {
     constexpr int LPS = K1Map<AERO, FIN>::LPS, SPW = K1Map<AERO, FIN>::SPW;
     constexpr int NU = K1Map<AERO, FIN>::NU, NP = K1Map<AERO, FIN>::NP, DSZ = K1Map<AERO, FIN>::DSZ, HV = K1Map<AERO, FIN>::HV;
     typedef typename Vec2<R>::type VEC2;
     typedef typename Vec2<O>::type OVEC2;
     constexpr int NC = PC_WAVES - 1;
+    nseg = k1_nseg(nseg, list, count, K);
+    if ((long)blockIdx.x * (NC * SPW) >= nseg) return;
     if (block_unchanged(skip, (long)blockIdx.x * (NC * SPW), NC * SPW, nseg, K)) return;
     constexpr int NS = NC * SPW;
     constexpr int NR = StageRec<AERO, FIN, TRQ>::N;
@@ -197,8 +212,9 @@
         long seg = seg_base + (live ? lane : 0);
         const bool valid = live && seg < nseg;
         if (seg >= nseg) seg = nseg - 1;
-        const long b = seg / K;
-        const int k = (int)(seg - b * K);
+        const long cb = seg / K;
+        const int k = (int)(seg - cb * K);
+        const long b = k1_traj(list, cb);
         const R* xk = x + ((size_t)b * (K + 1) + k) * 14;
         const R* uk = u + ((size_t)b * (K + 1) + k) * NU;
         const R sig = sigma[b];
@@ -236,7 +252,7 @@
             if (!SG || s == nsub) __syncthreads();
         }
         if (valid) {
-            R* ep = endpoint + (size_t)seg * 14;
+            R* ep = endpoint + ((size_t)b * K + k) * 14;
 #pragma unroll
             for (int i = 0; i < 14; i++) ep[i] = xs[i];
         }
@@ -252,7 +268,9 @@
     const int ls = cw * SPW + (lane_live ? sl : 0);
     long seg = seg_base + ls;
     if (seg >= nseg) seg = nseg - 1;
-    const R sig = sigma[seg / K];
+    const long ctraj = k1_traj(list, seg / K);
+    const long pseg = ctraj * K + seg % K;
+    const R sig = sigma[ctraj];
     R c[14], ca[14], ct[14];
 #pragma unroll
     for (int i = 0; i < 14; i++) { c[i] = (col == i) ? R(1.0) : R(0.0); ca[i] = c[i]; ct[i] = c[i]; }
@@ -307,12 +325,13 @@
         const long rem = nseg - seg0;
         const int nvalid = rem < SPW ? (int)rem : SPW;
         const int n2 = nvalid * HV;
-        OVEC2* out = reinterpret_cast<OVEC2*>(deriv + (size_t)seg0 * DSZ);
         const VEC2* src = reinterpret_cast<const VEC2*>(t);
 #pragma unroll
         for (int r = 0; r < (SPW * HV + 63) / 64; r++) {
             const int e = lane + 64 * r;
-            if (e < n2) { const VEC2 v = src[e]; OVEC2 o; o.x = O(v.x); o.y = O(v.y); out[e] = o; }
+            const int si = e / HV < SPW ? e / HV : SPW - 1;
+            const long ps = __shfl(pseg, si * LPS, 64);
+            if (e < n2) { const VEC2 v = src[e]; OVEC2 o; o.x = O(v.x); o.y = O(v.y); reinterpret_cast<OVEC2*>(deriv + (size_t)ps * DSZ)[e - si * HV] = o; }
         }
     }
 }
@@ -320,11 +339,11 @@
 #ifndef SCVX_K1_NB_EXO
 #define SCVX_K1_NB_EXO 1
 #endif
-template <bool AERO, typename R, typename O = R, bool FIN = false, int NB = 1, bool TRQ = false>
-__global__ __launch_bounds__(64 * PC_WAVES) void linearize_pcp_kernel(
-    DynPK<R, TRQ> p, long nseg, int K, const R* __restrict__ x, const R* __restrict__ u,
+template <bool LIST, bool AERO, typename R, typename O, bool FIN, int NB, bool TRQ>
+__device__ __forceinline__ void linearize_pcp_body(
+    const DynPK<R, TRQ>& p, long nseg, int K, const R* __restrict__ x, const R* __restrict__ u,
     const R* __restrict__ sigma, R dt, int nsub, R* __restrict__ endpoint,
-    O* __restrict__ deriv, const int* __restrict__ skip) {
+    O* __restrict__ deriv, const int* __restrict__ skip, const int* __restrict__ list, const int* __restrict__ count) {
     constexpr int LPS = K1Map<AERO, FIN>::LPS, SPW = K1Map<AERO, FIN>::SPW;
     constexpr int NU = K1Map<AERO, FIN>::NU, NP = K1Map<AERO, FIN>::NP, DSZ = K1Map<AERO, FIN>::DSZ, HV = K1Map<AERO, FIN>::HV;
     typedef typename Vec2<R>::type VEC2;
@@ -339,6 +358,7 @@
     constexpr bool SHARE = false;
     __shared__ __attribute__((aligned(16))) R lds[SHARE ? (RING_D > TILE_D ? RING_D : TILE_D) : RING_D + TILE_D];
     R* const tiles = SHARE ? lds : lds + RING_D;
+    __shared__ long psegs[LIST ? 2 * NS : 1];
     const int lane = threadIdx.x & 63;
     const int wave = threadIdx.x >> 6;
 #if defined(SCVX_K1_PROF)
@@ -347,6 +367,7 @@
 #endif
     const R h = dt / R(nsub);
     const R inv_n = R(1.0) / R(nsub);
+    if constexpr (LIST) nseg = (long)*count * K;
     const long ngrp = (nseg + NS - 1) / NS;
     auto advance = [&](long g) {
         while (g < ngrp && block_unchanged(skip, g * NS, NS, nseg, K)) g += gridDim.x;
@@ -358,11 +379,15 @@
         const bool live = lane < NS;
         const int l = live ? lane : 0;
         R nx[14], nu6[2 * NU], nsig = R(0.0);
+        long npseg = 0;
+        int par = 0;
         auto fetch = [&](long g) {
             long seg = g * NS + l;
             if (seg >= nseg) seg = nseg - 1;
-            const long b = seg / K;
-            const int k = (int)(seg - b * K);
+            const long cb = seg / K;
+            const int k = (int)(seg - cb * K);
+            const long b = k1_traj_t<LIST>(list, cb);
+            if constexpr (LIST) npseg = b * K + k;
             const R* xk = x + ((size_t)b * (K + 1) + k) * 14;
             const R* uk = u + ((size_t)b * (K + 1) + k) * NU;
 #pragma unroll
@@ -376,6 +401,7 @@
             const long nxt = advance(grp + gridDim.x);
             const long seg = grp * NS + l;
             const bool valid = live && seg < nseg;
+            if constexpr (LIST) { if (live) psegs[par * NS + l] = npseg; }
             const R sig = nsig;
             R xs[14], xa[14], xt[14];
 #pragma unroll
@@ -411,7 +437,7 @@
             }
             if (nxt < ngrp) fetch(nxt);
             if (valid) {
-                R* ep = endpoint + (size_t)seg * 14;
+                R* ep = endpoint + (size_t)(LIST ? psegs[par * NS + l] : seg) * 14;
 #pragma unroll
                 for (int i = 0; i < 14; i++) ep[i] = xs[i];
             }
@@ -419,6 +445,7 @@
             for (int bb = 0; bb < NB; bb++) K1_BAR();
             if (SHARE) K1_BAR();
             grp = nxt;
+            if constexpr (LIST) par ^= 1;
         }
 #if defined(SCVX_K1_PROF)
         if (blockIdx.x == 0 && lane == 0) { g_k1prof[2 * wave] = k1wait_; g_k1prof[2 * wave + 1] = (double)(__builtin_amdgcn_s_memtime() - k1t0_); }
@@ -444,11 +471,12 @@
     auto sigma_of = [&](long g, int bb) {
         long seg = g * NS + ls[bb];
         if (seg >= nseg) seg = nseg - 1;
-        return sigma[seg / K];
+        return sigma[k1_traj_t<LIST>(list, seg / K)];
     };
     R nsig[NB];
 #pragma unroll
     for (int bb = 0; bb < NB; bb++) nsig[bb] = grp < ngrp ? sigma_of(grp, bb) : R(0.0);
+    int par = 0;
     while (grp < ngrp) {
         const long nxt = advance(grp + gridDim.x);
         const long seg_base = grp * NS;
@@ -518,30 +546,55 @@
 #pragma unroll
                 for (int r = 0; r < (SPW * HV + 63) / 64; r++) {
                     const int e = lane + 64 * r;
-                    if (e < n2) { const VEC2 v = src[e]; OVEC2 o; o.x = O(v.x); o.y = O(v.y); out[e] = o; }
+                    if constexpr (LIST) {
+                        if (e < n2) {
+                            const int si = e / HV;
+                            const long ps = psegs[par * NS + (bb * NC + cw) * SPW + si];
+                            const VEC2 v = src[e]; OVEC2 o; o.x = O(v.x); o.y = O(v.y);
+                            reinterpret_cast<OVEC2*>(deriv + (size_t)ps * DSZ)[e - si * HV] = o;
+                        }
+                    } else {
+                        if (e < n2) { const VEC2 v = src[e]; OVEC2 o; o.x = O(v.x); o.y = O(v.y); out[e] = o; }
+                    }
                 }
             }
         }
         if (SHARE) K1_BAR();
         grp = nxt;
+        if constexpr (LIST) par ^= 1;
     }
 #if defined(SCVX_K1_PROF)
     if (blockIdx.x == 0 && lane == 0) { g_k1prof[2 * wave] = k1wait_; g_k1prof[2 * wave + 1] = (double)(__builtin_amdgcn_s_memtime() - k1t0_); }
 #endif
 }
 
-#ifndef SCVX_K1_SPLIT
-#define SCVX_K1_SPLIT 1
-#endif
-#ifndef SCVX_K1_NB
-#define SCVX_K1_NB 2
-#endif
-template <bool AERO> struct K1Split { static constexpr int NB = AERO ? SCVX_K1_NB : 1; };
-template <bool AERO, typename R, typename O = R, bool FIN = false, bool TRQ = false>
-__global__ __launch_bounds__(64 * PC_WAVES) void linearize_pcp2_kernel(
+template <bool AERO, typename R, typename O = R, bool FIN = false, int NB = 1, bool TRQ = false>
+__global__ __launch_bounds__(64 * PC_WAVES) void linearize_pcp_kernel(
     DynPK<R, TRQ> p, long nseg, int K, const R* __restrict__ x, const R* __restrict__ u,
     const R* __restrict__ sigma, R dt, int nsub, R* __restrict__ endpoint,
     O* __restrict__ deriv, const int* __restrict__ skip) {
+    linearize_pcp_body<false, AERO, R, O, FIN, NB, TRQ>(p, nseg, K, x, u, sigma, dt, nsub, endpoint, deriv, skip, nullptr, nullptr);
+}
+template <bool AERO, typename R, typename O = R, bool FIN = false, int NB = 1, bool TRQ = false>
+__global__ __launch_bounds__(64 * PC_WAVES) void linearize_pcp_list_kernel(
+    DynPK<R, TRQ> p, int K, const R* __restrict__ x, const R* __restrict__ u,
+    const R* __restrict__ sigma, R dt, int nsub, R* __restrict__ endpoint,
+    O* __restrict__ deriv, const int* __restrict__ list, const int* __restrict__ count) {
+    linearize_pcp_body<true, AERO, R, O, FIN, NB, TRQ>(p, 0, K, x, u, sigma, dt, nsub, endpoint, deriv, nullptr, list, count);
+}
+
+#ifndef SCVX_K1_SPLIT
+#define SCVX_K1_SPLIT 1
+#endif
+#ifndef SCVX_K1_NB
+#define SCVX_K1_NB 2
+#endif
+template <bool AERO> struct K1Split { static constexpr int NB = AERO ? SCVX_K1_NB : 1; };
+template <bool LIST, bool AERO, typename R, typename O, bool FIN, bool TRQ>
+__device__ __forceinline__ void linearize_pcp2_body(
+    const DynPK<R, TRQ>& p, long nseg, int K, const R* __restrict__ x, const R* __restrict__ u,
+    const R* __restrict__ sigma, R dt, int nsub, R* __restrict__ endpoint,
+    O* __restrict__ deriv, const int* __restrict__ skip, const int* __restrict__ list, const int* __restrict__ count) {
     static_assert(AERO || FIN, "the exo producer is not the bottleneck");
     constexpr int LPS = K1Map<AERO, FIN>::LPS, SPW = K1Map<AERO, FIN>::SPW;
     constexpr int NU = K1Map<AERO, FIN>::NU, NP = K1Map<AERO, FIN>::NP, DSZ = K1Map<AERO, FIN>::DSZ, HV = K1Map<AERO, FIN>::HV;
@@ -555,6 +608,7 @@
     __shared__ __attribute__((aligned(16))) R lds[RING_D + HAND_D + TILE_D];
     R* const hand = lds + RING_D;
     R* const tiles = hand + HAND_D;
+    __shared__ long psegs[LIST ? 2 * NS : 1];
     const int lane = threadIdx.x & 63;
     const int wave = threadIdx.x >> 6;
 #if defined(SCVX_K1_PROF)
@@ -564,6 +618,7 @@
     const R h = dt / R(nsub);
     const R inv_n = R(1.0) / R(nsub);
     const int T = 4 * nsub;
+    if constexpr (LIST) nseg = (long)*count * K;
     const long ngrp = (nseg + NS - 1) / NS;
     auto advance = [&](long g) {
         while (g < ngrp && block_unchanged(skip, g * NS, NS, nseg, K)) g += gridDim.x;
@@ -575,11 +630,15 @@
         const bool live = lane < NS;
         const int l = live ? lane : 0;
         R nx[14], nu6[2 * NU], nsig = R(0.0);
+        long npseg = 0;
+        int par = 0;
         auto fetch = [&](long g) {
             long seg = g * NS + l;
             if (seg >= nseg) seg = nseg - 1;
-            const long b = seg / K;
-            const int k = (int)(seg - b * K);
+            const long cb = seg / K;
+            const int k = (int)(seg - cb * K);
+            const long b = k1_traj_t<LIST>(list, cb);
+            if constexpr (LIST) npseg = b * K + k;
             const R* xk = x + ((size_t)b * (K + 1) + k) * 14;
             const R* uk = u + ((size_t)b * (K + 1) + k) * NU;
 #pragma unroll
@@ -593,6 +652,7 @@
             const long nxt = advance(grp + gridDim.x);
             const long seg = grp * NS + l;
             const bool valid = live && seg < nseg;
+            if constexpr (LIST) { if (live) psegs[par * NS + l] = npseg; }
             const R sig = nsig;
             R xs[14], xa[14], xt[14];
 #pragma unroll
@@ -630,13 +690,14 @@
             K1_BAR();
             if (nxt < ngrp) fetch(nxt);
             if (valid) {
-                R* ep = endpoint + (size_t)seg * 14;
+                R* ep = endpoint + (size_t)(LIST ? psegs[par * NS + l] : seg) * 14;
 #pragma unroll
                 for (int i = 0; i < 14; i++) ep[i] = xs[i];
             }
 #pragma unroll
             for (int bb = 0; bb < NB; bb++) K1_BAR();
             grp = nxt;
+            if constexpr (LIST) par ^= 1;
         }
 #if defined(SCVX_K1_PROF)
         if (blockIdx.x == 0 && lane == 0) { g_k1prof[2 * wave] = k1wait_; g_k1prof[2 * wave + 1] = (double)(__builtin_amdgcn_s_memtime() - k1t0_); }
@@ -685,11 +746,12 @@
     auto sigma_of = [&](long g, int bb) {
         long seg = g * NS + ls[bb];
         if (seg >= nseg) seg = nseg - 1;
-        return sigma[seg / K];
+        return sigma[k1_traj_t<LIST>(list, seg / K)];
     };
     R nsig[NB];
 #pragma unroll
     for (int bb = 0; bb < NB; bb++) nsig[bb] = grp < ngrp ? sigma_of(grp, bb) : R(0.0);
+    int par = 0;
     while (grp < ngrp) {
         const long nxt = advance(grp + gridDim.x);
         const long seg_base = grp * NS;
@@ -753,15 +815,75 @@
 #pragma unroll
                 for (int r = 0; r < (SPW * HV + 63) / 64; r++) {
                     const int e = lane + 64 * r;
-                    if (e < n2) { const VEC2 v = src[e]; OVEC2 o; o.x = O(v.x); o.y = O(v.y); out[e] = o; }
+                    if constexpr (LIST) {
+                        if (e < n2) {
+                            const int si = e / HV;
+                            const long ps = psegs[par * NS + (bb * NC + cw) * SPW + si];
+                            const VEC2 v = src[e]; OVEC2 o; o.x = O(v.x); o.y = O(v.y);
+                            reinterpret_cast<OVEC2*>(deriv + (size_t)ps * DSZ)[e - si * HV] = o;
+                        }
+                    } else {
+                        if (e < n2) { const VEC2 v = src[e]; OVEC2 o; o.x = O(v.x); o.y = O(v.y); out[e] = o; }
+                    }
                 }
             }
         }
         grp = nxt;
+        if constexpr (LIST) par ^= 1;
     }
 #if defined(SCVX_K1_PROF)
     if (blockIdx.x == 0 && lane == 0) { g_k1prof[2 * wave] = k1wait_; g_k1prof[2 * wave + 1] = (double)(__builtin_amdgcn_s_memtime() - k1t0_); }
 #endif
+}
+
+template <bool AERO, typename R, typename O = R, bool FIN = false, bool TRQ = false>
+__global__ __launch_bounds__(64 * PC_WAVES) void linearize_pcp2_kernel(
+    DynPK<R, TRQ> p, long nseg, int K, const R* __restrict__ x, const R* __restrict__ u,
+    const R* __restrict__ sigma, R dt, int nsub, R* __restrict__ endpoint,
+    O* __restrict__ deriv, const int* __restrict__ skip) {
+    linearize_pcp2_body<false, AERO, R, O, FIN, TRQ>(p, nseg, K, x, u, sigma, dt, nsub, endpoint, deriv, skip, nullptr, nullptr);
+}
+template <bool AERO, typename R, typename O = R, bool FIN = false, bool TRQ = false>
+__global__ __launch_bounds__(64 * PC_WAVES) void linearize_pcp2_list_kernel(
+    DynPK<R, TRQ> p, int K, const R* __restrict__ x, const R* __restrict__ u,
+    const R* __restrict__ sigma, R dt, int nsub, R* __restrict__ endpoint,
+    O* __restrict__ deriv, const int* __restrict__ list, const int* __restrict__ count) {
+    linearize_pcp2_body<true, AERO, R, O, FIN, TRQ>(p, 0, K, x, u, sigma, dt, nsub, endpoint, deriv, nullptr, list, count);
+}
+
+template <bool AERO, typename R, bool FIN, bool TRQ, int NU>
+__device__ __forceinline__ void propagate_segment(const DynPK<R, TRQ>& p, R (&xs)[14], const R (&ukv)[NU], const R (&upv)[NU], R sig, R dt,
+                                                  int nsub) {
+    const R h = dt / R(nsub);
+    const R inv_n = R(1.0) / R(nsub);
+    for (int s = 0; s < nsub; s++) {
+        R xa[14], xt[14];
+#pragma unroll
+        for (int i = 0; i < 14; i++) {
+            xa[i] = xs[i];
+            xt[i] = xs[i];
+        }
+#pragma unroll
+        for (int stg = 0; stg < 4; stg++) {
+            const R lkp = (R(s) + (stg == 0 ? R(0.0) : (stg == 3 ? R(1.0) : R(0.5)))) * inv_n;
+            const R lkm = R(1.0) - lkp;
+            R uu[NU];
+#pragma unroll
+            for (int j = 0; j < NU; j++) uu[j] = fma(ukv[j], lkm, upv[j] * lkp);
+            R g[14];
+            rhs_only<AERO, FIN, TRQ>(p, xt, uu, g);
+            const R wacc = h * ((stg == 0 || stg == 3) ? (R(1.0) / R(6.0)) : (R(1.0) / R(3.0)));
+            const R wnext = h * (stg == 2 ? R(1.0) : R(0.5));
+#pragma unroll
+            for (int i = 0; i < 14; i++) {
+                const R dx = sig * g[i];
+                xa[i] = fma(wacc, dx, xa[i]);
+                if (stg < 3) xt[i] = fma(wnext, dx, xs[i]);
+            }
+        }
+#pragma unroll
+        for (int i = 0; i < 14; i++) xs[i] = xa[i];
+    }
 }
 
 template <bool AERO, typename R, bool FIN = false, bool TRQ = false>
@@ -783,44 +905,120 @@
     R ukv[NU], upv[NU];
 #pragma unroll
     for (int j = 0; j < NU; j++) { ukv[j] = uk[j]; upv[j] = uk[NU + j]; }
-    const R h = dt / R(nsub);
-    const R inv_n = R(1.0) / R(nsub);
-    for (int s = 0; s < nsub; s++) {
-        R xa[14], xt[14];
-#pragma unroll
-        for (int i = 0; i < 14; i++) {
-            xa[i] = xs[i];
-            xt[i] = xs[i];
-        }
-#pragma unroll
-        for (int stg = 0; stg < 4; stg++) {
-            const R lkp = (R(s) + (stg == 0 ? R(0.0) : (stg == 3 ? R(1.0) : R(0.5)))) * inv_n;
-            const R lkm = R(1.0) - lkp;
-            R uu[NU];
-#pragma unroll
-            for (int j = 0; j < NU; j++) uu[j] = fma(ukv[j], lkm, upv[j] * lkp);
-            R g[14];
-            rhs_only<AERO, FIN, TRQ>(p, xt, uu, g);
-            const R wacc = h * ((stg == 0 || stg == 3) ? (R(1.0) / R(6.0)) : (R(1.0) / R(3.0)));
-            const R wnext = h * (stg == 2 ? R(1.0) : R(0.5));
-#pragma unroll
-            for (int i = 0; i < 14; i++) {
-                const R dx = sig * g[i];
-                xa[i] = fma(wacc, dx, xa[i]);
-                if (stg < 3) xt[i] = fma(wnext, dx, xs[i]);
-            }
-        }
-#pragma unroll
-        for (int i = 0; i < 14; i++) xs[i] = xa[i];
-    }
+    propagate_segment<AERO, R, FIN, TRQ, NU>(p, xs, ukv, upv, sig, dt, nsub);
     R* o = xnext + (size_t)seg * 14;
 #pragma unroll
     for (int i = 0; i < 14; i++) o[i] = xs[i];
+}
+
+template <bool AERO, bool FIN = false, bool TRQ = false>
+__global__ __launch_bounds__(64) void step_tail_kernel(DynPK<double, TRQ> p, StepTail a, double dt, int nsub) {
+    extern __shared__ __attribute__((aligned(16))) double tail_lds[];
+    const int b = blockIdx.x;
+    if (b >= a.B) return;
+    if (b == 0 && threadIdx.x == 0) *a.k1count_next = 0;
+    if (!a.mask[b]) {
+        if (threadIdx.x == 0) a.k1skip[b] = SCVX_ST_REJECTED;
+        return;
+    }
+    const TrParams& P = a.P;
+    constexpr int NU = FIN ? 5 : 3;
+    const int K = P.K, nrec = (K + 1) * (14 + NU) + 1, nx = (K + 1) * 14;
+    double* const c = tail_lds;
+    double* const xp = tail_lds + nrec;
+    double* const t = a.traj + (size_t)b * nrec;
+    const double* const so = a.sol + (size_t)b * nrec;
+    for (int i = threadIdx.x; i < nrec; i += 64) c[i] = t[i] + so[i];
+    __syncthreads();
+    const double sig = c[nrec - 1];
+    for (int k = threadIdx.x; k < K; k += 64) {
+        double xs[14], ukv[NU], upv[NU];
+#pragma unroll
+        for (int i = 0; i < 14; i++) xs[i] = c[14 * k + i];
+#pragma unroll
+        for (int j = 0; j < NU; j++) { ukv[j] = c[nx + NU * k + j]; upv[j] = c[nx + NU * (k + 1) + j]; }
+        propagate_segment<AERO, double, FIN, TRQ, NU>(p, xs, ukv, upv, sig, dt, nsub);
+#pragma unroll
+        for (int i = 0; i < 14; i++) xp[14 * k + i] = xs[i];
+    }
+    __syncthreads();
+    const double* nv = a.nu + (size_t)b * K * 14;
+    double d2 = 0, n2 = 0;
+    for (int i = threadIdx.x; i < K * 14; i += 64) {
+        const double d = c[14 + i] - xp[i];
+        d2 += d * d;
+        n2 += nv[i] * nv[i];
+    }
+#pragma unroll
+    for (int o = 32; o > 0; o >>= 1) { d2 += __shfl_xor(d2, o, 64); n2 += __shfl_xor(n2, o, 64); }
+    const double mf = c[14 * K];
+    const double jK = -mf + P.wNu * sqrt(d2);
+    const double nun = sqrt(n2);
+    const double lK = -mf + P.wNu * nun;
+    const int sstat = (int)a.info[4 * b];
+    int st;
+    bool accept = false;
+    const double rkb = a.rk[b];
+    double next_rk = rkb, dJ = INFINITY;
+    if (sstat != 0 && sstat != 4) {
+        st = sstat == 3 ? SCVX_ST_NONFINITE : (sstat == 5 ? SCVX_ST_INFEASIBLE : SCVX_ST_SOLVER);
+    } else if (!(jK == jK) || !(lK == lK)) {
+        st = SCVX_ST_NONFINITE;
+    } else {
+        const double jKm = a.cost[b];
+        const double djk = jKm - jK, dlk = jKm - lK;
+        const double rhk = djk / dlk;
+        if (rkb == INFINITY) { next_rk = P.ri; accept = true; dJ = NAN; }
+        else if (rhk < P.rh0) { next_rk = rkb / P.alph; accept = false; dJ = INFINITY; }
+        else {
+            accept = true;
+            dJ = djk;
+            if (rhk < P.rh1) next_rk = rkb / P.alph;
+            else if (P.rh1 <= rhk && rhk < P.rh2) next_rk = rkb;
+            else next_rk = P.bet * rkb;
+        }
+        st = accept ? SCVX_ST_RUNNING : SCVX_ST_REJECTED;
+    }
+    if (accept) {
+        double* xo = a.x + (size_t)b * nx;
+        double* uo = a.u + (size_t)b * (K + 1) * NU;
+        for (int i = threadIdx.x; i < nrec; i += 64) {
+            const double v = c[i];
+            t[i] = v;
+            if (i < nx) xo[i] = v;
+            else if (i < nrec - 1) uo[i - nx] = v;
+            else a.sigma[b] = v;
+        }
+    }
+    if (threadIdx.x == 0) {
+        const int it = a.iter[b] + 1;
+        a.iter[b] = it;
+        const int was_live = a.live[b];
+        if (st == SCVX_ST_SOLVER || st == SCVX_ST_NONFINITE || st == SCVX_ST_INFEASIBLE) {
+            a.active[b] = 0;
+            a.live[b] = 0;
+        } else {
+            a.rk[b] = next_rk;
+            if (accept) a.cost[b] = jK;
+            if (accept && nun <= P.nuTol && dJ <= P.delTol) { st = SCVX_ST_CONVERGED; a.live[b] = 0; }
+        }
+        if (was_live && !a.live[b]) atomicSub(a.nlive, 1);
+        a.status[b] = st;
+        a.k1skip[b] = accept ? SCVX_ST_RUNNING : SCVX_ST_REJECTED;
+        if (accept) a.k1list[atomicAdd(a.k1count, 1)] = b;
+        a.out[2 * b] = nun;
+        a.out[2 * b + 1] = dJ;
+        atomicAdd(a.acc + ACC_TRAJ_STEPS, 1.0);
+        if (st == SCVX_ST_REJECTED) atomicAdd(a.acc + ACC_REJECTED, 1.0);
+        else if (st == SCVX_ST_CONVERGED) atomicAdd(a.acc + ACC_CONVERGED, 1.0);
+        else if (st != SCVX_ST_RUNNING) atomicAdd(a.acc + ACC_FAILED, 1.0);
+    }
 }
 
 template <typename R>
 hipError_t launch_linearize_simple(const scvx_ctx* ctx, int B, int K, const R* x, const R* u, const R* sigma, R dt,
-                                   R* endpoint, R* deriv, hipStream_t st, const int* skip = nullptr) {
+                                   R* endpoint, R* deriv, hipStream_t st, const int* skip = nullptr, const int* list = nullptr,
+                                   const int* count = nullptr) {
     const long nseg = (long)B * K;
     if (nseg == 0) return hipSuccess;
     const int spw = ctx->dyn.aero ? K1Map<true>::SPW : K1Map<false>::SPW;
@@ -829,22 +1027,22 @@
     const DynP<R> dp(ctx->dyn);
     if (ctx->dyn.aero)
         hipLaunchKernelGGL((linearize_kernel<true, R>), dim3(grid), dim3(64 * WAVES_PER_BLOCK), 0, st, dp, nseg, K, x, u,
-                           sigma, dt, ctx->nsub, endpoint, deriv, skip);
+                           sigma, dt, ctx->nsub, endpoint, deriv, skip, list, count);
     else
         hipLaunchKernelGGL((linearize_kernel<false, R>), dim3(grid), dim3(64 * WAVES_PER_BLOCK), 0, st, dp, nseg, K, x, u,
-                           sigma, dt, ctx->nsub, endpoint, deriv, skip);
+                           sigma, dt, ctx->nsub, endpoint, deriv, skip, list, count);
     return hipGetLastError();
 }
 
 template <typename R, typename O = R>
 hipError_t launch_linearize_t(const scvx_ctx* ctx, int B, int K, const R* x, const R* u, const R* sigma, R dt, R* endpoint,
-                              O* deriv, hipStream_t st, const int* skip = nullptr) {
+                              O* deriv, hipStream_t st, const int* skip = nullptr, const int* list = nullptr, const int* count = nullptr) {
     const long nseg = (long)B * K;
     if (nseg == 0) return hipSuccess;
     const bool fin = ctx->dyn.fin != 0;
     const bool trq = ctx->dyn.trq != 0;
     if constexpr (std::is_same<R, O>::value)
-        if (ctx->k1_variant == 0 && !fin && !trq) return launch_linearize_simple<R>(ctx, B, K, x, u, sigma, dt, endpoint, deriv, st, skip);
+        if (ctx->k1_variant == 0 && !fin && !trq) return launch_linearize_simple<R>(ctx, B, K, x, u, sigma, dt, endpoint, deriv, st, skip, list, count);
     const bool split = SCVX_K1_SPLIT != 0 && (fin || ctx->dyn.aero) && ctx->k1_sg != 0 && (ctx->k1_persist < 0 ? ctx->nsub >= 3 : ctx->k1_persist != 0);
     const bool exo_nb = !fin && !ctx->dyn.aero && ctx->k1_sg != 0 && (ctx->k1_persist < 0 ? ctx->nsub >= 3 : ctx->k1_persist != 0);
     const int ns = (PC_WAVES - (split ? 2 : 1)) * (split ? (ctx->dyn.aero ? K1Split<true>::NB : K1Split<false>::NB) : (exo_nb ? SCVX_K1_NB_EXO : 1))
@@ -856,52 +1054,64 @@
     const unsigned grid = (unsigned)(!persist || ngrp < cap ? ngrp : cap);
     const dim3 g(grid), blk(64 * PC_WAVES);
     const DynP<R> dp(ctx->dyn);
+#define K1_PERSISTENT(KERN, DP, ...)                                                                                                              \
+    do {                                                                                                                                          \
+        if constexpr (std::is_same<R, double>::value) {                                                                                           \
+            if (list) {                                                                                                                           \
+                hipLaunchKernelGGL((KERN##_list_kernel<__VA_ARGS__>), g, blk, 0, st, DP, K, x, u, sigma, dt, ctx->nsub, endpoint, deriv, list, count); \
+                break;                                                                                                                            \
+            }                                                                                                                                     \
+        }                                                                                                                                         \
+        hipLaunchKernelGGL((KERN##_kernel<__VA_ARGS__>), g, blk, 0, st, DP, nseg, K, x, u, sigma, dt, ctx->nsub, endpoint, deriv, skip);         \
+    } while (0)
     if (trq) {
         const DynPT<R> dpt(ctx->dyn);
         if (split) {
-            if (fin) hipLaunchKernelGGL((linearize_pcp2_kernel<true, R, O, true, true>), g, blk, 0, st, dpt, nseg, K, x, u, sigma, dt, ctx->nsub, endpoint, deriv, skip);
-            else hipLaunchKernelGGL((linearize_pcp2_kernel<true, R, O, false, true>), g, blk, 0, st, dpt, nseg, K, x, u, sigma, dt, ctx->nsub, endpoint, deriv, skip);
+            if (fin) K1_PERSISTENT(linearize_pcp2, dpt, true, R, O, true, true);
+            else K1_PERSISTENT(linearize_pcp2, dpt, true, R, O, false, true);
         } else if (persist) {
-            if (fin) hipLaunchKernelGGL((linearize_pcp_kernel<true, R, O, true, 1, true>), g, blk, 0, st, dpt, nseg, K, x, u, sigma, dt, ctx->nsub, endpoint, deriv, skip);
-            else hipLaunchKernelGGL((linearize_pcp_kernel<true, R, O, false, 1, true>), g, blk, 0, st, dpt, nseg, K, x, u, sigma, dt, ctx->nsub, endpoint, deriv, skip);
+            if (fin) K1_PERSISTENT(linearize_pcp, dpt, true, R, O, true, 1, true);
+            else K1_PERSISTENT(linearize_pcp, dpt, true, R, O, false, 1, true);
         } else {
-            if (fin) hipLaunchKernelGGL((linearize_pc_kernel<true, true, R, O, true, true>), g, blk, 0, st, dpt, nseg, K, x, u, sigma, dt, ctx->nsub, endpoint, deriv, skip);
-            else hipLaunchKernelGGL((linearize_pc_kernel<true, true, R, O, false, true>), g, blk, 0, st, dpt, nseg, K, x, u, sigma, dt, ctx->nsub, endpoint, deriv, skip);
+            if (fin) hipLaunchKernelGGL((linearize_pc_kernel<true, true, R, O, true, true>), g, blk, 0, st, dpt, nseg, K, x, u, sigma, dt, ctx->nsub, endpoint, deriv, skip, list, count);
+            else hipLaunchKernelGGL((linearize_pc_kernel<true, true, R, O, false, true>), g, blk, 0, st, dpt, nseg, K, x, u, sigma, dt, ctx->nsub, endpoint, deriv, skip, list, count);
         }
     } else if (split) {
         if (fin) {
-            if (ctx->dyn.aero) hipLaunchKernelGGL((linearize_pcp2_kernel<true, R, O, true>), g, blk, 0, st, dp, nseg, K, x, u, sigma, dt, ctx->nsub, endpoint, deriv, skip);
-            else hipLaunchKernelGGL((linearize_pcp2_kernel<false, R, O, true>), g, blk, 0, st, dp, nseg, K, x, u, sigma, dt, ctx->nsub, endpoint, deriv, skip);
-        } else hipLaunchKernelGGL((linearize_pcp2_kernel<true, R, O, false>), g, blk, 0, st, dp, nseg, K, x, u, sigma, dt, ctx->nsub, endpoint, deriv, skip);
+            if (ctx->dyn.aero) K1_PERSISTENT(linearize_pcp2, dp, true, R, O, true);
+            else K1_PERSISTENT(linearize_pcp2, dp, false, R, O, true);
+        } else K1_PERSISTENT(linearize_pcp2, dp, true, R, O, false);
     } else if (fin) {
         if (persist) {
-            if (ctx->dyn.aero) hipLaunchKernelGGL((linearize_pcp_kernel<true, R, O, true>), g, blk, 0, st, dp, nseg, K, x, u, sigma, dt, ctx->nsub, endpoint, deriv, skip);
-            else hipLaunchKernelGGL((linearize_pcp_kernel<false, R, O, true>), g, blk, 0, st, dp, nseg, K, x, u, sigma, dt, ctx->nsub, endpoint, deriv, skip);
+            if (ctx->dyn.aero) K1_PERSISTENT(linearize_pcp, dp, true, R, O, true);
+            else K1_PERSISTENT(linearize_pcp, dp, false, R, O, true);
         } else {
-            if (ctx->dyn.aero) hipLaunchKernelGGL((linearize_pc_kernel<true, true, R, O, true>), g, blk, 0, st, dp, nseg, K, x, u, sigma, dt, ctx->nsub, endpoint, deriv, skip);
-            else hipLaunchKernelGGL((linearize_pc_kernel<false, true, R, O, true>), g, blk, 0, st, dp, nseg, K, x, u, sigma, dt, ctx->nsub, endpoint, deriv, skip);
+            if (ctx->dyn.aero) hipLaunchKernelGGL((linearize_pc_kernel<true, true, R, O, true>), g, blk, 0, st, dp, nseg, K, x, u, sigma, dt, ctx->nsub, endpoint, deriv, skip, list, count);
+            else hipLaunchKernelGGL((linearize_pc_kernel<false, true, R, O, true>), g, blk, 0, st, dp, nseg, K, x, u, sigma, dt, ctx->nsub, endpoint, deriv, skip, list, count);
         }
     } else if (persist) {
-        if (ctx->dyn.aero) hipLaunchKernelGGL((linearize_pcp_kernel<true, R, O>), g, blk, 0, st, dp, nseg, K, x, u, sigma, dt, ctx->nsub, endpoint, deriv, skip);
-        else hipLaunchKernelGGL((linearize_pcp_kernel<false, R, O, false, SCVX_K1_NB_EXO>), g, blk, 0, st, dp, nseg, K, x, u, sigma, dt, ctx->nsub, endpoint, deriv, skip);
+        if (ctx->dyn.aero) K1_PERSISTENT(linearize_pcp, dp, true, R, O);
+        else K1_PERSISTENT(linearize_pcp, dp, false, R, O, false, SCVX_K1_NB_EXO);
     } else if (ctx->dyn.aero) {
-        if (sg) hipLaunchKernelGGL((linearize_pc_kernel<true, true, R, O>), g, blk, 0, st, dp, nseg, K, x, u, sigma, dt, ctx->nsub, endpoint, deriv, skip);
-        else hipLaunchKernelGGL((linearize_pc_kernel<true, false, R, O>), g, blk, 0, st, dp, nseg, K, x, u, sigma, dt, ctx->nsub, endpoint, deriv, skip);
+        if (sg) hipLaunchKernelGGL((linearize_pc_kernel<true, true, R, O>), g, blk, 0, st, dp, nseg, K, x, u, sigma, dt, ctx->nsub, endpoint, deriv, skip, list, count);
+        else hipLaunchKernelGGL((linearize_pc_kernel<true, false, R, O>), g, blk, 0, st, dp, nseg, K, x, u, sigma, dt, ctx->nsub, endpoint, deriv, skip, list, count);
     } else {
-        if (sg) hipLaunchKernelGGL((linearize_pc_kernel<false, true, R, O>), g, blk, 0, st, dp, nseg, K, x, u, sigma, dt, ctx->nsub, endpoint, deriv, skip);
-        else hipLaunchKernelGGL((linearize_pc_kernel<false, false, R, O>), g, blk, 0, st, dp, nseg, K, x, u, sigma, dt, ctx->nsub, endpoint, deriv, skip);
-    }
+        if (sg) hipLaunchKernelGGL((linearize_pc_kernel<false, true, R, O>), g, blk, 0, st, dp, nseg, K, x, u, sigma, dt, ctx->nsub, endpoint, deriv, skip, list, count);
+        else hipLaunchKernelGGL((linearize_pc_kernel<false, false, R, O>), g, blk, 0, st, dp, nseg, K, x, u, sigma, dt, ctx->nsub, endpoint, deriv, skip, list, count);
+    }
+#undef K1_PERSISTENT
     return hipGetLastError();
 }
 
 hipError_t launch_linearize(const scvx_ctx* ctx, int B, int K, const double* x, const double* u, const double* sigma,
-                            double dt, double* endpoint, double* deriv, hipStream_t st, const int* skip) {
-    return launch_linearize_t<double>(ctx, B, K, x, u, sigma, dt, endpoint, deriv, st, skip);
+                            double dt, double* endpoint, double* deriv, hipStream_t st, const int* skip, const int* list, const int* count) {
+    return launch_linearize_t<double>(ctx, B, K, x, u, sigma, dt, endpoint, deriv, st, skip, list, count);
 }
 
 hipError_t launch_linearize_store_f32(const scvx_ctx* ctx, int B, int K, const double* x, const double* u, const double* sigma,
-                                      double dt, double* endpoint, float* deriv, hipStream_t st, const int* skip) {
-    return launch_linearize_t<double, float>(ctx, B, K, x, u, sigma, dt, endpoint, deriv, st, skip);
+                                      double dt, double* endpoint, float* deriv, hipStream_t st, const int* skip, const int* list,
+                                      const int* count) {
+    return launch_linearize_t<double, float>(ctx, B, K, x, u, sigma, dt, endpoint, deriv, st, skip, list, count);
 }
 
 hipError_t launch_linearize_f32(const scvx_ctx* ctx, int B, int K, const float* x, const float* u, const float* sigma,
@@ -942,6 +1152,26 @@
     return launch_propagate_t<float>(ctx, B, K, x, u, sigma, dt, xnext, st);
 }
 
+hipError_t launch_step_tail(const scvx_ctx* ctx, const StepTail& a, double dt, hipStream_t st) {
+    if (a.B == 0) return hipSuccess;
+    const int K = a.P.K;
+    const size_t lds = ((size_t)(K + 1) * (14 + a.P.NU) + 1 + (size_t)K * 14) * sizeof(double);
+    const dim3 g(a.B), blk(64);
+    const DynP<double> dp(ctx->dyn);
+    if (ctx->dyn.trq) {
+        const DynPT<double> dpt(ctx->dyn);
+        if (ctx->dyn.fin) hipLaunchKernelGGL((step_tail_kernel<true, true, true>), g, blk, lds, st, dpt, a, dt, ctx->nsub);
+        else hipLaunchKernelGGL((step_tail_kernel<true, false, true>), g, blk, lds, st, dpt, a, dt, ctx->nsub);
+    } else if (ctx->dyn.fin) {
+        if (ctx->dyn.aero) hipLaunchKernelGGL((step_tail_kernel<true, true>), g, blk, lds, st, dp, a, dt, ctx->nsub);
+        else hipLaunchKernelGGL((step_tail_kernel<false, true>), g, blk, lds, st, dp, a, dt, ctx->nsub);
+    } else if (ctx->dyn.aero)
+        hipLaunchKernelGGL((step_tail_kernel<true>), g, blk, lds, st, dp, a, dt, ctx->nsub);
+    else
+        hipLaunchKernelGGL((step_tail_kernel<false>), g, blk, lds, st, dp, a, dt, ctx->nsub);
+    return hipGetLastError();
+}
+
 #if defined(SCVX_K1_PROF)
 extern "C" int scvx_debug_k1_prof(double* out32) {
     (void)hipDeviceSynchronize();
diff --git a/successiveconvexification_amd/csrc/scvx_internal.hpp b/successiveconvexification_amd/csrc/scvx_internal.hpp
--- a/successiveconvexification_amd/csrc/scvx_internal.hpp
+++ b/successiveconvexification_amd/csrc/scvx_internal.hpp
@@ -31,11 +31,33 @@
 struct NcclId { char internal[SCVX_COMM_ID_BYTES]; };
 
 hipError_t launch_linearize(const scvx_ctx* ctx, int B, int K, const double* x, const double* u, const double* sigma,
-                            double dt, double* endpoint, double* deriv, hipStream_t st, const int* skip = nullptr);
+                            double dt, double* endpoint, double* deriv, hipStream_t st, const int* skip = nullptr,
+                            const int* list = nullptr, const int* count = nullptr);
 hipError_t launch_linearize_store_f32(const scvx_ctx* ctx, int B, int K, const double* x, const double* u, const double* sigma,
-                                      double dt, double* endpoint, float* deriv, hipStream_t st, const int* skip = nullptr);
+                                      double dt, double* endpoint, float* deriv, hipStream_t st, const int* skip = nullptr,
+                                      const int* list = nullptr, const int* count = nullptr);
 hipError_t launch_propagate(const scvx_ctx* ctx, int B, int K, const double* x, const double* u, const double* sigma,
                             double dt, double* xnext, hipStream_t st);
+
+struct TrParams {
+    double wNu, rh0, rh1, rh2, alph, bet, ri, nuTol, delTol;
+    int K, imax, NU, pad;
+};
+enum { ACC_TRAJ_STEPS = 0, ACC_SOLVES, ACC_IPM_ITERS, ACC_WARM, ACC_SKIPPED, ACC_REJECTED, ACC_FAILED, ACC_CONVERGED, ACC_N };
+struct StepTail {
+    TrParams P;
+    int B;
+    const double *sol, *nu, *info;
+    double *traj, *x, *u, *sigma;
+    double *rk, *cost;
+    int *iter, *status;
+    const int* mask;
+    int *active, *live;
+    double *out, *acc;
+    int *nlive, *k1skip, *k1list, *k1count;
+    int *k1count_next;
+};
+hipError_t launch_step_tail(const scvx_ctx* ctx, const StepTail& a, double dt, hipStream_t st);
 
 hipError_t launch_linearize_f32(const scvx_ctx* ctx, int B, int K, const float* x, const float* u, const float* sigma,
                                 float dt, float* endpoint, float* deriv, hipStream_t st);
diff --git a/successiveconvexification_amd/csrc/scvx_ipm_core.hpp b/successiveconvexification_amd/csrc/scvx_ipm_core.hpp
--- a/successiveconvexification_amd/csrc/scvx_ipm_core.hpp
+++ b/successiveconvexification_amd/csrc/scvx_ipm_core.hpp
@@ -412,6 +412,7 @@
     gptr tmpl, tmpl2;
     gptr uhat, lb0, tmx;
     cgptr marg = nullptr;
+    bool keep_at = false;
     gptr wh, Vw, yw, Sw, Zw;
     double h_tr[4], h_nu[4], hrk, hnui;
     double q_tr[2], q_nu[2], q_sg[4], h00s;
@@ -3187,6 +3188,7 @@
     }
 
     SCVX_HD void set_margins(cgptr m) { marg = m; }
+    SCVX_HD void keep_transposes(bool k) { keep_at = k; }
 
     SCVX_HD Result solve(cdptr xbar_, cdptr ubar_, cdptr endpoint_, dcptr D_,
                          double rk_, cdptr ic, gptr work, bool warm = false) {
@@ -3195,7 +3197,7 @@
         carve(work);
         const int K = L.K;
         for (int r = ex.lane(); r < L.ny; r += ex.nlanes()) dk[r] = endpoint[r] - xbar[14 + r];
-        {
+        if (!keep_at) {
             const dcptr D_ = D; const dptr At_ = At;
             stream(0, 196 * K, [&](int e) { const int k = e / 196, r = e - 196 * k, i = r / 14, j = r - 14 * i; return D_[(size_t)k * DSZ + 14 * j + i]; },
                    [&](int e, double v) { At_[e] = v; });
diff --git a/successiveconvexification_amd/csrc/scvx_socp.hpp b/successiveconvexification_amd/csrc/scvx_socp.hpp
--- a/successiveconvexification_amd/csrc/scvx_socp.hpp
+++ b/successiveconvexification_amd/csrc/scvx_socp.hpp
@@ -546,7 +546,9 @@
     }
 };
 
-enum { ACC_TRAJ_STEPS = 0, ACC_SOLVES, ACC_IPM_ITERS, ACC_WARM, ACC_SKIPPED, ACC_REJECTED, ACC_FAILED, ACC_CONVERGED, ACC_N };
+#ifndef SCVX_KEEP_AT
+#define SCVX_KEEP_AT 1
+#endif
 
 template <class Ex, class DS = double, int NU = 3>
 __device__ __forceinline__ void socp_body(const ipm::Consts& Cin, int B, size_t work_stride, const double* x, const double* u,
@@ -580,8 +582,10 @@
     const ipm::Consts& C = F->C;
     Ex& ex = F->ex;
     SolverT& S = F->S;
-    const bool warm = C.warm && step_status[b] == SCVX_ST_REJECTED && ttr[b] < 1e300;
+    const bool same_data = step_status[b] == SCVX_ST_REJECTED && ttr[b] < 1e300;
+    const bool warm = C.warm && same_data;
     S.set_margins(marg ? (ipm::cgptr)(marg + (size_t)b * (K + 1) * 2) : (ipm::cgptr) nullptr);
+    S.keep_transposes(SCVX_KEEP_AT != 0 && same_data);
     const ipm::Result r = S.solve((ipm::cgptr)(x + (size_t)b * (K + 1) * 14), (ipm::cgptr)(u + (size_t)b * (K + 1) * NU),
                                   (ipm::cgptr)(endpoint + (size_t)b * K * 14), (typename ipm::gp<DS>::cptr)(deriv + (size_t)b * K * (14 * (14 + 2 * NU + 1))), rk[b],
                                   (ipm::cgptr)(ic + (size_t)b * 6), (ipm::gptr)(work + (size_t)b * work_stride), warm);
```

After: 149,000, median of 6. About the same (+0.7%).
